# BaeHann/feature_level_style_transfer_for_TSC

Measured on AMD Instinct MI355X. Metric: train-step samples/sec (univariate TS, len=512, batch=256) at 1/2/4/8 MI355X, higher is better.
Workload: dtype bf16x3

## Files before the change

### feature_level_style_transfer_for_tsc_amd/_lib.py

```python
from __future__ import annotations

import ctypes
import os
from ctypes import POINTER, Structure, c_char_p, c_float, c_int, c_int32, c_int64, c_void_p
from typing import Optional

import torch

ABI_VERSION = 21
_LIB_NAME = "libfst_hip.so"
_HERE = os.path.dirname(os.path.abspath(__file__))
LIB_PATH = os.environ.get("FST_HIP_LIB", os.path.join(_HERE, _LIB_NAME))


class FstLibraryError(RuntimeError):
    pass


class WSrc(Structure):
    _fields_ = [("w", c_void_p), ("off0", c_int64), ("sm", c_int64), ("sc", c_int64), ("st", c_int64)]


_P = c_void_p
_I32P = c_void_p
_SIGNATURES = {
    "fst_version": (c_int, []),
    "fst_last_error": (c_char_p, []),
    "fst_pack_weights": (c_int, [_I32P, _I32P, c_int, POINTER(WSrc), POINTER(WSrc), c_int, c_int, c_int, c_int, _P, c_void_p]),
    "fst_pack_weights_bf16x3": (c_int, [_I32P, _I32P, c_int, POINTER(WSrc), POINTER(WSrc), c_int, c_int, c_int, c_int, _P, c_void_p]),
    "fst_unpack_weights": (c_int, [_I32P, _I32P, c_int, _P, c_int, _P, c_int64, c_int64, c_int64, c_int64,
                                   _P, c_int64, c_int64, c_int64, c_int64, c_int, c_void_p]),
    "fst_mask_taps": (c_int, [_P, _I32P, _I32P, c_int, c_int, c_int, c_void_p]),
    "fst_conv_gemm": (c_int, [_P, c_int64, _P, c_int64, _P, _I32P, _I32P, c_int, _P, _P, c_int64, _P, c_int64,
                              _P, c_int64, c_int, c_int, c_int, c_int, c_int, c_int, c_int, c_int, c_void_p]),
    "fst_conv_wgrad": (c_int, [_P, c_int64, _P, c_int64, _P, c_int64, _P, c_int64, c_int, _P, _I32P, _I32P, c_int,
                               c_int, c_int, c_int, c_int, c_int, c_int64, c_void_p]),
    "fst_conv_last_route": (c_int, [POINTER(c_int32)]),
    "fst_row_sum": (c_int, [_P, c_int64, c_int, c_int, c_int, _P, c_void_p]),
    "fst_bn_stats": (c_int, [_P, c_int, c_int, c_int, _P, c_int64, c_void_p]),
    "fst_bn_finalize": (c_int, [_P, c_int, _P, _P, _P, _P, c_int, c_int, c_float, c_float, _P, c_void_p]),
    "fst_bn_apply": (c_int, [_P, _P, _P, _P, _P, c_int, c_int, c_int, c_int, c_int64, c_void_p]),
    "fst_bn_bwd_reduce": (c_int, [_P, _P, _P, _P, c_int, c_int, c_int, c_int, _P, c_int64, c_void_p]),
    "fst_bn_bwd_apply": (c_int, [_P, _P, _P, _P, _P, c_int, _P, _P, _P, c_int, c_int, c_int, c_int, c_int, c_int, c_int64, c_void_p]),
    "fst_bn_bwd_reduce_join": (c_int, [_P, _P, _P, _P, _P, c_int, c_int, c_int, _P, _P, c_int64, c_void_p]),
    "fst_bn_bwd_apply_join": (c_int, [_P, _P, _P, _P, _P, _P, _P, c_int, _P, _P, _P, _P, _P, _P, c_int, c_int, c_int, c_int, c_int,
                                      c_int64, c_void_p]),
    "fst_gate_fwd": (c_int, [_P, _P, c_int, c_int, c_int, c_int64, c_void_p]),
    "fst_gate_bwd": (c_int, [_P, _P, _P, c_int, c_int, c_int, c_int64, c_void_p]),
    "fst_coupling_sum_slots": (c_int64, [c_int, c_int, c_int]),
    "fst_coupling_fwd": (c_int, [_P, _P, _P, c_int, c_int, c_int, c_int64, _P, c_void_p]),
    "fst_coupling_bwd": (c_int, [_P, _P, _P, _P, _P, _P, _P, _P, c_int, c_int, c_int, c_int64, c_void_p]),
    "fst_coupling_inv_fwd": (c_int, [_P, _P, _P, c_int, c_int, c_int, c_int64, c_void_p]),
    "fst_coupling_inv_bwd": (c_int, [_P, _P, _P, _P, _P, c_int, c_int, c_int, c_int64, c_void_p]),
    "fst_rmsprop_multi": (c_int, [_P, _P, _P, _P, _P, c_int, c_float, c_float, c_void_p]),
    "fst_adam_multi": (c_int, [_P, _P, _P, _P, _P, c_int, _P, c_float, c_float, c_float, c_float, c_void_p]),
    "fst_rmsprop_multi_dev": (c_int, [_P, _P, _P, _P, _P, c_int, c_float, c_float, c_void_p]),
    "fst_adam_multi_dev": (c_int, [_P, _P, _P, _P, _P, c_int, _P, _P, c_float, c_float, c_float, c_void_p]),
    "fst_nonfinite_slots": (c_int64, [c_int]),
    "fst_nonfinite_multi": (c_int, [_P, _P, _I32P, c_int, c_int32, _I32P, c_int64, _I32P, _I32P, _P, _I32P, c_void_p]),
    "fst_rmsprop_multi_guard": (c_int, [_P, _P, _P, _P, _P, _P, c_int, c_float, c_float, _I32P, c_void_p]),
    "fst_adam_multi_guard": (c_int, [_P, _P, _P, _P, _P, c_int, _P, c_float, _P, c_float, c_float, c_float, _I32P, c_void_p]),
    "fst_guard_copy_multi": (c_int, [_P, _P, _P, c_int, _I32P, c_int, c_void_p]),
    "fst_wn_stack_fwd_ok": (c_int, [c_int, c_int, c_int, c_int]),
    "fst_wn_stack_fwd": (c_int, [_P, _P, _P, c_int64, _P, _P, _P, c_int64, _P, c_int, c_int, c_int, c_int, c_int, c_int64, c_void_p]),
    "fst_wn_stack_infer": (c_int, [_P, _P, _P, c_int64, _P, _P, c_int64, _P, c_int, c_int, c_int, c_int, c_int, c_int64, c_void_p]),
    "fst_wn_stack_bwd_ok": (c_int, [c_int, c_int, c_int, c_int]),
    "fst_wn_stack_bwd": (c_int, [_P, _P, _P, _P, _P, _P, _P, _P, _P, c_int64, c_int, c_int, c_int, c_int, c_int, c_int64, c_void_p]),
    "fst_wn_stack_bwd_proj": (c_int, [_P, _P, _P, _P, _P, _P, _P, _P, c_int, c_int64, _P, c_int64, c_int, c_int, c_int, c_int, c_int,
                                      c_int64, c_void_p]),
    "fst_wn_wgrad_ok": (c_int, [c_int, c_int, c_int, c_int, c_int, c_int]),
    "fst_wn_wgrad_workspace_floats": (c_int64, [c_int, c_int, c_int, c_int, c_int, c_int]),
    "fst_wn_wgrad_in": (c_int, [_P, _P, _P, c_int, c_int64, _P, _P, _P, c_int64, c_int, c_int, c_int, c_int, c_int, c_int, c_int64,
                                c_void_p]),
    "fst_wn_wgrad_rs": (c_int, [_P, _P, _P, c_int, _P, _P, c_int64, c_int, c_int, c_int, c_int, c_int64, c_void_p]),
    "fst_wn_wgrad_in_slabs": (c_int, [_P, _P, _P, c_int, c_int64, _P, c_int64, c_int, c_int, c_int, c_int, c_int, c_int, c_int64,
                                      c_void_p]),
    "fst_wn_wgrad_rs_slabs": (c_int, [_P, _P, _P, c_int, _P, c_int64, c_int, c_int, c_int, c_int, c_int64, c_void_p]),
    "fst_wn_wgrad_reduce_many": (c_int, [_I32P, _I32P, _I32P, _P, _P, _P, _P, c_int, c_int, c_int, c_int, c_int, c_void_p]),
    "fst_nt_gemm_workspace_floats": (c_int64, [c_int, c_int, c_int]),
    "fst_nt_gemm": (c_int, [_P, _P, _P, _P, c_int64, c_int, c_int, c_int, _P, _P, c_int, c_float, _P, c_void_p]),
    "fst_tap_wgrad_ok": (c_int, [c_int, c_int, c_int, c_int, c_int, c_int, c_int]),
    "fst_tap_wgrad_workspace_floats": (c_int64, [c_int, c_int, c_int, c_int, c_int]),
    "fst_tap_wgrad": (c_int, [_P, _P, _P, _P, c_int64, c_int, c_int, c_int, c_int, c_int, c_int, c_int, c_int, c_int64, c_int64, c_void_p]),
    "fst_dense_tap_wgrad_ok": (c_int, [c_int, c_int, c_int, c_int, c_int, c_int]),
    "fst_dense_tap_wgrad_workspace_floats": (c_int64, [c_int, c_int, c_int, c_int, c_int]),
    "fst_dense_tap_wgrad": (c_int, [_P, _P, _P, _P, c_int64, c_int, c_int, c_int, c_int, c_int, c_int, c_int64, c_int64, c_void_p]),
    "fst_wn_last_route": (c_int, [POINTER(c_int32)]),
    "fst_relu_bwd": (c_int, [_P, _P, _P, c_int64, c_void_p]),
    "fst_gemm_workspace_floats": (c_int64, [c_int, c_int, c_int]),
    "fst_gemm": (c_int, [_P, c_int64, c_int, _P, c_int64, c_int, _P, c_int64, c_int, c_int, c_int, _P, c_int, c_float, _P, c_int64,
                         c_void_p]),
    "fst_gemm_f32_workspace_floats": (c_int64, [c_int, c_int, c_int]),
    "fst_gemm_f32": (c_int, [_P, c_int64, c_int, _P, c_int64, c_int, _P, c_int64, c_int, c_int, c_int, _P, c_int, c_float, _P, c_int64,
                             c_void_p]),
    "fst_act_bwd": (c_int, [_P, _P, _P, c_int64, c_float, c_void_p]),
    "fst_batch_sum": (c_int, [_P, _P, _P, c_int, c_int64, c_int, c_void_p]),
    "fst_noise_transfer_fwd": (c_int, [_P, c_int, c_int, _P, _P, c_float, c_float, _P, _P, _P, _P, _P, _P, _P, c_int, c_int, c_void_p]),
    "fst_bcast_add": (c_int, [_P, _P, _P, c_int, c_int64, c_void_p]),
    "fst_noise_transfer_bwd": (c_int, [_P, c_int, _P, _P, _P, _P, c_int, c_int, c_void_p]),
    "fst_noise_transfer_dw": (c_int, [_P, _P, _P, _P, c_int, c_int, c_void_p]),
    "fst_noise_transfer_bwd_apply": (c_int, [_P, _P, _P, _P, c_float, c_float, c_int, _P, _P, c_int64, c_void_p]),
    "fst_wn_fold_fwd": (c_int, [_P, c_int, _P, _P, c_void_p]),
    "fst_wn_fold_bwd": (c_int, [_P, c_int, _P, _P, _P, c_void_p]),
    "fst_logdet_inv": (c_int, [_P, c_int, _P, _P, c_void_p]),
    "fst_wn_image_bytes": (c_int64, [c_int, c_int]),
    "fst_wn_pack": (c_int, [_P, _P, _P, _P, _P, _P, c_int, c_int, c_int, c_int, _P, c_int64, c_void_p]),
    "fst_wn_pack_stack": (c_int, [_P, _P, _P, _P, _P, _P, c_int, c_int, c_int, c_int, _P, c_int64, c_void_p]),
    "fst_wn_layer_fwd": (c_int, [_P, c_int64, _P, c_int64, _P, c_int64, _P, _P, _P, _P, c_int, c_int, c_int, c_int, c_int, c_int,
                                 c_int, c_int64, c_void_p]),
    "fst_wn_layer_infer": (c_int, [_P, c_int64, _P, c_int64, _P, c_int64, _P, _P, c_int, c_int, c_int, c_int, c_int, c_int, c_int,
                                   c_int64, c_void_p]),
    "fst_wn_bwd_image_bytes": (c_int64, [c_int, c_int]),
    "fst_wn_pack_bwd": (c_int, [_P, c_int, c_int, c_int, _P, c_int64, c_void_p]),
    "fst_wn_pack_bwd_stack": (c_int, [_P, c_int, c_int, c_int, _P, c_int64, c_void_p]),
    "fst_wn_bwd_proj_image_bytes": (c_int64, [c_int, c_int, c_int]),
    "fst_wn_pack_bwd_proj_stack": (c_int, [_P, _P, c_int, c_int, c_int, _P, c_int64, c_void_p]),
    "fst_wn_layer_bwd": (c_int, [_P, _P, _P, _P, c_int64, _P, _P, c_int64, c_int, c_int, c_int, c_int, c_int64, c_void_p]),
    "fst_wn_dgrad_image_bytes": (c_int64, [c_int]),
    "fst_wn_pack_dgrad": (c_int, [_P, _P, c_int, c_int, c_int, _P, c_int64, c_void_p]),
    "fst_wn_pack_dgrad_stack": (c_int, [_P, _P, c_int, c_int, c_int, c_int, _P, c_int64, c_void_p]),
    "fst_wn_dgrad_fits": (c_int, [c_int, c_int, c_int]),
    "fst_wn_layer_dgrad": (c_int, [_P, _P, c_int64, _P, _P, _P, _P, c_int64, c_int, c_int, c_int, c_int, c_int, c_int64, c_int64,
                                   c_void_p]),
    "fst_gru_fwd": (c_int, [_P, _P, _P, _P, _P, _I32P, c_int, c_int, c_int, c_int, c_int64, c_void_p]),
    "fst_gru_bwd": (c_int, [_P, _P, _P, _P, _I32P, c_int, _P, _P, c_int, c_int, c_int, c_int64, c_void_p]),
    "fst_lstm2_fwd": (c_int, [_P, _P, _P, _P, c_int, c_int, c_int64, c_void_p]),
    "fst_lstm2_bwd": (c_int, [_P, _P, _P, _P, _P, c_int, c_int, c_int64, c_void_p]),
    "fst_axpy": (c_int, [_P, _P, c_float, c_int64, c_void_p]),
    "fst_add_slices": (c_int, [_P, c_int64, _P, c_int64, _P, c_int64, c_int, c_int, c_int, c_void_p]),
    "fst_cpc_workspace_floats": (c_int64, [c_int, c_int, c_int, c_int]),
    "fst_cpc_nce_slots": (c_int64, [c_int, c_int, c_int, c_int]),
    "fst_cpc_nce_fwd": (c_int, [_P, c_int64, c_int64, c_int64, _I32P, _P, c_int, c_int, c_int, c_int, c_int, _P, _P, _P, c_void_p]),
    "fst_cpc_nce_bwd": (c_int, [_P, c_int64, c_int64, c_int64, _I32P, _P, _P, c_int, c_int, c_int, c_int, c_int, _P, _P, _P,
                                c_void_p]),
}
EXPORTED_SYMBOLS = tuple(_SIGNATURES)

_lib: Optional[ctypes.CDLL] = None


def load(path: Optional[str] = None) -> ctypes.CDLL:
    global _lib
    if _lib is not None and path is None:
        return _lib
    p = path or LIB_PATH
    if not os.path.exists(p):
        raise FstLibraryError(
            f"{p} not found — build it with `python -c 'import __graft_entry__ as g; g.build()'` "
            "(hipcc --offload-arch=gfx950).  There is no CPU fallback.")
    try:
        lib = ctypes.CDLL(p)
    except OSError as e:
        raise FstLibraryError(f"cannot load {p}: {e}") from e
    for name, (res, args) in _SIGNATURES.items():
        try:
            fn = getattr(lib, name)
        except AttributeError as e:
            raise FstLibraryError(f"{p} does not export {name}; rebuild the library") from e
        fn.restype, fn.argtypes = res, args
    if lib.fst_version() != ABI_VERSION:
        raise FstLibraryError(f"{p}: ABI version {lib.fst_version()} != expected {ABI_VERSION}; rebuild")
    if path is None:
        _lib = lib
    return lib


def check(rc: int, what: str) -> None:
    if rc != 0:
        msg = load().fst_last_error()
        raise RuntimeError(f"{what} failed (rc={rc}): {msg.decode() if msg else '?'}")


def stream_ptr() -> int:
    return torch.cuda.current_stream().cuda_stream


def ptr(t: Optional[torch.Tensor]) -> Optional[int]:
    return None if t is None else t.data_ptr()


def require_gpu_tensor(t: torch.Tensor, name: str) -> None:
    if not t.is_cuda:
        raise FstLibraryError(f"{name} lives on {t.device}; the fst ops run on an MI355X only (no CPU fallback)")
    if t.dtype != torch.float32:
        raise TypeError(f"{name} must be float32, got {t.dtype}")
```

### feature_level_style_transfer_for_tsc_amd/csrc/wn_fused.hip

```cpp
#include "fst_device.h"
#include <type_traits>

#define WS_MAXL 10
#define WN_TN 128
#define WN_A_BYTES (8 * 2048)
#define WN_TILE_BYTES (32 * 36 * 4)
#define WN_FWD_LDS(NW) (3 * (WN_A_BYTES + 2 * (((NW) + 1) * 1024 + 128)))

__device__ __forceinline__ float wn_sigmoid(float x) {
  return __builtin_amdgcn_rcpf(1.0f + __builtin_amdgcn_exp2f(-1.44269504f * x));
}
__device__ __forceinline__ float wn_tanh(float x) {
  return 1.0f - 2.0f * __builtin_amdgcn_rcpf(1.0f + __builtin_amdgcn_exp2f(2.88539008f * x));
}

constexpr int WN_GRP = 2;
__host__ __device__ __forceinline__ void wn_stage_chunk_tap(int k, int CH, int& c, int& tap) {
  const int g = k / (3 * WN_GRP), rem = k - g * 3 * WN_GRP;
  const int gs = CH - g * WN_GRP < WN_GRP ? CH - g * WN_GRP : WN_GRP;
  tap = rem / gs;
  c = g * WN_GRP + rem - gs * tap;
}

struct WnPackParams {
// ... 508 lines not shown
#pragma unroll
    for (int mb = 0; mb < 8; ++mb) {
      if (mb + 1 < 8 && !(p.last && mb + 1 < 4)) a_frag(mb + 1);
      if (!(p.last && mb < 4)) mfma_bf3(acc[mb], fah[mb % 2], fal[mb % 2], bh2[ks], bl2[ks]);
      if (more && mb >= 4) {
        __builtin_amdgcn_sched_barrier(0);
        issue_piece(nxt, mb - 4);
        __builtin_amdgcn_sched_barrier(0);
      }
    }
    slot = slot == 2 ? 0 : slot + 1;
  }

  FST_T(tg2);
  FST_ACC(7, tg1, tg2);
#pragma unroll
  for (int blk = 0; blk < 4; ++blk) {
    const int rows_e = n - blk * 32;
    if (!p.last) ws_acc_store(acc[blk], an_rs, wl, blk * 32, tcol, rows_e, L);
    ws_acc_store(acc[blk + 4], out_rs, wl, blk * 32, tcol, rows_e, L);
  }
  FST_T(tg3);
  FST_ACC(8, tg2, tg3);
  FST_ACC(9, ts0, tg3);
  FST_FLUSH(wn_stamps);
}

template <int NW>
__global__ __launch_bounds__(64 * NW, NW == 4 ? 2 : 1) void wn_layer_fwd_kernel(WnFwdParams p) {
  extern __shared__ __attribute__((aligned(16))) float lds[];
  int wg = blockIdx.x;
  if ((p.n_wg & 7) == 0) wg = (wg & 7) * (p.n_wg >> 3) + (wg >> 3);
  const int b = wg / p.tiles_per_seq;
  const int t0 = (wg - b * p.tiles_per_seq) * (32 * NW);
  wn_fwd_tile<NW>(*(WnFwdArgs*)__builtin_amdgcn_kernarg_segment_ptr(), b, t0, reinterpret_cast<char*>(lds));
}

struct WnFwdStackParams {
  WnFwdParams layer[WS_MAXL];
  int nl;
};

__global__ __launch_bounds__(512, 1) void wn_stack_fwd_kernel(WnFwdStackParams ps_by_value) {
  extern __shared__ __attribute__((aligned(16))) float lds[];
  typedef const __attribute__((address_space(4))) WnFwdStackParams StackArgs;
  StackArgs& ps = *(StackArgs*)__builtin_amdgcn_kernarg_segment_ptr();
  (void)ps_by_value;
  char* const ldsb = reinterpret_cast<char*>(lds);
  const int B = ps.layer[0].B, passes = ps.layer[0].tiles_per_seq;
  for (int b = blockIdx.x; b < B; b += gridDim.x) {
    for (int layer = 0; layer < ps.nl; ++layer) {
      for (int pass = 0; pass < passes; ++pass) {
        WnFwdArgs* qp = &ps.layer[layer];
        asm volatile("" : "+s"(qp));
        wn_fwd_tile<8>(*qp, b, pass * 256, ldsb);
        wait_vmcnt<0>();
        __syncthreads();
      }
    }
  }
}

template <int NW>
__global__ __launch_bounds__(64 * NW, NW == 4 ? 2 : 1) void wn_layer_infer_kernel(WnFwdParams p) {
  extern __shared__ __attribute__((aligned(16))) float lds[];
  int wg = blockIdx.x;
  if ((p.n_wg & 7) == 0) wg = (wg & 7) * (p.n_wg >> 3) + (wg >> 3);
  const int b = wg / p.tiles_per_seq;
  const int t0 = (wg - b * p.tiles_per_seq) * (32 * NW);
  wn_fwd_tile<NW, false>(*(WnFwdArgs*)__builtin_amdgcn_kernarg_segment_ptr(), b, t0, reinterpret_cast<char*>(lds));
}

__global__ __launch_bounds__(512, 1) void wn_stack_infer_kernel(WnFwdStackParams ps_by_value) {
  extern __shared__ __attribute__((aligned(16))) float lds[];
  typedef const __attribute__((address_space(4))) WnFwdStackParams StackArgs;
  StackArgs& ps = *(StackArgs*)__builtin_amdgcn_kernarg_segment_ptr();
  (void)ps_by_value;
  char* const ldsb = reinterpret_cast<char*>(lds);
  const int B = ps.layer[0].B, passes = ps.layer[0].tiles_per_seq;
  for (int b = blockIdx.x; b < B; b += gridDim.x) {
    for (int layer = 0; layer < ps.nl; ++layer) {
      for (int pass = 0; pass < passes; ++pass) {
        WnFwdArgs* qp = &ps.layer[layer];
        asm volatile("" : "+s"(qp));
        wn_fwd_tile<8, false>(*qp, b, pass * 256, ldsb);
        wait_vmcnt<0>();
        __syncthreads();
      }
    }
  }
}

extern "C" int fst_wn_stack_fwd_ok(int n, int h, int L, int nl) {
  return n > 0 && n < 128 && h > 0 && L > 0 && L % 256 == 0 && nl >= 1 && nl <= WS_MAXL;
}

static int wn_stack_fwd_launch(const char* who, bool save, const float* const* a_in, const int64_t* a_bs, const void* const* images,
                               int64_t image_bytes, float* const* ts, float* const* a_next, const float* u0, int64_t u0_bs,
                               float* out, int nl, int B, int L, int n, int h, int64_t numel_a, void* stream) {
  FST_REQUIRE(a_in && a_bs && images && (ts || !save) && a_next && u0 && out, "%s: null operand", who);
  FST_REQUIRE(fst_wn_stack_fwd_ok(n, h, L, nl) && B > 0, "%s: B=%d L=%d n=%d h=%d nl=%d (needs n < 128, L %% 256 == 0, "
              "1 <= nl <= %d)", who, B, L, n, h, nl, WS_MAXL);
  FST_REQUIRE((long long)B * n * L == (long long)numel_a, "%s: B*n*L = %d*%d*%d does not match the element count %lld "
              "of the [B, n, L] tensors", who, B, n, L, (long long)numel_a);
  FST_REQUIRE(image_bytes == fst_wn_image_bytes(n, h), "%s: images are %lld bytes, expected %lld", who,
              (long long)image_bytes, (long long)fst_wn_image_bytes(n, h));
  FST_REQUIRE(B == 1 || u0_bs >= (int64_t)h * L, "%s: batch stride of u0 smaller than a sample", who);
  FST_REQUIRE(u0_bs % 4 == 0 && fst_aligned16(u0) && fst_aligned16(out), "%s: needs 16-byte aligned tensors", who);
  WnFwdStackParams p = {};
  for (int i = 0; i < nl; ++i) {
    const bool last = i == nl - 1;
    float* const ts_i = save ? ts[i] : nullptr;
    FST_REQUIRE(a_in[i] && images[i] && (ts_i || !save) && (a_next[i] || last), "%s: null operand of layer %d", who, i);
    FST_REQUIRE(a_bs[i] >= (int64_t)n * L && a_bs[i] % 4 == 0 && fst_aligned16(a_in[i]) && fst_aligned16(images[i]) && fst_aligned16(ts_i) && fst_aligned16(a_next[i]),
                "%s: layer %d: batch stride %lld smaller than a sample, or an operand that is not 16-byte aligned", who, i,
                (long long)a_bs[i]);
    FST_REQUIRE(last || a_in[i + 1] == a_next[i], "%s: the input of layer %d is not the a_next of layer %d", who, i + 1, i);
    FST_REQUIRE(save || last || a_next[i] != a_in[i], "%s: layer %d would store a_next over the input its neighbouring "
                "tiles still read", who, i);
    WnFwdParams& q = p.layer[i];
    q.a = a_in[i]; q.a_bs = a_bs[i]; q.u0 = u0; q.u0_bs = u0_bs; q.img = static_cast<const char*>(images[i]);
    q.ts = ts_i; q.acts = nullptr; q.a_next = last ? nullptr : a_next[i]; q.out = out;
    q.B = B; q.L = L; q.n = n; q.h = h; q.dil = 1 << i; q.first = i == 0; q.last = last;
    q.CH = wn_ch(n); q.CH2 = wn_ch2(h); q.tiles_per_seq = L / 256; q.n_wg = 0;
  }
  p.nl = nl;
  const int cus = fst_cu_count_or(256);
  const dim3 grid((unsigned)(B < cus ? B : cus));
  if (int rc = fst_allow_full_lds(save ? (const void*)wn_stack_fwd_kernel : (const void*)wn_stack_infer_kernel, who)) return rc;
  fst_wn_set_route(save ? FST_WN_ROUTE_STACK_FWD : FST_WN_ROUTE_STACK_INFER, 8, 0, 0, 0, (int)grid.x, 1, 1, L / 256, 3, nl, WN_FWD_LDS(8));
  if (save) {
    hipLaunchKernelGGL(wn_stack_fwd_kernel, grid, dim3(512), WN_FWD_LDS(8), (hipStream_t)stream, p);
  } else {
    hipLaunchKernelGGL(wn_stack_infer_kernel, grid, dim3(512), WN_FWD_LDS(8), (hipStream_t)stream, p);
  }
  FST_LAUNCH_CHECK();
  return 0;
}

extern "C" int fst_wn_stack_fwd(const float* const* a_in, const int64_t* a_bs, const void* const* images, int64_t image_bytes,
                                float* const* ts, float* const* a_next, const float* u0, int64_t u0_bs, float* out, int nl, int B,
                                int L, int n, int h, int64_t numel_a, void* stream) {
  fst_wn_clear_route();
  return wn_stack_fwd_launch("fst_wn_stack_fwd", true, a_in, a_bs, images, image_bytes, ts, a_next, u0, u0_bs, out, nl, B, L, n, h,
                             numel_a, stream);
}

extern "C" int fst_wn_stack_infer(const float* const* a_in, const int64_t* a_bs, const void* const* images, int64_t image_bytes,
                                  float* const* a_next, const float* u0, int64_t u0_bs, float* out, int nl, int B, int L, int n, int h,
                                  int64_t numel_a, void* stream) {
  fst_wn_clear_route();
  return wn_stack_fwd_launch("fst_wn_stack_infer", false, a_in, a_bs, images, image_bytes, nullptr, a_next, u0, u0_bs, out, nl, B, L,
                             n, h, numel_a, stream);
}

static int wn_layer_fwd_launch(const char* who, bool save, const float* a, int64_t a_bs, const float* u0, int64_t u0_bs,
                               const void* image, int64_t image_bytes, float* ts, float* acts, float* a_next, float* out, int first,
                               int last, int B, int L, int n, int h, int dil, int64_t numel_a, void* stream) {
  FST_REQUIRE(a && u0 && image && (ts || !save) && out && (last || a_next), "%s: null operand", who);
  FST_REQUIRE(B > 0 && L > 0 && n > 0 && n < 128 && h > 0 && dil > 0, "%s: B=%d L=%d n=%d h=%d dil=%d (needs n < 128)", who,
              B, L, n, h, dil);
  FST_REQUIRE((long long)B * n * L == (long long)numel_a, "%s: B*n*L = %d*%d*%d does not match the element count %lld "
              "of the [B, n, L] tensors", who, B, n, L, (long long)numel_a);
  FST_REQUIRE(image_bytes == fst_wn_image_bytes(n, h), "%s: image is %lld bytes, expected %lld", who,
              (long long)image_bytes, (long long)fst_wn_image_bytes(n, h));
  FST_REQUIRE(B == 1 || (a_bs >= (int64_t)n * L && u0_bs >= (int64_t)h * L), "%s: batch stride smaller than a sample", who);
  FST_REQUIRE(L % 4 == 0 && a_bs % 4 == 0 && u0_bs % 4 == 0 && fst_aligned16(a) && fst_aligned16(u0) && fst_aligned16(image) && fst_aligned16(ts) && fst_aligned16(acts) &&
              fst_aligned16(a_next) && fst_aligned16(out), "%s: needs L %% 4 == 0 and 16-byte aligned tensors (L=%d)", who, L);
  FST_REQUIRE(save || last || a_next != a, "%s: a_next is a — a tile's neighbours read a's halo while the tile stores a_next", who);
  WnFwdParams p;
  p.a = a; p.a_bs = a_bs; p.u0 = u0; p.u0_bs = u0_bs; p.img = static_cast<const char*>(image);
  p.ts = ts; p.acts = acts; p.a_next = last ? nullptr : a_next; p.out = out;
  p.B = B; p.L = L; p.n = n; p.h = h; p.dil = dil; p.first = first ? 1 : 0; p.last = last ? 1 : 0;
  p.CH = wn_ch(n); p.CH2 = wn_ch2(h);
  const int cus = fst_cu_count_or(256);
  const int nw = (L % 256 == 0 && (long long)B * (L / 256) >= cus) ? 8 : 4;
  const int tn = 32 * nw;
  p.tiles_per_seq = (L + tn - 1) / tn;
  p.n_wg = B * p.tiles_per_seq;
  const dim3 grid((unsigned)p.n_wg), block(64 * nw);
  const int lds = nw == 8 ? WN_FWD_LDS(8) : WN_FWD_LDS(4);
  const void* const kernel = save ? (nw == 8 ? (const void*)wn_layer_fwd_kernel<8> : (const void*)wn_layer_fwd_kernel<4>)
                                  : (nw == 8 ? (const void*)wn_layer_infer_kernel<8> : (const void*)wn_layer_infer_kernel<4>);
  if (int rc = fst_allow_full_lds(kernel, who)) return rc;
  fst_wn_set_route(save ? FST_WN_ROUTE_LAYER_FWD : FST_WN_ROUTE_LAYER_INFER, nw, 0, 0, 0, p.n_wg, 1, 1, p.tiles_per_seq, 3, 1, lds);
  if (save) {
    if (nw == 8) hipLaunchKernelGGL(wn_layer_fwd_kernel<8>, grid, block, lds, (hipStream_t)stream, p);
    else hipLaunchKernelGGL(wn_layer_fwd_kernel<4>, grid, block, lds, (hipStream_t)stream, p);
  } else {
    if (nw == 8) hipLaunchKernelGGL(wn_layer_infer_kernel<8>, grid, block, lds, (hipStream_t)stream, p);
    else hipLaunchKernelGGL(wn_layer_infer_kernel<4>, grid, block, lds, (hipStream_t)stream, p);
  }
  FST_LAUNCH_CHECK();
  return 0;
}

extern "C" int fst_wn_layer_fwd(const float* a, int64_t a_bs, const float* u0, int64_t u0_bs, const void* image,
                                int64_t image_bytes, float* ts, float* acts, float* a_next, float* out, int first, int last,
                                int B, int L, int n, int h, int dil, int64_t numel_a, void* stream) {
  fst_wn_clear_route();
  return wn_layer_fwd_launch("fst_wn_layer_fwd", true, a, a_bs, u0, u0_bs, image, image_bytes, ts, acts, a_next, out, first, last, B, L,
                             n, h, dil, numel_a, stream);
}

extern "C" int fst_wn_layer_infer(const float* a, int64_t a_bs, const float* u0, int64_t u0_bs, const void* image,
                                  int64_t image_bytes, float* a_next, float* out, int first, int last, int B, int L, int n, int h,
                                  int dil, int64_t numel_a, void* stream) {
  fst_wn_clear_route();
  return wn_layer_fwd_launch("fst_wn_layer_infer", false, a, a_bs, u0, u0_bs, image, image_bytes, nullptr, nullptr, a_next, out, first,
                             last, B, L, n, h, dil, numel_a, stream);
}

constexpr int WN_BWD_OCC = 2;
#define WN_BW_NB 4
#define WN_BW_GS (WN_BW_NB * 1024 + 128)
#define WN_BW_A (4 * 2048)
#define WN_BW_SLOT (WN_BW_A + 2 * WN_BW_GS)
#define WN_BW_LDS (3 * WN_BW_SLOT)

struct WnPackBwdParams {
  const float* rs_w;
  int n, last, CH;
  uint4* img;
  int acc_order;
};

__device__ __forceinline__ void wn_pack_bwd_body(const WnPackBwdParams& p, int bx, int n_blocks) {
  const int lane = threadIdx.x, blk = bx & 3, st = bx >> 2;
  const int n = p.n, hh = lane >> 5, m = blk * 32 + (lane & 31);
  const int src = p.last ? 0 : st / p.CH, c = st - src * p.CH;
  float v[8];
#pragma unroll
  for (int j = 0; j < 8; ++j) {
    const bool perm = p.acc_order && !p.last && src == 0;
    const int ch = 16 * c + (perm ? 8 * (j >> 2) + 4 * hh + (j & 3) : 8 * hh + j);
    v[j] = (m < n && ch < n) ? p.rs_w[(long long)(src * n + ch) * n + m] : 0.f;
  }
  unsigned hi[4], lo[4];
#pragma unroll
  for (int j = 0; j < 4; ++j) split_bf16_pair(v[2 * j], v[2 * j + 1], hi[j], lo[j]);
  uint4* dst = p.img + ((long long)st * 4 + blk) * 128 + lane;
  dst[0] = make_uint4(hi[0], hi[1], hi[2], hi[3]);
  dst[64] = make_uint4(lo[0], lo[1], lo[2], lo[3]);
  if (bx == 0 && lane == 0) p.img[(long long)n_blocks * 128] = make_uint4(0u, 0u, 0u, 0u);
}

__global__ __launch_bounds__(64) void wn_pack_bwd_kernel(WnPackBwdParams p) { wn_pack_bwd_body(p, blockIdx.x, gridDim.x); }

struct WnPackBwdStackParams {
  const float* rs_w[WS_MAXL];
  uint4* img[WS_MAXL];
  int n, nl, CH, acc_order;
};

__global__ __launch_bounds__(64) void wn_pack_bwd_stack_kernel(WnPackBwdStackParams s) {
  const int i = blockIdx.y, last = i == s.nl - 1 ? 1 : 0, n_blocks = (last ? 1 : 2) * s.CH * 4;
  if ((int)blockIdx.x >= n_blocks) return;
  const WnPackBwdParams p = {s.rs_w[i], s.n, last, s.CH, s.img[i], s.acc_order};
  wn_pack_bwd_body(p, blockIdx.x, n_blocks);
}

extern "C" int64_t fst_wn_bwd_image_bytes(int n, int last) {
  if (n <= 0) return -1;
  return (int64_t)(last ? 1 : 2) * wn_ch(n) * WN_BW_A + 16;
}

extern "C" int fst_wn_pack_bwd(const float* rs_w, int n, int last, int acc_order, void* image, int64_t image_bytes, void* stream) {
  FST_REQUIRE(rs_w && image && n > 0 && n <= 128, "fst_wn_pack_bwd: bad arguments (n=%d, needs n <= 128)", n);
  FST_REQUIRE(image_bytes == fst_wn_bwd_image_bytes(n, last), "fst_wn_pack_bwd: image is %lld bytes, expected %lld",
              (long long)image_bytes, (long long)fst_wn_bwd_image_bytes(n, last));
  FST_REQUIRE(fst_aligned16(image), "fst_wn_pack_bwd: image must be 16-byte aligned");
  WnPackBwdParams p = {rs_w, n, last ? 1 : 0, wn_ch(n), static_cast<uint4*>(image), acc_order ? 1 : 0};
  const int stages = (last ? 1 : 2) * p.CH;
  hipLaunchKernelGGL(wn_pack_bwd_kernel, dim3((unsigned)(stages * 4)), dim3(64), 0, (hipStream_t)stream, p);
  FST_LAUNCH_CHECK();
  return 0;
}

extern "C" int fst_wn_pack_bwd_stack(const float* const* rs_w, int nl, int n, int acc_order, void* const* images, int64_t image_bytes,
                                     void* stream) {
  FST_REQUIRE(rs_w && images && n > 0 && n <= 128, "fst_wn_pack_bwd_stack: bad arguments (n=%d, needs n <= 128)", n);
  FST_REQUIRE(nl >= 1 && nl <= WS_MAXL, "fst_wn_pack_bwd_stack: %d layers (1..%d)", nl, WS_MAXL);
  FST_REQUIRE(image_bytes == fst_wn_bwd_image_bytes(n, 0), "fst_wn_pack_bwd_stack: images are %lld bytes, expected %lld",
              (long long)image_bytes, (long long)fst_wn_bwd_image_bytes(n, 0));
  WnPackBwdStackParams s = {};
  for (int i = 0; i < nl; ++i) {
    FST_REQUIRE(rs_w[i] && images[i], "fst_wn_pack_bwd_stack: null operand in layer %d", i);
    FST_REQUIRE(fst_aligned16(images[i]), "fst_wn_pack_bwd_stack: images must be 16-byte aligned");
    s.rs_w[i] = rs_w[i];
    s.img[i] = static_cast<uint4*>(images[i]);
  }
  s.n = n; s.nl = nl; s.CH = wn_ch(n); s.acc_order = acc_order ? 1 : 0;
  const int stages = (nl > 1 ? 2 : 1) * s.CH;
  hipLaunchKernelGGL(wn_pack_bwd_stack_kernel, dim3((unsigned)(stages * 4), (unsigned)nl), dim3(64), 0, (hipStream_t)stream, s);
  FST_LAUNCH_CHECK();
  return 0;
}

struct WnPackBwdProjParams {
  const float* rs_w[WS_MAXL];
  uint4* img[WS_MAXL];
  const float* end_w;
  int n, h2, nl, CH, CHO;
};

__global__ __launch_bounds__(64) void wn_pack_bwd_proj_stack_kernel(WnPackBwdProjParams s) {
  const int i = blockIdx.y, last = i == s.nl - 1 ? 1 : 0, n_da = last ? 0 : s.CH, n_blocks = (n_da + s.CHO) * 4;
  const int bx = blockIdx.x;
  if (bx >= n_blocks) return;
  if ((bx >> 2) < n_da) {
    const WnPackBwdParams p = {s.rs_w[i], s.n, 0, s.CH, s.img[i], 1};
    wn_pack_bwd_body(p, bx, n_blocks);
    return;
  }
  const int lane = threadIdx.x, blk = bx & 3, c = (bx >> 2) - n_da;
  const int n = s.n, m = blk * 32 + (lane & 31), hh = lane >> 5;
  const float* const w_skip = s.rs_w[i] + (long long)(last ? 0 : n) * n;
  __shared__ float e_rows[16 * 128];
  for (int x = lane; x < 16 * n; x += 64) {
    const int r = x / n, k = x - r * n;
    e_rows[r * 128 + k] = 16 * c + r < s.h2 ? s.end_w[(long long)(16 * c + r) * n + k] : 0.f;
  }
  __syncthreads();
  float v[8];
#pragma unroll
  for (int j = 0; j < 8; ++j) v[j] = 0.f;
  if (m < n) {
#pragma unroll 8
    for (int k = 0; k < n; ++k) {
      const float w = w_skip[(long long)k * n + m];
#pragma unroll
      for (int j = 0; j < 8; ++j) v[j] = fmaf(e_rows[(8 * hh + j) * 128 + k], w, v[j]);
    }
  }
#pragma unroll
  for (int j = 0; j < 8; ++j)
    if (16 * c + 8 * hh + j >= s.h2) v[j] = 0.f;
  unsigned hi[4], lo[4];
#pragma unroll
  for (int j = 0; j < 4; ++j) split_bf16_pair(v[2 * j], v[2 * j + 1], hi[j], lo[j]);
  uint4* dst = s.img[i] + ((long long)(bx >> 2) * 4 + blk) * 128 + lane;
  dst[0] = make_uint4(hi[0], hi[1], hi[2], hi[3]);
  dst[64] = make_uint4(lo[0], lo[1], lo[2], lo[3]);
  if (bx == 0 && lane == 0) s.img[i][(long long)n_blocks * 128] = make_uint4(0u, 0u, 0u, 0u);
}

extern "C" int64_t fst_wn_bwd_proj_image_bytes(int n, int h2, int last) {
  if (n <= 0 || h2 <= 0) return -1;
  return (int64_t)((last ? 0 : wn_ch(n)) + wn_ch(h2)) * WN_BW_A + 16;
}

extern "C" int fst_wn_pack_bwd_proj_stack(const float* const* rs_w, const float* end_w, int nl, int n, int h2, void* const* images,
                                          int64_t image_bytes, void* stream) {
  FST_REQUIRE(rs_w && end_w && images && n > 0 && n <= 128 && h2 > 0 && h2 <= 64,
              "fst_wn_pack_bwd_proj_stack: bad arguments (n=%d, h2=%d; needs n <= 128, h2 <= 64)", n, h2);
  FST_REQUIRE(nl >= 1 && nl <= WS_MAXL, "fst_wn_pack_bwd_proj_stack: %d layers (1..%d)", nl, WS_MAXL);
  FST_REQUIRE(image_bytes == fst_wn_bwd_proj_image_bytes(n, h2, 0), "fst_wn_pack_bwd_proj_stack: images are %lld bytes, expected %lld",
              (long long)image_bytes, (long long)fst_wn_bwd_proj_image_bytes(n, h2, 0));
  WnPackBwdProjParams s = {};
  for (int i = 0; i < nl; ++i) {
    FST_REQUIRE(rs_w[i] && images[i], "fst_wn_pack_bwd_proj_stack: null operand in layer %d", i);
    FST_REQUIRE(fst_aligned16(images[i]), "fst_wn_pack_bwd_proj_stack: images must be 16-byte aligned");
    s.rs_w[i] = rs_w[i];
    s.img[i] = static_cast<uint4*>(images[i]);
  }
  s.end_w = end_w; s.n = n; s.h2 = h2; s.nl = nl; s.CH = wn_ch(n); s.CHO = wn_ch(h2);
  const int stages = (nl > 1 ? s.CH : 0) + s.CHO;
  hipLaunchKernelGGL(wn_pack_bwd_proj_stack_kernel, dim3((unsigned)(stages * 4), (unsigned)nl), dim3(64), 0, (hipStream_t)stream, s);
  FST_LAUNCH_CHECK();
  return 0;
}

struct WnBwdParams {
  const float* d_a;
  const float* d_out;
  const float* ts;
  const char* img;
  float* dg;
  float* row_sums;
  int B, L, n, last, CH, tiles_per_seq, n_wg;
};

__device__ __forceinline__ void wn_bwd_multiply(f32x16 (&acc)[4], const char* base, int lane, bf16x8 bh, bf16x8 bl) {
#pragma unroll
  for (int mb = 0; mb < 4; ++mb) {
    bf16x8 ah, al;
    lds_read_a_frag(base, mb, lane, ah, al);
    mfma_bf3(acc[mb], ah, al, bh, bl);
  }
}

__device__ __forceinline__ void wn_reduce_row_sums(const float* rsum, int R, float* out, int stride, int col, int tid) {
  __syncthreads();
  if (tid < R) {
    float s8 = 0.f;
#pragma unroll
    for (int w = 0; w < 8; ++w) s8 += rsum[w * R + tid];
    out[(long long)tid * stride + col] = s8;
  }
}

__global__ __launch_bounds__(256, WN_BWD_OCC) void wn_layer_bwd_kernel(WnBwdParams p) {
  extern __shared__ __attribute__((aligned(16))) float lds[];
  char* const ldsb = reinterpret_cast<char*>(lds);
  const int tid = threadIdx.x, lane = tid & 63;
  const int half = lane >> 5, l31 = lane & 31;
  const int wave_s = __builtin_amdgcn_readfirstlane(tid >> 6);
  int wg = blockIdx.x;
  if ((p.n_wg & 7) == 0) wg = (wg & 7) * (p.n_wg >> 3) + (wg >> 3);
  const int b = wg / p.tiles_per_seq;
  const int t0 = (wg - b * p.tiles_per_seq) * WN_TN;
  const int wave_n0 = wave_s * 32;
  const int L = p.L, n = p.n, CH = p.CH;
  const int S3 = (p.last ? 1 : 2) * CH;
  const char* const zero16 = p.img + (long long)S3 * WN_BW_A;
  const float* const ts_b = p.ts + (long long)b * (2 * n) * L;
  const int tcol = t0 + wave_n0;

  auto issue = [&](int k, int slot) {
    char* const sl = ldsb + slot * WN_BW_SLOT;
    const char* asrc = p.img + (long long)k * WN_BW_A;
    const bool from_da = !p.last && k < CH;
    const int c = from_da ? k : k - (p.last ? 0 : CH);
    const float* xb = (from_da ? p.d_a : p.d_out) + ((long long)b * n + 16 * c) * L;
    const int c_count = min(16, n - 16 * c);
#pragma unroll
    for (int i = 0; i < 4; ++i) {
      const int idx = wave_s + 4 * i;
      if (idx < 8) {
        lds_dma16(asrc + idx * 1024 + lane * 16, sl + idx * 1024);
      } else {
        const int bi = idx - 8;
        const int gq = bi >> 2, m = bi & 3;
        const int row = 8 * gq + (lane >> 3);
        const int t = t0 + 32 * m + 4 * (lane & 7);
        const bool ok = row < c_count && t < L;
        const char* src = ok ? reinterpret_cast<const char*>(xb + ((long long)row * L + t)) : zero16;
        lds_dma16(src, sl + WN_BW_A + gq * WN_BW_GS + m * 1024);
      }
    }
  };

  f32x16 acc[4];
#pragma unroll
  for (int mb = 0; mb < 4; ++mb)
#pragma unroll
    for (int r = 0; r < 16; ++r) acc[mb][r] = 0.f;

  float4 qt[4], qs[4];
  wn_fetch_tile(qt, ts_b, n, L, tcol, lane);
  wn_fetch_tile(qs, ts_b + (long long)n * L, n, L, tcol, lane);
  asm volatile("" ::: "memory");
  issue(0, 0);
  if (S3 > 1) issue(1, 1);
  int slot = 0;
  for (int k = 0; k < S3; ++k) {
    if (k + 1 < S3) wait_vmcnt<4>(); else wait_vmcnt<0>();
    __builtin_amdgcn_s_barrier();
    if (k + 2 < S3) issue(k + 2, slot >= 1 ? slot - 1 : 2);
    const char* base = ldsb + slot * WN_BW_SLOT;
    const int colx = wave_n0 + l31;
    const char* bp = base + WN_BW_A + half * WN_BW_GS + (colx >> 5) * 1024 + (colx & 31) * 4;
    float v[8];
#pragma unroll
    for (int j = 0; j < 8; ++j) v[j] = *reinterpret_cast<const float*>(bp + j * 128);
    bf16x8 bh, bl;
    split_bf16x8(v, bh, bl);
    wn_bwd_multiply(acc, base, lane, bh, bl);
    slot = slot == 2 ? 0 : slot + 1;
  }
  __syncthreads();
  float* const tile = reinterpret_cast<float*>(ldsb + wave_s * WN_TILE_BYTES);
  float* const rsum = reinterpret_cast<float*>(ldsb + 4 * WN_TILE_BYTES);
  float* const rsum_w = rsum + wave_s * 256;
  if (p.row_sums) {
#pragma unroll
    for (int w = 0; w < 4; ++w) rsum[w * 256 + tid] = 0.f;
    __syncthreads();
  }
  float* const dg_b = p.dg + (long long)b * (2 * n) * L;
#pragma unroll
  for (int blk = 0; blk < 4; ++blk) {
    const int rows_valid = n - blk * 32;
    float tv[16], sv[16], gt[16], gs[16];
    wn_tile_to_acc(tv, qt, tile, lane);
    wn_tile_to_acc(sv, qs, tile, lane);
    if (blk < 3) {
      wn_fetch_tile(qt, ts_b + (long long)((blk + 1) * 32) * L, n - (blk + 1) * 32, L, tcol, lane);
      wn_fetch_tile(qs, ts_b + (long long)(n + (blk + 1) * 32) * L, n - (blk + 1) * 32, L, tcol, lane);
    }
#pragma unroll
    for (int r = 0; r < 16; ++r) {
      const float d = acc[blk][r], t = tv[r], s = sv[r];
      gt[r] = d * s * (1.f - t * t);
      gs[r] = d * t * s * (1.f - s);
    }
    wn_store_tile<0>(gt, tile, dg_b + (long long)(blk * 32) * L, nullptr, rows_valid, L, tcol, lane);
    if (p.row_sums) wn_tile_row_sums(tile, rsum_w, blk * 32, rows_valid, L, tcol, lane);
    wn_store_tile<0>(gs, tile, dg_b + (long long)(n + blk * 32) * L, nullptr, rows_valid, L, tcol, lane);
    if (p.row_sums) wn_tile_row_sums(tile, rsum_w, n + blk * 32, rows_valid, L, tcol, lane);
  }
  if (p.row_sums) {
    __syncthreads();
    p.row_sums[(long long)tid * p.n_wg + wg] = (rsum[tid] + rsum[256 + tid]) + (rsum[512 + tid] + rsum[768 + tid]);
  }
}

extern "C" int fst_wn_layer_bwd(const float* d_a, const float* d_out, const float* ts, const void* image, int64_t image_bytes,
                                float* dg, float* row_sums, int64_t row_sums_rows, int last, int B, int L, int n,
                                int64_t numel_a, void* stream) {
  fst_wn_clear_route();
  FST_REQUIRE(d_out && ts && image && dg && (last || d_a), "fst_wn_layer_bwd: null operand");
  FST_REQUIRE(B > 0 && L > 0 && n > 0 && n <= 128, "fst_wn_layer_bwd: B=%d L=%d n=%d (needs n <= 128)", B, L, n);
  FST_REQUIRE((long long)B * n * L == (long long)numel_a, "fst_wn_layer_bwd: B*n*L = %d*%d*%d does not match the element count %lld "
              "of the [B, n, L] tensors", B, n, L, (long long)numel_a);
  FST_REQUIRE(image_bytes == fst_wn_bwd_image_bytes(n, last), "fst_wn_layer_bwd: image is %lld bytes, expected %lld",
              (long long)image_bytes, (long long)fst_wn_bwd_image_bytes(n, last));
  FST_REQUIRE(L % 4 == 0 && fst_aligned16(d_a) && fst_aligned16(d_out) && fst_aligned16(ts) && fst_aligned16(image) && fst_aligned16(dg),
              "fst_wn_layer_bwd: needs L %% 4 == 0 and 16-byte aligned tensors (L=%d)", L);
  WnBwdParams p;
  p.d_a = last ? nullptr : d_a; p.d_out = d_out; p.ts = ts; p.img = static_cast<const char*>(image); p.dg = dg;
  p.row_sums = row_sums;
  p.B = B; p.L = L; p.n = n; p.last = last ? 1 : 0; p.CH = wn_ch(n);
  p.tiles_per_seq = (L + WN_TN - 1) / WN_TN;
  p.n_wg = B * p.tiles_per_seq;
  FST_REQUIRE(row_sums == nullptr || row_sums_rows == p.n_wg, "fst_wn_layer_bwd: row_sums has %lld rows, the launch has %d "
              "workgroups (B x ceil(L/128))", (long long)row_sums_rows, p.n_wg);
  if (int rc = fst_allow_full_lds((const void*)wn_layer_bwd_kernel, "fst_wn_layer_bwd")) return rc;
  fst_wn_set_route(FST_WN_ROUTE_LAYER_BWD, 0, 0, 0, 0, p.n_wg, 1, 1, p.tiles_per_seq, 3, 1, WN_BW_LDS);
  hipLaunchKernelGGL(wn_layer_bwd_kernel, dim3((unsigned)p.n_wg), dim3(256), WN_BW_LDS, (hipStream_t)stream, p);
  FST_LAUNCH_CHECK();
  return 0;
}

#define DG_NCB 2
#define DG_TN (8 * 32 * DG_NCB)
#define DG_A_BLOCKS 13
#define DG_A_BYTES (DG_A_BLOCKS * 2048)

struct WnPackDgradParams {
  const float* in_w;
  const float* cond_w;
  int n, h, CHK;
  uint4* img;
};

__device__ __forceinline__ void wn_pack_dgrad_body(const WnPackDgradParams& p, int bx, int n_blocks) {
  const int lane = threadIdx.x, ab = bx % DG_A_BLOCKS, c = bx / DG_A_BLOCKS;
  const int n = p.n, h = p.h, hh = lane >> 5, l31 = lane & 31;
  int tap, blk;
  if (ab < 4) { tap = 0; blk = ab; } else if (ab < 9) { tap = 1; blk = ab - 4; } else { tap = 2; blk = ab - 9; }
  float v[8];
#pragma unroll
  for (int j = 0; j < 8; ++j) {
    const int k = 16 * c + 8 * hh + j;
    float w = 0.f;
    if (k < 2 * n) {
      if (blk < 4) {
        const int m = blk * 32 + l31;
        if (m < n) w = p.in_w[((long long)k * n + m) * 3 + tap];
      } else {
        if (l31 < h) w = p.cond_w[(long long)k * h + l31];
      }
    }
    v[j] = w;
  }
  unsigned hi[4], lo[4];
#pragma unroll
  for (int j = 0; j < 4; ++j) split_bf16_pair(v[2 * j], v[2 * j + 1], hi[j], lo[j]);
  uint4* dst = p.img + (long long)bx * 128 + lane;
  dst[0] = make_uint4(hi[0], hi[1], hi[2], hi[3]);
  dst[64] = make_uint4(lo[0], lo[1], lo[2], lo[3]);
  if (bx == 0 && lane == 0) p.img[(long long)n_blocks * 128] = make_uint4(0u, 0u, 0u, 0u);
}

__global__ __launch_bounds__(64) void wn_pack_dgrad_kernel(WnPackDgradParams p) { wn_pack_dgrad_body(p, blockIdx.x, gridDim.x); }

struct WnPackDgradStackParams {
  const float* in_w[WS_MAXL];
  const float* cond_w[WS_MAXL];
  uint4* img[WS_MAXL];
  int n, h, CHK;
};

__global__ __launch_bounds__(64) void wn_pack_dgrad_stack_kernel(WnPackDgradStackParams s) {
  const int i = blockIdx.y;
  const WnPackDgradParams p = {s.in_w[i], s.cond_w[i], s.n, s.h, s.CHK, s.img[i]};
  wn_pack_dgrad_body(p, blockIdx.x, gridDim.x);
}

extern "C" int64_t fst_wn_dgrad_image_bytes(int n) {
  if (n <= 0) return -1;
  return (int64_t)((2 * n + 15) / 16) * DG_A_BYTES + 16;
}

extern "C" int fst_wn_pack_dgrad(const float* in_w, const float* cond_w, int n, int h, int ntaps, void* image, int64_t image_bytes,
                                 void* stream) {
  FST_REQUIRE(in_w && cond_w && image && n > 0 && n <= 128 && h > 0 && h <= 32, "fst_wn_pack_dgrad: needs n <= 128, h <= 32 (n=%d h=%d)", n, h);
  FST_REQUIRE(ntaps == 3, "fst_wn_pack_dgrad: the fused WN kernels are 3-tap (in_w [2n][n][3]); got %d taps", ntaps);
  FST_REQUIRE(image_bytes == fst_wn_dgrad_image_bytes(n), "fst_wn_pack_dgrad: image is %lld bytes, expected %lld",
              (long long)image_bytes, (long long)fst_wn_dgrad_image_bytes(n));
  FST_REQUIRE(fst_aligned16(image), "fst_wn_pack_dgrad: image must be 16-byte aligned");
  WnPackDgradParams p = {in_w, cond_w, n, h, (2 * n + 15) / 16, static_cast<uint4*>(image)};
  hipLaunchKernelGGL(wn_pack_dgrad_kernel, dim3((unsigned)(p.CHK * DG_A_BLOCKS)), dim3(64), 0, (hipStream_t)stream, p);
  FST_LAUNCH_CHECK();
  return 0;
}

extern "C" int fst_wn_pack_dgrad_stack(const float* const* in_w, const float* const* cond_w, int nl, int n, int h, int ntaps,
                                       void* const* images, int64_t image_bytes, void* stream) {
  FST_REQUIRE(in_w && cond_w && images && n > 0 && n <= 128 && h > 0 && h <= 32, "fst_wn_pack_dgrad_stack: needs n <= 128, h <= 32 (n=%d h=%d)", n, h);
  FST_REQUIRE(nl >= 1 && nl <= WS_MAXL, "fst_wn_pack_dgrad_stack: %d layers (1..%d)", nl, WS_MAXL);
  FST_REQUIRE(ntaps == 3, "fst_wn_pack_dgrad_stack: the fused WN kernels are 3-tap (in_w [2n][n][3]); got %d taps", ntaps);
  FST_REQUIRE(image_bytes == fst_wn_dgrad_image_bytes(n), "fst_wn_pack_dgrad_stack: images are %lld bytes, expected %lld",
              (long long)image_bytes, (long long)fst_wn_dgrad_image_bytes(n));
  WnPackDgradStackParams s = {};
  for (int i = 0; i < nl; ++i) {
    FST_REQUIRE(in_w[i] && cond_w[i] && images[i], "fst_wn_pack_dgrad_stack: null operand in layer %d", i);
    FST_REQUIRE(fst_aligned16(images[i]), "fst_wn_pack_dgrad_stack: images must be 16-byte aligned");
    s.in_w[i] = in_w[i]; s.cond_w[i] = cond_w[i];
    s.img[i] = static_cast<uint4*>(images[i]);
  }
  s.n = n; s.h = h; s.CHK = (2 * n + 15) / 16;
  hipLaunchKernelGGL(wn_pack_dgrad_stack_kernel, dim3((unsigned)(s.CHK * DG_A_BLOCKS), (unsigned)nl), dim3(64), 0, (hipStream_t)stream, s);
  FST_LAUNCH_CHECK();
  return 0;
}

__device__ __forceinline__ void wn_dgrad_issue(char* sl, const char* img, const float* dg_b, int c, int t0, int n, int L, int dil,
                                               int nblkw, int gsw, int wave_s, int lane) {
  const char* asrc = img + (long long)c * DG_A_BYTES;
  const char* const zero16 = img + (long long)((2 * n + 15) / 16) * DG_A_BYTES;
  const float* xb = dg_b + (long long)(16 * c) * L;
  const int c_count = min(16, 2 * n - 16 * c);
  const int w4 = (t0 - dil) & ~3;
  const int NI = DG_A_BLOCKS * 2 + 2 * nblkw;
  for (int idx = wave_s; idx < NI; idx += 8) {
    if (idx < 2 * DG_A_BLOCKS) {
      lds_dma16(asrc + idx * 1024 + lane * 16, sl + idx * 1024);
    } else {
      const int bi = idx - 2 * DG_A_BLOCKS;
      const int gq = bi >= nblkw ? 1 : 0, m = bi - gq * nblkw;
      const int row = 8 * gq + (lane >> 3);
      const int t = w4 + 32 * m + 4 * (lane & 7);
      const bool ok = row < c_count && t >= 0 && t < L;
      const char* src = ok ? reinterpret_cast<const char*>(xb + ((long long)row * L + t)) : zero16;
      lds_dma16(src, sl + DG_A_BYTES + gq * gsw + m * 1024);
    }
  }
}

__device__ __forceinline__ void wn_dgrad_stage(f32x16 (&acc)[5][DG_NCB], const char* base, int gsw, int wave_n0, int dil, int sub,
                                               int lane) {
  const int half = lane >> 5, l31 = lane & 31;
#pragma unroll
  for (int tap = 0; tap < 3; ++tap) {
    bf16x8 bh[DG_NCB], bl[DG_NCB];
#pragma unroll
    for (int cb = 0; cb < DG_NCB; ++cb) {
      const int colx = wave_n0 + 32 * cb + l31 + (2 - tap) * dil + sub;
      const char* bp = base + DG_A_BYTES + half * gsw + (colx >> 5) * 1024 + (colx & 31) * 4;
      float v8[8];
#pragma unroll
      for (int j = 0; j < 8; ++j) v8[j] = *reinterpret_cast<const float*>(bp + j * 128);
      split_bf16x8(v8, bh[cb], bl[cb]);
    }
    const char* ab = base + (tap == 0 ? 0 : (tap == 1 ? 4 : 9)) * 2048;
#pragma unroll
    for (int mb = 0; mb < 5; ++mb) {
      if (mb == 4 && tap != 1) continue;
      bf16x8 ah, al;
      lds_read_a_frag(ab, mb, lane, ah, al);
#pragma unroll
      for (int cb = 0; cb < DG_NCB; ++cb) mfma_bf3(acc[mb][cb], ah, al, bh[cb], bl[cb]);
    }
  }
}

struct WnDgradParams {
  const float* dg;
  const char* img;
  const float* d_a;
  float* d_a_new;
  float* d_u0;
  long long d_u0_bs;
  float* row_sums;
  int B, L, n, h, dil, CHK, tiles_per_seq, n_wg;
  int nblkw;
  int gsw;
  int slot;
  int ns;
};

template <int N>
__device__ __forceinline__ void wn_wait_sw(int n) {
  if (n == N) { wait_vmcnt<N>(); return; }
  if constexpr (N > 0) wn_wait_sw<N - 1>(n);
}

__global__ __launch_bounds__(512, 2) void wn_layer_dgrad_kernel(WnDgradParams p) {
  extern __shared__ __attribute__((aligned(16))) float lds[];
  char* const ldsb = reinterpret_cast<char*>(lds);
  const int tid = threadIdx.x, lane = tid & 63;
  const int half = lane >> 5, l31 = lane & 31;
  const int wave_s = __builtin_amdgcn_readfirstlane(tid >> 6);
  const int wave_n0 = wave_s * (32 * DG_NCB);
  const int L = p.L, n = p.n, CHK = p.CHK, dil = p.dil;
  const int NI = DG_A_BLOCKS * 2 + 2 * p.nblkw;
  const int my_pieces = (NI - wave_s + 7) >> 3;
  const int depth = p.ns - 1;

  auto tile_of = [&](int v, int& b, int& t0) {
    int wg = v;
    if ((p.n_wg & 7) == 0) wg = (wg & 7) * (p.n_wg >> 3) + (wg >> 3);
    b = wg / p.tiles_per_seq;
    t0 = (wg - b * p.tiles_per_seq) * DG_TN;
    return wg;
  };
  auto issue = [&](int b, int t0, int c, int slot) {
    wn_dgrad_issue(ldsb + slot * p.slot, p.img, p.dg + (long long)b * (2 * n) * L, c, t0, n, L, dil, p.nblkw, p.gsw, wave_s, lane);
  };

  int first_slot = 0;
  for (int v = blockIdx.x; v < p.n_wg; v += gridDim.x) {
    int b, t0;
    const int wg = tile_of(v, b, t0);
    const int sub = (t0 - dil) & 3;
    f32x16 acc[5][DG_NCB];
#pragma unroll
    for (int mb = 0; mb < 5; ++mb)
#pragma unroll
      for (int cb = 0; cb < DG_NCB; ++cb) {
        const float* src = mb < 4 ? (p.d_a ? p.d_a + ((long long)b * n + mb * 32) * L : nullptr) : p.d_u0 + (long long)b * p.d_u0_bs;
        const int rows = mb < 4 ? (p.d_a ? n - mb * 32 : 0) : p.h;
        wn_acc_load(acc[mb][cb], src, rows, L, t0 + wave_n0 + 32 * cb, lane);
      }
    if (first_slot == 0)
      for (int d = 0; d < depth && d < CHK; ++d) issue(b, t0, d, d);

    int slot = first_slot;
    for (int c = 0; c < CHK; ++c) {
      const int newer = min(depth - 1, CHK - 1 - c);
      wn_wait_sw<16>(newer * my_pieces);
      __builtin_amdgcn_s_barrier();
      if (c + depth < CHK) issue(b, t0, c + depth, (slot + depth) % p.ns);
      wn_dgrad_stage(acc, ldsb + slot * p.slot, p.gsw, wave_n0, dil, sub, lane);
      slot = slot + 1 == p.ns ? 0 : slot + 1;
    }
    __syncthreads();
    if (v + (int)gridDim.x < p.n_wg) {
      int bn, tn;
      tile_of(v + gridDim.x, bn, tn);
      for (int d = 0; d < depth && d < CHK; ++d) issue(bn, tn, d, 1 + d);
      first_slot = 1;
    }
    float* const tile = reinterpret_cast<float*>(ldsb + wave_s * WN_TILE_BYTES);
    float* const rsum = reinterpret_cast<float*>(ldsb + 8 * WN_TILE_BYTES);
    float* const rsum_w = rsum + wave_s * 128;
    if (p.row_sums) {
      rsum[tid] = 0.f; rsum[512 + tid] = 0.f;
      __syncthreads();
    }
#pragma unroll
    for (int k = 0; k < 5 * DG_NCB; ++k) {
      const int i = k / DG_NCB, cb = k % DG_NCB, tcol = t0 + wave_n0 + 32 * cb;
      float* dst = i < 4 ? p.d_a_new + ((long long)b * n + i * 32) * L : p.d_u0 + (long long)b * p.d_u0_bs;
      const int rows = i < 4 ? n - i * 32 : p.h;
      wn_acc_store(acc[i][cb], dst, rows, L, tcol, lane);
      if (p.row_sums && i < 4) {
#pragma unroll
        for (int r = 0; r < 16; ++r) tile[((r & 3) + 8 * (r >> 2) + 4 * half) * 36 + l31] = acc[i][cb][r];
        wn_tile_row_sums(tile, rsum_w, i * 32, rows, L, tcol, lane);
      }
    }
    if (p.row_sums) wn_reduce_row_sums(rsum, 128, p.row_sums, p.n_wg, wg, tid);
  }
}

static inline void wn_dgrad_geometry(int dil, int* nblkw, int* gsw, int* slot) {
  *nblkw = (DG_TN + 2 * dil + 3 + 31) / 32;
  *gsw = *nblkw * 1024 + 128;
  *slot = DG_A_BYTES + 2 * *gsw;
}

extern "C" int fst_wn_dgrad_fits(int n, int h, int dil) {
  if (!(n > 0 && n <= 128 && h > 0 && h <= 32 && dil > 0)) return 0;
  int nblkw, gsw, slot;
  wn_dgrad_geometry(dil, &nblkw, &gsw, &slot);
  return 2 * slot <= 160 * 1024 ? 1 : 0;
}

extern "C" int fst_wn_layer_dgrad(const float* dg, const void* image, int64_t image_bytes, const float* d_a, float* d_a_new,
                                  float* d_u0, float* row_sums, int64_t row_sums_rows, int B, int L, int n, int h, int dil,
                                  int64_t numel_a, int64_t d_u0_bs, void* stream) {
  fst_wn_clear_route();
  FST_REQUIRE(dg && image && d_a_new && d_u0, "fst_wn_layer_dgrad: null operand");
  FST_REQUIRE(B > 0 && L > 0 && n > 0 && n <= 128 && h > 0 && h <= 32 && dil > 0, "fst_wn_layer_dgrad: B=%d L=%d n=%d h=%d dil=%d", B, L,
              n, h, dil);
  FST_REQUIRE((long long)B * n * L == (long long)numel_a,
              "fst_wn_layer_dgrad: B*n*L does not match the element count %lld of the [B][n][L] tensors", (long long)numel_a);
  FST_REQUIRE(d_u0_bs >= (int64_t)h * L && d_u0_bs % 4 == 0,
              "fst_wn_layer_dgrad: d_u0 batch stride %lld (needs >= h*L = %lld and a multiple of 4)", (long long)d_u0_bs, (long long)h * L);
  FST_REQUIRE(image_bytes == fst_wn_dgrad_image_bytes(n), "fst_wn_layer_dgrad: image is %lld bytes, expected %lld",
              (long long)image_bytes, (long long)fst_wn_dgrad_image_bytes(n));
  FST_REQUIRE(L % 4 == 0 && fst_aligned16(dg) && fst_aligned16(image) && fst_aligned16(d_a) && fst_aligned16(d_a_new) && fst_aligned16(d_u0),
              "fst_wn_layer_dgrad: needs L %% 4 == 0 and 16-byte aligned tensors (L=%d)", L);
  WnDgradParams p;
  p.dg = dg; p.img = static_cast<const char*>(image); p.d_a = d_a; p.d_a_new = d_a_new; p.d_u0 = d_u0; p.d_u0_bs = d_u0_bs;
  p.row_sums = row_sums;
  p.B = B; p.L = L; p.n = n; p.h = h; p.dil = dil; p.CHK = (2 * n + 15) / 16;
  p.tiles_per_seq = (L + DG_TN - 1) / DG_TN;
  p.n_wg = B * p.tiles_per_seq;
  FST_REQUIRE(row_sums == nullptr || row_sums_rows == p.n_wg, "fst_wn_layer_dgrad: row_sums has %lld rows, the launch has %d "
              "workgroups (B x ceil(L/512))", (long long)row_sums_rows, p.n_wg);
  wn_dgrad_geometry(dil, &p.nblkw, &p.gsw, &p.slot);
  p.ns = 2;
  FST_REQUIRE(2 * p.slot <= 160 * 1024, "fst_wn_layer_dgrad: dilation %d needs a %d-byte window slot: too large for LDS", dil, p.slot);
  size_t lds_bytes = (size_t)p.ns * p.slot;
  if (lds_bytes < 8 * WN_TILE_BYTES + 4096) lds_bytes = 8 * WN_TILE_BYTES + 4096;
  if (int rc = fst_allow_full_lds((const void*)wn_layer_dgrad_kernel, "fst_wn_layer_dgrad")) return rc;
  int grid = p.n_wg;
  const int cus = fst_cu_count();
  if (cus > 0 && grid > cus && (size_t)2 * lds_bytes > 160 * 1024) grid = cus;
  fst_wn_set_route(FST_WN_ROUTE_LAYER_DGRAD, 0, 0, 0, 0, grid, 1, 1, p.tiles_per_seq, p.ns, 1, (int)lds_bytes);
  hipLaunchKernelGGL(wn_layer_dgrad_kernel, dim3((unsigned)grid), dim3(512), lds_bytes, (hipStream_t)stream, p);
  FST_LAUNCH_CHECK();
  return 0;
}

__device__ __forceinline__ void ws_row_sums(const float (&v)[16], float* rows_w, int row0, int rows_valid, bool col_ok, int lane) {
  const int l31 = lane & 31, half = lane >> 5;
  float a8[8], a4[4], a2[2];
  const bool b4 = (l31 & 16) != 0, b3 = (l31 & 8) != 0, b2 = (l31 & 4) != 0, b1 = (l31 & 2) != 0;
#pragma unroll
  for (int j = 0; j < 8; ++j) {
    const float lo = col_ok ? v[j] : 0.f, hi = col_ok ? v[8 + j] : 0.f;
    a8[j] = (b4 ? hi : lo) + __shfl_xor(b4 ? lo : hi, 16, 64);
  }
#pragma unroll
  for (int j = 0; j < 4; ++j) a4[j] = (b3 ? a8[4 + j] : a8[j]) + __shfl_xor(b3 ? a8[j] : a8[4 + j], 8, 64);
#pragma unroll
  for (int j = 0; j < 2; ++j) a2[j] = (b2 ? a4[2 + j] : a4[j]) + __shfl_xor(b2 ? a4[j] : a4[2 + j], 4, 64);
  float a1 = (b1 ? a2[1] : a2[0]) + __shfl_xor(b1 ? a2[0] : a2[1], 2, 64);
  a1 += __shfl_xor(a1, 1, 64);
  const int j = (b4 ? 8 : 0) + (b3 ? 4 : 0) + (b2 ? 2 : 0) + (b1 ? 1 : 0);
  const int row = (j & 3) + 8 * (j >> 2) + 4 * half;
  if ((l31 & 1) == 0 && row < rows_valid) rows_w[row0 + row] += a1;
}

#define WS_TN 512
#define WS_NB 8
#define WS_GS (WS_NB * 1024 + 128)
#define WS_SLOT_A (WN_BW_A + 2 * WS_GS)
#define WS_LDS_A (16 * WN_BW_A)

struct WnStackParams {
  const float* ts[WS_MAXL];
  const char* img_b[WS_MAXL];
  const char* img_d[WS_MAXL];
  float* dg[WS_MAXL];
  float* da_out[WS_MAXL];
  float* rs_b[WS_MAXL];
  float* rs_d[WS_MAXL];
  const float* d_out;
  float* d_u0;
  long long d_u0_bs;
  int dil[WS_MAXL], nblkw[WS_MAXL], gsw[WS_MAXL], slot_d[WS_MAXL];
  int nl, B, L, n, h, CH, CHK;
  int SR, SCH;
};

__global__ __launch_bounds__(512, 2) void wn_stack_bwd_kernel(WnStackParams p_by_value) {
  const auto& p = *(const __attribute__((address_space(4))) WnStackParams*)__builtin_amdgcn_kernarg_segment_ptr();
  (void)p_by_value;
  extern __shared__ __attribute__((aligned(16))) float lds[];
  char* const ldsb = reinterpret_cast<char*>(lds);
  const int tid = threadIdx.x, lane = tid & 63;
  const int half = lane >> 5, l31 = lane & 31;
  const int wave_s = __builtin_amdgcn_readfirstlane(tid >> 6);
  const int wave_n0 = wave_s * 64;
  const int L = p.L, n = p.n, CH = p.CH, CHK = p.CHK;
  float* const rsum = reinterpret_cast<float*>(ldsb + WS_LDS_A);
  float* const rsum_w = rsum + wave_s * 256;
  const unsigned vlane = (unsigned)(4 * half * L + l31) * 4u;
  const WsLane wl0 = ws_lane(vlane, wave_n0, L, lane), wl1 = ws_lane(vlane, wave_n0 + 32, L, lane);

  auto issue_res = [&](int i) {
    const int S3 = (i == p.nl - 1 ? 0 : CH) + p.SCH;
    const char* const img = p.img_b[i];
    for (int c = 0; c < S3; ++c)
      lds_dma16(img + (long long)c * WN_BW_A + wave_s * 1024 + lane * 16, ldsb + c * WN_BW_A + wave_s * 1024);
  };
  const unsigned vfrag = (unsigned)(8 * half * L + l31) * 4u;

  FST_SUMS(12);
  FST_T(tw0);
  bool primed = false;
  for (int b = blockIdx.x; b < p.B; b += gridDim.x) {
    f32x16 acc[5][2];
#pragma unroll
    for (int mb = 0; mb < 4; ++mb)
#pragma unroll
      for (int cb = 0; cb < 2; ++cb)
#pragma unroll
        for (int r = 0; r < 16; ++r) acc[mb][cb][r] = 0.f;
    for (int i = p.nl - 1; i >= 0; --i) {
      const bool last = i == p.nl - 1;
      {
        const __amdgpu_buffer_rsrc_t ts_t = ws_rsrc(p.ts[i] + (long long)b * (2 * n) * L);
        const __amdgpu_buffer_rsrc_t ts_s = ws_rsrc(p.ts[i] + ((long long)b * 2 + 1) * n * L);
        const __amdgpu_buffer_rsrc_t dg_t = ws_rsrc(p.dg[i] + (long long)b * (2 * n) * L);
        const __amdgpu_buffer_rsrc_t dg_s = ws_rsrc(p.dg[i] + ((long long)b * 2 + 1) * n * L);
        const __amdgpu_buffer_rsrc_t dout_r = ws_rsrc(p.d_out + (long long)b * p.SR * L);
        float* const rs_out = p.rs_b[i];
        FST_T(ta0);
        if (!primed) issue_res(i);
        primed = false;
        if (rs_out) {
#pragma unroll
          for (int w = 0; w < 4; ++w) rsum[w * 512 + tid] = 0.f;
        }
        wait_vmcnt<0>();
        __syncthreads();
        FST_T(ta1);
        FST_ACC(0, ta0, ta1);
        const char* const w_dout = ldsb + (long long)(last ? 0 : CH) * WN_BW_A;
        auto run_pass = [&](auto pc) {
          constexpr int cb = decltype(pc)::value;
          const WsLane wl = cb ? wl1 : wl0;
          const int tcol = wave_n0 + 32 * cb;
          f32x16 da[4];
#pragma unroll
          for (int mb = 0; mb < 4; ++mb)
#pragma unroll
            for (int r = 0; r < 16; ++r) da[mb][r] = 0.f;
          FST_T(tp0);
          const unsigned vf = tcol + l31 < L ? vfrag : WS_OOB, vf_lo = half == 0 ? vf : WS_OOB;
          auto load_dout = [&](float (&v)[8], int c) {
            const int Lq = ws_opaque(L), nq = ws_opaque(p.SR);
            const int sbase = (16 * c * Lq + tcol) * 4;
#pragma unroll
            for (int j = 0; j < 8; ++j) {
              float x = 0.f;
              if (16 * c + j < nq)
                x = __builtin_bit_cast(float, __builtin_amdgcn_raw_buffer_load_b32(dout_r, 16 * c + 8 + j < nq ? vf : vf_lo, sbase + j * Lq * 4, 0));
              v[j] = x;
            }
          };
          float vn[8];
          load_dout(vn, 0);
          const int SCH = p.SCH;
          for (int k = 0; k < SCH; ++k) {
            float v[8];
#pragma unroll
            for (int j = 0; j < 8; ++j) v[j] = vn[j];
            if (k + 1 < SCH) load_dout(vn, k + 1);
            bf16x8 bh, bl;
            split_bf16x8(v, bh, bl);
            wn_bwd_multiply(da, w_dout + k * WN_BW_A, lane, bh, bl);
          }
          if (!last) {
            auto da_stage = [&](auto cc) {
              constexpr int c = decltype(cc)::value;
              if (c < CH) {
                float v[8];
#pragma unroll
                for (int j = 0; j < 8; ++j) v[j] = acc[c >> 1][cb][8 * (c & 1) + j];
                bf16x8 bh, bl;
                split_bf16x8(v, bh, bl);
                wn_bwd_multiply(da, ldsb + c * WN_BW_A, lane, bh, bl);
                __builtin_amdgcn_sched_barrier(0);
              }
            };
            da_stage(std::integral_constant<int, 0>{}); da_stage(std::integral_constant<int, 1>{});
            da_stage(std::integral_constant<int, 2>{}); da_stage(std::integral_constant<int, 3>{});
            da_stage(std::integral_constant<int, 4>{}); da_stage(std::integral_constant<int, 5>{});
            da_stage(std::integral_constant<int, 6>{}); da_stage(std::integral_constant<int, 7>{});
          }
          FST_T(tp1);
          FST_ACC(1, tp0, tp1);
#pragma unroll
          for (int blk = 0; blk < 4; ++blk) {
            const int rows_valid = n - blk * 32;
            f32x16 tv, sv;
            ws_acc_load(tv, ts_t, wl, blk * 32, tcol, rows_valid, L);
            ws_acc_load(sv, ts_s, wl, blk * 32, tcol, rows_valid, L);
            float gt[16], gs[16];
#pragma unroll
            for (int r = 0; r < 16; ++r) {
              const float d = da[blk][r], t = tv[r], s2 = sv[r];
              gt[r] = d * s2 * (1.f - t * t);
              gs[r] = d * t * s2 * (1.f - s2);
            }
            ws_acc_store(gt, dg_t, wl, blk * 32, tcol, rows_valid, L);
            ws_acc_store(gs, dg_s, wl, blk * 32, tcol, rows_valid, L);
            if (rs_out) {
              ws_row_sums(gt, rsum_w, blk * 32, rows_valid, tcol + l31 < L, lane);
              ws_row_sums(gs, rsum_w, n + blk * 32, rows_valid, tcol + l31 < L, lane);
            }
            __builtin_amdgcn_sched_barrier(0);
          }
          FST_T(tp2);
          FST_ACC(2, tp1, tp2);
        };
        run_pass(std::integral_constant<int, 0>{});
        run_pass(std::integral_constant<int, 1>{});
        if (rs_out) wn_reduce_row_sums(rsum, 256, rs_out, p.B, b, tid);
        FST_T(ta3);
        wait_vmcnt<0>();
        __syncthreads();
        FST_T(ta4);
        FST_ACC(3, ta3, ta4);
      }
      {
        const int dil = p.dil[i], nblkw = p.nblkw[i], gsw = p.gsw[i], slotb = p.slot_d[i];
        const char* const img = p.img_d[i];
        const float* const dgr = p.dg[i] + (long long)b * (2 * n) * L;
        float* const da_store = p.da_out[i];
        const __amdgpu_buffer_rsrc_t dan_r = ws_rsrc(da_store ? da_store + (long long)b * n * L : nullptr);
        const __amdgpu_buffer_rsrc_t du_r = ws_rsrc(p.d_u0 + (long long)b * p.d_u0_bs);
        float* const rs_out = p.rs_d[i];
        const int sub = (0 - dil) & 3;
        auto issue = [&](int c, int slot) { wn_dgrad_issue(ldsb + slot * slotb, img, dgr, c, 0, n, L, dil, nblkw, gsw, wave_s, lane); };
        FST_T(tb0);
        ws_acc_load(acc[4][0], du_r, wl0, 0, wave_n0, p.h, L);
        ws_acc_load(acc[4][1], du_r, wl1, 0, wave_n0 + 32, p.h, L);
        asm volatile("" ::: "memory");
        issue(0, 0);
        int slot = 0;
        FST_T(tb1);
        FST_ACC(4, tb0, tb1);
        for (int c = 0; c < CHK; ++c) {
          wait_vmcnt<0>();
          __builtin_amdgcn_s_barrier();
          if (c + 1 < CHK) issue(c + 1, slot ^ 1);
          wn_dgrad_stage(acc, ldsb + slot * slotb, gsw, wave_n0, dil, sub, lane);
          slot ^= 1;
        }
        FST_T(tb2);
        FST_ACC(5, tb1, tb2);
        __syncthreads();
        {
          const int ni = i > 0 ? i - 1 : p.nl - 1, nb = i > 0 ? b : b + (int)gridDim.x;
          if (nb < p.B) {
            issue_res(ni);
            primed = true;
          }
        }
        if (rs_out) {
          rsum[tid] = 0.f; rsum[512 + tid] = 0.f;
          __syncthreads();
        }
#pragma unroll
        for (int k = 0; k < 5 * DG_NCB; ++k) {
          const int ib = k / DG_NCB, cb = k % DG_NCB, tcol = wave_n0 + 32 * cb;
          const int rows = ib < 4 ? n - ib * 32 : p.h;
          if (ib < 4) {
            if (da_store) ws_acc_store(acc[ib][cb], dan_r, cb ? wl1 : wl0, ib * 32, tcol, rows, L);
          } else {
            ws_acc_store(acc[ib][cb], du_r, cb ? wl1 : wl0, 0, tcol, rows, L);
          }
          if (rs_out && ib < 4) {
            float av[16];
#pragma unroll
            for (int r = 0; r < 16; ++r) av[r] = acc[ib][cb][r];
            ws_row_sums(av, rsum + wave_s * 128, ib * 32, rows, tcol + l31 < L, lane);
          }
        }
        if (rs_out) wn_reduce_row_sums(rsum, 128, rs_out, p.B, b, tid);
        FST_T(tb3);
        FST_ACC(6, tb2, tb3);
        wait_vmcnt<0>();
        __syncthreads();
        FST_T(tb4);
        FST_ACC(7, tb3, tb4);
      }
    }
  }
  FST_T(tw1);
  FST_ACC(9, tw0, tw1);
  FST_FLUSH(wn_stamps);
}

extern "C" int fst_wn_stack_bwd_ok(int n, int h, int L, int nl) {
  if (!(n > 0 && n <= 128 && h > 0 && h <= 32 && L > 0 && L <= WS_TN && L % 4 == 0 && nl > 0 && nl <= WS_MAXL)) return 0;
  for (int i = 0; i < nl; ++i)
    if (i >= 20 || !fst_wn_dgrad_fits(n, h, 1 << i)) return 0;
  return 1;
}

static int wn_stack_bwd_launch(const char* who, const float* const* ts, const void* const* img_b, const void* const* img_d,
                               float* const* dg, float* const* da_out, float* const* rs_b, float* const* rs_d, const float* skip,
                               int skip_rows, float* d_u0, int64_t d_u0_bs, int nl, int B, int L, int n, int h, int64_t numel_a,
                               void* stream) {
  FST_REQUIRE(ts && img_b && img_d && dg && da_out && skip && d_u0, "%s: null table", who);
  FST_REQUIRE(fst_wn_stack_bwd_ok(n, h, L, nl), "%s: not served: n=%d h=%d L=%d nl=%d (needs n <= 128, h <= 32, "
              "L <= 512, L %% 4 == 0, nl <= %d)", who, n, h, L, nl, WS_MAXL);
  FST_REQUIRE(B > 0 && (long long)B * n * L == (long long)numel_a,
              "%s: B*n*L does not match the element count %lld of the [B][n][L] tensors", who, (long long)numel_a);
  FST_REQUIRE(d_u0_bs >= (int64_t)h * L && d_u0_bs % 4 == 0,
              "%s: d_u0 batch stride %lld (needs >= h*L = %lld and a multiple of 4)", who, (long long)d_u0_bs, (long long)h * L);
  FST_REQUIRE((rs_b == nullptr) == (rs_d == nullptr), "%s: row sums of both kinds or of neither", who);
  WnStackParams p = {};
  size_t lds_bytes = WS_LDS_A + 8192;
  for (int i = 0; i < nl; ++i) {
    FST_REQUIRE(ts[i] && img_b[i] && img_d[i] && dg[i] && (i > 0 || da_out[i]), "%s: null operand of layer %d", who, i);
    FST_REQUIRE(fst_aligned16(ts[i]) && fst_aligned16(img_b[i]) && fst_aligned16(img_d[i]) && fst_aligned16(dg[i]) && fst_aligned16(da_out[i]),
                "%s: operands of layer %d must be 16-byte aligned", who, i);
    p.ts[i] = ts[i]; p.img_b[i] = static_cast<const char*>(img_b[i]); p.img_d[i] = static_cast<const char*>(img_d[i]);
    p.dg[i] = dg[i]; p.da_out[i] = da_out[i];
    p.rs_b[i] = rs_b ? rs_b[i] : nullptr; p.rs_d[i] = rs_d ? rs_d[i] : nullptr;
    p.dil[i] = 1 << i;
    wn_dgrad_geometry(p.dil[i], &p.nblkw[i], &p.gsw[i], &p.slot_d[i]);
    if ((size_t)2 * p.slot_d[i] > lds_bytes) lds_bytes = (size_t)2 * p.slot_d[i];
  }
  FST_REQUIRE(fst_aligned16(skip) && fst_aligned16(d_u0), "%s: %s / d_u0 must be 16-byte aligned", who, skip_rows == n ? "d_out" : "d_o");
  FST_REQUIRE(lds_bytes <= 160 * 1024, "%s: %zu bytes of LDS", who, lds_bytes);
  p.d_out = skip; p.d_u0 = d_u0; p.d_u0_bs = d_u0_bs;
  p.nl = nl; p.B = B; p.L = L; p.n = n; p.h = h; p.CH = wn_ch(n); p.CHK = (2 * n + 15) / 16;
  p.SR = skip_rows; p.SCH = wn_ch(skip_rows);
  FST_REQUIRE((size_t)(p.CH + p.SCH) * WN_BW_A <= WS_LDS_A, "%s: a weight image of %d stages does not fit its LDS", who, p.CH + p.SCH);
  if (int rc = fst_allow_full_lds((const void*)wn_stack_bwd_kernel, who)) return rc;
  const int cus = fst_cu_count_or(256);
  const int grid = B < cus ? B : cus;
  fst_wn_set_route(FST_WN_ROUTE_STACK_BWD, 0, 0, 0, 0, grid, 1, 1, 1, 2, nl, (int)lds_bytes);
  hipLaunchKernelGGL(wn_stack_bwd_kernel, dim3((unsigned)grid), dim3(512), lds_bytes, (hipStream_t)stream, p);
  FST_LAUNCH_CHECK();
  return 0;
}

extern "C" int fst_wn_stack_bwd(const float* const* ts, const void* const* img_b, const void* const* img_d, float* const* dg,
                                float* const* da_out, float* const* rs_b, float* const* rs_d, const float* d_out, float* d_u0,
                                int64_t d_u0_bs, int nl, int B, int L, int n, int h, int64_t numel_a, void* stream) {
  fst_wn_clear_route();
  return wn_stack_bwd_launch("fst_wn_stack_bwd", ts, img_b, img_d, dg, da_out, rs_b, rs_d, d_out, n, d_u0, d_u0_bs, nl, B, L, n, h,
                             numel_a, stream);
}

extern "C" int fst_wn_stack_bwd_proj(const float* const* ts, const void* const* img_b, const void* const* img_d, float* const* dg,
                                     float* const* da_out, float* const* rs_b, float* const* rs_d, const float* d_o, int h2,
                                     int64_t numel_o, float* d_u0, int64_t d_u0_bs, int nl, int B, int L, int n, int h,
                                     int64_t numel_a, void* stream) {
  fst_wn_clear_route();
  FST_REQUIRE(h2 > 0 && h2 <= 64, "fst_wn_stack_bwd_proj: h2=%d (needs 0 < h2 <= 64)", h2);
  FST_REQUIRE(B > 0 && L > 0 && (long long)B * h2 * L == (long long)numel_o,
              "fst_wn_stack_bwd_proj: B*h2*L does not match the element count %lld of d_o [B][h2][L]", (long long)numel_o);
  return wn_stack_bwd_launch("fst_wn_stack_bwd_proj", ts, img_b, img_d, dg, da_out, rs_b, rs_d, d_o, h2, d_u0, d_u0_bs, nl, B, L, n, h,
                             numel_a, stream);
}
```

### feature_level_style_transfer_for_tsc_amd/ops.py

```python
from __future__ import annotations

import ctypes
import math
import os
from typing import Callable, Dict, List, NamedTuple, Optional, Sequence, Tuple

import torch

from . import _lib
from . import dist as _dist
from ._lib import WSrc, check, ptr, stream_ptr
from .plan import Plan, Segment, build_plan, pick_mb

EPI_RELU, EPI_ACC2, EPI_ATOMIC, EPI_ACC1 = 1, 2, 4, 8
GEMM_BF16X3 = 16
WGRAD_SLABS = 32
MATH = os.environ.get("FST_MATH", "bf16x3")
LDS_BUDGET = 96 * 1024
LDS_MULTI_CHUNK = 44 * 1024
PIPE_C = 16

_PARTIAL_BACKWARD = False


class KernelTimer:

    def __init__(self, detail: bool = False):
        self.detail = detail
        self.records = {}

    def begin(self):
        ev = torch.cuda.Event(enable_timing=True)
        ev.record()
        return ev

    def end(self, key: str, start, flops: float, nbytes: float = 0.0):
        ev = torch.cuda.Event(enable_timing=True)
        ev.record()
        self.records.setdefault(key, []).append((start, ev, flops, nbytes))

    def summary(self):
        torch.cuda.synchronize()
        out = {}
        for key, recs in self.records.items():
            ms = sum(r[0].elapsed_time(r[1]) for r in recs)
            out[key] = {"launches": len(recs), "total_ms": ms, "avg_us": 1e3 * ms / len(recs),
                        "flops": sum(r[2] for r in recs), "bytes": sum(r[3] for r in recs)}
        return out


KERNEL_TIMER: Optional[KernelTimer] = None


ROUTE_GEMM, ROUTE_PIPE, ROUTE_BF3, ROUTE_WIN_BF3, ROUTE_WIN_ROWS, ROUTE_WGRAD = 1, 2, 3, 4, 5, 6
ROUTE_EPI_PLAIN, ROUTE_EPI_ADD, ROUTE_EPI_ATOMIC, ROUTE_EPI_VEC, ROUTE_EPI_VEC_ADD = 0, 1, 2, 3, 4
_ROUTE_NAMES = {ROUTE_GEMM: "conv_gemm_kernel", ROUTE_PIPE: "conv_gemm_pipe_kernel", ROUTE_BF3: "conv_gemm_bf3_kernel",
                ROUTE_WIN_BF3: "conv_win_bf3_kernel", ROUTE_WIN_ROWS: "conv_win_rows_kernel", ROUTE_WGRAD: "conv_wgrad_kernel"}
_ROUTE_NARGS = {ROUTE_GEMM: 2, ROUTE_PIPE: 3, ROUTE_BF3: 2, ROUTE_WIN_BF3: 2, ROUTE_WIN_ROWS: 0, ROUTE_WGRAD: 5}
_ROUTE_BOOLS = {(ROUTE_PIPE, 2), (ROUTE_WGRAD, 2), (ROUTE_WGRAD, 4)}


def last_route() -> Tuple[int, ...]:
    out = (ctypes.c_int32 * 8)()
    _lib.load().fst_conv_last_route(out)
    return tuple(out)


WN_ROUTE_WGRAD, WN_ROUTE_TZ, WN_ROUTE_LAYER_FWD, WN_ROUTE_STACK_FWD, WN_ROUTE_LAYER_BWD, WN_ROUTE_LAYER_DGRAD, WN_ROUTE_STACK_BWD = \
    1, 2, 3, 4, 5, 6, 7
WN_ROUTE_LAYER_INFER, WN_ROUTE_STACK_INFER = 8, 9
WN_ROUTE_LEN = 12
_WN_ROUTE_NAMES = {WN_ROUTE_WGRAD: "wn_wgrad_kernel", WN_ROUTE_TZ: "tz_wgrad_kernel", WN_ROUTE_LAYER_FWD: "wn_layer_fwd_kernel",
                   WN_ROUTE_STACK_FWD: "wn_stack_fwd_kernel", WN_ROUTE_LAYER_BWD: "wn_layer_bwd_kernel",
                   WN_ROUTE_LAYER_DGRAD: "wn_layer_dgrad_kernel", WN_ROUTE_STACK_BWD: "wn_stack_bwd_kernel",
                   WN_ROUTE_LAYER_INFER: "wn_layer_infer_kernel", WN_ROUTE_STACK_INFER: "wn_stack_infer_kernel"}


def wn_last_route() -> Tuple[int, ...]:
    out = (ctypes.c_int32 * WN_ROUTE_LEN)()
    _lib.load().fst_wn_last_route(out)
    return tuple(out)


def wn_route_kernel_name(route: Sequence[int]) -> str:
    fam, tf = route[0], ("false", "true")
    if fam == WN_ROUTE_WGRAD:
        return f"wn_wgrad_kernel<2, {route[1]}, {tf[route[2]]}, {tf[route[3]]}, {route[4]}>"
    if fam == WN_ROUTE_TZ:
        return f"tz_wgrad_kernel<{route[1]}, {tf[route[2]]}>"
    if fam == WN_ROUTE_LAYER_FWD:
        return f"wn_layer_fwd_kernel<{route[1]}>"
    if fam == WN_ROUTE_LAYER_INFER:
        return f"wn_layer_infer_kernel<{route[1]}>"
    return _WN_ROUTE_NAMES[fam]


def route_kernel_name(route: Sequence[int]) -> str:
    fam = route[0]
    args = [("true" if route[1 + i] else "false") if (fam, i) in _ROUTE_BOOLS else str(route[1 + i])
            for i in range(_ROUTE_NARGS[fam])]
    return _ROUTE_NAMES[fam] + (f"<{', '.join(args)}>" if args else "")


def bf3_ok(plan: Plan, L: int) -> bool:
    if MATH != "bf16x3":
        return False
    return (plan.pipeable and L % 4 == 0) or plan.windowed16


def _plan_macs_per_step(plan: Plan, M: int) -> int:
    total = 0
    ch, en = plan.chunks(), plan.entries()
    rows_per_group = plan.MB * 32
    for g in range(plan.n_mgroups):
        rows = max(0, min(M, (g + 1) * rows_per_group) - g * rows_per_group)
        for q in range(plan.n_chunks):
            lo, hi = int(en[g, q, 0]), int(en[g, q, 1])
            if hi > lo:
                total += rows * (hi - lo) * int(ch[q, 2])
    return total


class partial_backward:

    def __enter__(self):
        global _PARTIAL_BACKWARD
        self._prev, _PARTIAL_BACKWARD = _PARTIAL_BACKWARD, True
        return self

    def __exit__(self, *exc):
        global _PARTIAL_BACKWARD
        _PARTIAL_BACKWARD = self._prev
        return False


def _want_weight_grad(spec=None) -> bool:
    return (not _PARTIAL_BACKWARD) or bool(getattr(spec, "always_weight_grad", False))

Tensor = torch.Tensor


def _ncl(t: Tensor, name: str) -> Tuple[int, int]:
    _lib.require_gpu_tensor(t, name)
    if t.dim() != 3 or t.stride(2) != 1 or (t.size(1) > 1 and t.stride(1) != t.size(2)):
        raise ValueError(f"{name}: expected NCL view with channel stride L, got shape {tuple(t.shape)} strides {t.stride()}")
    return t.stride(0), t.size(2)


def _same_numel(*tensors: Optional[Tensor]) -> int:
    ts = [t for t in tensors if t is not None]
    n = ts[0].numel()
    for t in ts:
        if t.numel() != n or not t.is_contiguous():
            raise ValueError(f"pointwise launch over tensors of different extents / non-contiguous: {[tuple(x.shape) for x in ts]}")
    return n


def _gate_numel(acts: Tensor, *pairs: Tensor) -> int:
    n = _same_numel(acts)
    for t in pairs:
        if t.numel() != 2 * n or not t.is_contiguous():
            raise ValueError(f"gate launch: {tuple(t.shape)} is not the contiguous [B, 2n, L] partner of {tuple(acts.shape)}")
    return n


def _wsrc(t: Optional[Tensor], off0: int, sm: int, sc: int, st: int) -> WSrc:
    if t is not None:
        _lib.require_gpu_tensor(t, "weight")
    return WSrc(ptr(t) if t is not None else None, off0, sm, sc, st)


_PACK_CACHE: Optional[dict] = None


class pack_cache:

    def __enter__(self):
        global _PACK_CACHE
        self._prev, _PACK_CACHE = _PACK_CACHE, {}
        return self

    def __exit__(self, *exc):
        global _PACK_CACHE
        _PACK_CACHE = self._prev
        return False


def pack_weights(plan: Plan, M: int, w0: Tensor, s0: Tuple[int, int, int, int], w1: Optional[Tensor] = None,
                 s1: Tuple[int, int, int, int] = (0, 0, 0, 0), parts=None, bf3: bool = False) -> Tensor:
    if _PACK_CACHE is not None:
        key = (id(plan), bf3, M, w0.data_ptr(), w0._version, s0, None if w1 is None else (w1.data_ptr(), w1._version), s1,
               None if parts is None else tuple((p[0], p[1], p[2], p[3], p[4].data_ptr(), p[4]._version, p[5]) for p in parts))
        hit = _PACK_CACHE.get(key)
        if hit is not None:
            return hit[0]
        a = _pack_weights(plan, M, w0, s0, w1, s1, parts, bf3)
        _PACK_CACHE[key] = (a, w0, w1, plan, parts)
        return a
    return _pack_weights(plan, M, w0, s0, w1, s1, parts, bf3)


def _pack_weights(plan: Plan, M: int, w0: Tensor, s0, w1: Optional[Tensor], s1, parts=None, bf3: bool = False) -> Tensor:
    lib = _lib.load()
    a = torch.empty(plan.packed_floats_bf3 if bf3 else plan.packed_floats, device=w0.device, dtype=torch.float32)
    fn, who = (lib.fst_pack_weights_bf16x3, "fst_pack_weights_bf16x3") if bf3 else (lib.fst_pack_weights, "fst_pack_weights")
    second = (w1, s1)
    if parts is None:
        parts = [(0, -1, 0, M, w0, s0)]
    else:
        second = (None, (0, 0, 0, 0))
    for (g0, g1, row_base, row_end, w, sw) in parts:
        src0 = _wsrc(w, *sw)
        src1 = _wsrc(second[0], *second[1]) if second[0] is not None else None
        check(fn(ptr(plan.dev(w0.device)), plan.host_ptr(), plan.length, ctypes.byref(src0),
                 ctypes.byref(src1) if src1 is not None else None, row_end, g0, g1, row_base, ptr(a), stream_ptr()), who)
    return a


def unpack_weights(plan: Plan, M: int, a: Tensor, dw0: Tensor, s0, dw1: Optional[Tensor] = None, s1=(0, 0, 0, 0)) -> None:
    lib = _lib.load()
    n_slabs = a.size(0) if a.dim() == 2 else 1
    check(lib.fst_unpack_weights(ptr(plan.dev(a.device)), plan.host_ptr(), plan.length, ptr(a), M, ptr(dw0), *s0,
                                 ptr(dw1), *s1, n_slabs, stream_ptr()), "fst_unpack_weights")


def conv_gemm(plan: Plan, a: Tensor, x0: Tensor, x1: Optional[Tensor], bias: Optional[Tensor], B: int, L: int, M: int,
              y: Optional[Tensor], res: Optional[Tensor] = None, y2: Optional[Tensor] = None, msplit: Optional[int] = None,
              nb: int = 1, ksplit: int = 1, flags: int = 0, m2_start: Optional[int] = None, bf3: bool = False) -> None:
    lib = _lib.load()
    if bf3:
        flags |= GEMM_BF16X3
    msplit = M if msplit is None else msplit
    m2_start = msplit if m2_start is None else m2_start
    x0_bs, _ = _ncl(x0, "x0")
    x1_bs = _ncl(x1, "x1")[0] if x1 is not None else 0
    y_bs = _ncl(y, "y")[0] if y is not None else 0
    res_bs = _ncl(res, "res")[0] if res is not None else 0
    y2_bs = _ncl(y2, "y2")[0] if y2 is not None else 0
    t0 = KERNEL_TIMER.begin() if KERNEL_TIMER is not None else None
    check(lib.fst_conv_gemm(ptr(x0), x0_bs, ptr(x1), x1_bs, ptr(a), ptr(plan.dev(x0.device)), plan.host_ptr(),
                            plan.length, ptr(bias), ptr(y), y_bs, ptr(res), res_bs, ptr(y2), y2_bs, msplit, m2_start, B, L,
                            M, nb, ksplit, flags, stream_ptr()), "fst_conv_gemm")
    if t0 is not None:
        key = route_kernel_name(last_route())
        if KERNEL_TIMER.detail:
            key += f" M={M} rec={plan.total_records} dil={plan.dil}"
        rows_in = x0.size(1) + (x1.size(1) if x1 is not None else 0) + (res.size(1) if res is not None else 0)
        rows_out = (msplit if y is not None else 0) + ((M - m2_start) if y2 is not None else 0)
        if y2 is not None and flags & EPI_ACC2:
            rows_in += M - m2_start
        if flags & EPI_ACC1 and y is not None:
            rows_in += msplit
        KERNEL_TIMER.end(key, t0, 2.0 * B * L * _plan_macs_per_step(plan, M), 4.0 * B * L * (rows_in + rows_out))


def conv_wgrad(plan: Plan, x0: Tensor, x1: Optional[Tensor], dy: Tensor, dy2: Optional[Tensor], msplit: int, B: int,
               L: int, M: int, ksplit: int, x0_mul_off: int = 0) -> Tensor:
    lib = _lib.load()
    n_slabs = max(1, min(ksplit, B * ((L + 31) // 32)))
    da = torch.empty(n_slabs, plan.packed_floats, device=x0.device, dtype=torch.float32)
    x0_bs, _ = _ncl(x0, "x0")
    x1_bs = _ncl(x1, "x1")[0] if x1 is not None else 0
    dy_bs, _ = _ncl(dy, "dy")
    dy2_bs = _ncl(dy2, "dy2")[0] if dy2 is not None else 0
    t0 = KERNEL_TIMER.begin() if KERNEL_TIMER is not None else None
    bf3 = MATH == "bf16x3"
    check(lib.fst_conv_wgrad(ptr(x0), x0_bs, ptr(x1), x1_bs, ptr(dy), dy_bs, ptr(dy2), dy2_bs, msplit, ptr(da),
                             ptr(plan.dev(x0.device)), plan.host_ptr(), plan.length, B, L, M, ksplit,
                             (GEMM_BF16X3 if bf3 else 0) | WGRAD_SLABS, x0_mul_off, stream_ptr()),
          "fst_conv_wgrad")
    if t0 is not None:
        key = route_kernel_name(last_route())
        if KERNEL_TIMER.detail:
            key += f" M={M} rec={plan.total_records} ksplit={ksplit}"
        rows_in = x0.size(1) + (x1.size(1) if x1 is not None else 0) + M
        KERNEL_TIMER.end(key, t0, 2.0 * B * L * _plan_macs_per_step(plan, M), 4.0 * B * L * rows_in + 8.0 * plan.packed_floats)
    return da


def row_sum(x: Tensor, out: Optional[Tensor] = None) -> Tensor:
    lib = _lib.load()
    bs, L = _ncl(x, "x")
    B, C = x.size(0), x.size(1)
    if out is None:
        out = torch.empty(C, device=x.device, dtype=torch.float32)
    check(lib.fst_row_sum(ptr(x), bs, B, C, L, ptr(out), stream_ptr()), "fst_row_sum")
    return out


def wgrad_ksplit(B: int, L: int, n_wg_per_slice: int) -> int:
    tiles = B * ((L + 31) // 32)
    target = 384 if n_wg_per_slice == 1 else 512
    k = max(1, target // max(1, n_wg_per_slice))
    if k >= 16:
        k -= k % 8
    return max(1, min(tiles, k))


class ConvSpec:

    def __init__(self, M: int, C0: int, ntaps: int = 1, dil: int = 1, pad_left: int = 0, C1: int = 0,
                 row_live: Optional[Sequence[Tuple[int, int]]] = None, dense_dw: bool = True):
        self.M, self.C0, self.ntaps, self.dil, self.pad_left, self.C1 = M, C0, ntaps, dil, pad_left, C1
        self.row_live = list(row_live) if row_live is not None else None
        self.dense_dw = dense_dw
        self.dense_if_fast = False
        if C1:
            if pad_left % dil or not (0 <= pad_left // dil < ntaps):
                raise ValueError("the 1x1 side input needs a tap with zero offset")
        self.x1_tap = pad_left // dil if C1 else 0
        self._plans: Dict[Tuple[str, int], Plan] = {}
        self.mb = 1 if self.row_live is not None and ntaps > 2 else pick_mb(M)

    def dense_tap_wgrad_ok(self, B: int, L: int, x0: Tensor, dy: Tensor) -> bool:
        if self.C1 or MATH != "bf16x3" or not (self.dense_dw or self.row_live is None or self.dense_if_fast) or self.dil != 1:
            return False
        if not (x0.is_contiguous() and dy.is_contiguous()):
            return False
        if x0.data_ptr() % 16 or dy.data_ptr() % 16 or dy.size(1) != self.M or x0.size(1) != self.C0:
            return False
        return bool(_lib.load().fst_dense_tap_wgrad_ok(B, L, self.M, self.C0, self.ntaps, self.pad_left))

    def tap_wgrad_ok(self, B: int, L: int, x0: Tensor, dy: Tensor) -> bool:
        if self.C1 or MATH != "bf16x3" or not (self.dense_dw or self.row_live is None) or self.ntaps < 2 or self.C0 < 64:
            return False
        if os.environ.get("FST_TAP_WGRAD", "0") != "1" or not (x0.is_contiguous() and dy.is_contiguous()):
            return False
        if x0.data_ptr() % 16 or dy.data_ptr() % 16:
            return False
        served = _lib.load().fst_tap_wgrad_ok(B, L, self.M, self.C0, self.ntaps, self.dil, self.pad_left)
        return served == 1 or (served == 2 and has_slack(x0))

    def _halo(self) -> int:
        return (self.ntaps - 1) * self.dil

    def nb_for(self, B: int, L: int, mb: int, windowed_c: int, halo: int) -> int:
        tiles128 = (L + 127) // 128
        win_bf3 = windowed_c >= 8 and MATH == "bf16x3"
        if win_bf3:
            windowed_c, mb = min(windowed_c, PIPE_C), min(mb, 2)
        best = 1
        for nb in ((4, 2, 1) if windowed_c else (2, 1)):
            if mb * nb > (4 if win_bf3 else 8) or nb > max(1, tiles128):
                continue
            if windowed_c and windowed_c <= 64 and ((windowed_c + 1) & ~1) * (128 * nb + halo) * 4 > LDS_BUDGET:
                continue
            if windowed_c > 64 and nb > 2:
                continue
            best = nb
            if B * ((L + 128 * nb - 1) // (128 * nb)) >= 512:
                break
        return best

    def _fwd_segments(self) -> List[Segment]:
        segs = [Segment(0, self.C0, 0, self.ntaps)]
        if self.C1:
            segs.append(Segment(1, self.C1, self.x1_tap, self.x1_tap + 1))
        return segs

    def _windowed(self, channels: int) -> bool:
        return self.dil == 1 and self.ntaps > 3

    def _chunking(self, channels: int, nb: int, ntaps: int) -> Tuple[int, bool]:
        if not self._windowed(channels):
            return PIPE_C, True
        if MATH == "bf16x3" and channels >= 8:
            return PIPE_C, False
        halo = (ntaps - 1) * self.dil
        cap = (LDS_BUDGET // (4 * (128 * nb + halo))) & ~1
        if channels <= cap:
            return (channels + 1) & ~1, False
        cap = (LDS_MULTI_CHUNK // (4 * (128 * nb + halo))) & ~1
        n = (channels + cap - 1) // cap
        return ((channels + n - 1) // n + 1) & ~1, False

    def fwd_plan(self, nb: int) -> Plan:
        key = ("fwd", nb)
        if key not in self._plans:
            chunk_c, split = self._chunking(max(self.C0, self.C1), nb, self.ntaps)
            mb = min(self.mb, 2) if (chunk_c == PIPE_C and not split) else self.mb
            self._plans[key] = build_plan(self.M, self._fwd_segments(), self.ntaps, self.dil, self.pad_left, MB=mb,
                                          chunk_c=chunk_c, split_taps=split, row_live=self.row_live)
        return self._plans[key]

    def dx0_plan(self, nb: int) -> Plan:
        key = ("dx0", nb)
        if key not in self._plans:
            col_live = None
            if self.row_live is not None:
                col_live = [(self.ntaps - hi, self.ntaps - lo) for lo, hi in self.row_live]
            chunk_c, split = self._chunking(self.M, nb, self.ntaps)
            mb = min(pick_mb(self.C0), 2) if (chunk_c == PIPE_C and not split) else None
            self._plans[key] = build_plan(self.C0, [Segment(0, self.M, 0, self.ntaps, col_live)], self.ntaps, self.dil,
                                          self._halo() - self.pad_left, MB=mb, chunk_c=chunk_c, split_taps=split)
        return self._plans[key]

# ... 578 lines not shown

def wn_wgrad_reduce_many(slabs: list, B: int, L: int, n: int, h: int) -> None:
    lib = _lib.load()
    for c0 in range(0, len(slabs), WN_WGRAD_MAX_REDUCE):
        chunk = slabs[c0: c0 + WN_WGRAD_MAX_REDUCE]
        ne = len(chunk)
        ints = lambda vals: (ctypes.c_int32 * ne)(*[int(v) for v in vals])
        check(lib.fst_wn_wgrad_reduce_many(ints(e[0] for e in chunk), ints(e[1] for e in chunk), ints(e[2] for e in chunk),
                                           _ptr_table([e[3] for e in chunk]), (ctypes.c_int64 * ne)(*[e[3].numel() for e in chunk]),
                                           _ptr_table([e[4] for e in chunk]), _ptr_table([e[5] for e in chunk]), ne, B, L, n, h,
                                           stream_ptr()), "fst_wn_wgrad_reduce_many")
    del slabs[:]


def _tap_wgrad(who: str, taps_name: str, timer_key: str, dy: Tensor, x: Tensor, dw: Tensor, M: int, C: int, taps: int, *geometry) -> None:
    lib = _lib.load()
    B, _, L = dy.shape
    if tuple(dy.shape) != (B, M, L) or tuple(x.shape) != (B, C, L) or not (dy.is_contiguous() and x.is_contiguous()):
        raise ValueError(f"{who}: dy {tuple(dy.shape)} / x {tuple(x.shape)} must be contiguous [B, {M}, L] / [B, {C}, L]")
    if tuple(dw.shape) != (M, C, taps) or not dw.is_contiguous() or dw.dtype != torch.float32:
        raise ValueError(f"{who}: gradient target of shape {tuple(dw.shape)}, expected contiguous {(M, C, taps)}")
    ws_n = getattr(lib, f"fst_{who}_workspace_floats")(B, L, M, C, taps)
    if ws_n <= 0:
        raise ValueError(f"{who}: unsupported shape B={B} L={L} M={M} C={C} {taps_name}={taps}")
    ws = torch.empty(ws_n, device=dy.device, dtype=torch.float32)
    t0 = KERNEL_TIMER.begin() if KERNEL_TIMER is not None else None
    check(getattr(lib, f"fst_{who}")(ptr(dy), ptr(x), ptr(dw), ptr(ws), ws_n, B, L, M, C, taps, *geometry, dy.numel(), x.numel(),
                                     stream_ptr()), f"fst_{who}")
    if t0 is not None:
        KERNEL_TIMER.end(timer_key, t0, 2.0 * B * L * M * C * taps, 4.0 * B * L * (M + C))


def dense_tap_wgrad(dy: Tensor, x: Tensor, dw: Tensor, M: int, C: int, K: int, pad_left: int) -> None:
    _tap_wgrad("dense_tap_wgrad", "K", f"tz_wgrad_kernel M={M} C={C} bf3", dy, x, dw, M, C, K, pad_left)


def tap_wgrad(dy: Tensor, x: Tensor, dw: Tensor, M: int, C: int, ntaps: int, dil: int, pad_left: int) -> None:
    _tap_wgrad("tap_wgrad", "ntaps", "tap_wgrad (wn_wgrad_kernel<2, 3>) bf3", dy, x, dw, M, C, ntaps, dil, pad_left, int(has_slack(x)))


def _ptr_sets(ts: Sequence[Tensor]):
    arr = (ctypes.c_void_p * len(ts))()
    for i, t in enumerate(ts):
        if t.dtype != torch.float32 or not t.is_cuda:
            raise ValueError("operand sets must be fp32 device tensors")
        arr[i] = t.data_ptr()
    return arr


class WNGradPool:

    def __init__(self):
        self.pending: dict = {}
        self.task = None

    def add(self, key, operands) -> None:
        task = torch._C._current_graph_task_id()
        if task != self.task:
            self.pending, self.task = {}, task
        self.pending.setdefault(key, []).append(operands)

    def take(self) -> dict:
        pending, self.pending = self.pending, {}
        return pending if self.task == torch._C._current_graph_task_id() else {}


class WGradJoinFn(torch.autograd.Function):

    @staticmethod
    def forward(ctx, pool: WNGradPool, specs: "WNSpecs", flat: Tensor):
        ctx.pool, ctx.specs = pool, specs
        return flat.view_as(flat)

    @staticmethod
    def backward(ctx, g):
        S, pool = ctx.specs, ctx.pool
        pending = pool.take()
        if not pending:
            return None, None, g
        g = g.contiguous()
        nl, n, h = S.n_layers, S.n, S.h
        dw = S.unflatten(g)
        g_cond_w, g_in_w, g_rs_w = dw[2], dw[6: 6 + nl], dw[6 + 2 * nl: 6 + 3 * nl]
        slabs, later = {}, []
        for (kind, i), sets in pending.items():
            groups = {}
            for s in sets:
                lead = s[0] if kind == 0 else s[1]
                shape = (lead.size(0), lead.size(2)) + ((s[2].stride(0),) if kind == 0 else ())
                groups.setdefault(shape, []).append(s)
            own = True
            for shape, members in groups.items():
                for c0 in range(0, len(members), WN_WGRAD_MAX_SETS):
                    chunk = members[c0: c0 + WN_WGRAD_MAX_SETS]
                    cols = [list(col) for col in zip(*chunk)]
                    to = None if c0 else slabs.setdefault(shape[:2], [])
                    if kind == 0:
                        t_in, t_cond = g_in_w[i], g_cond_w[2 * n * i: 2 * n * (i + 1)]
                        if not own:
                            t_in, t_cond = torch.empty_like(t_in), torch.empty_like(t_cond)
                            later += [(g_in_w[i], t_in), (g_cond_w[2 * n * i: 2 * n * (i + 1)], t_cond)]
                        wn_wgrad_in(cols[0], cols[1], cols[2], t_in, t_cond, n, h, 2 ** i, slabs=to)
                    else:
                        last = i == nl - 1
                        t_rs = g_rs_w[i]
                        if not own:
                            t_rs = torch.empty_like(t_rs)
                            later.append((g_rs_w[i], t_rs))
                        wn_wgrad_rs(None if last else cols[0], cols[1], cols[2], t_rs, last, n, slabs=to)
                    own = False
        for (B, L), entries in slabs.items():
            wn_wgrad_reduce_many(entries, B, L, n, h)
        for seg, t in later:
            seg.add_(t)
        return None, None, g


class WNFoldPlan:

    def __init__(self, specs: "WNSpecs", normed: Sequence[bool]):
        assert len(normed) == len(specs.shapes)
        self.specs, self.normed = specs, list(normed)
        self._key, self._table = None, None
        self.n_rows = sum(sh[0] if nm else 1 for sh, nm in zip(specs.shapes, normed))
        self.grad_offsets, off = [], 0
        for sh, nm in zip(specs.shapes, normed):
            numel = int(math.prod(sh))
            self.grad_offsets.append(off)
            off += numel
            if nm:
                self.grad_offsets.append(off)
                off += sh[0]
        self.grad_numel = off

    def n_inputs(self) -> int:
        return len(self.grad_offsets)

    def table(self, tensors: Sequence[Tensor]) -> Tensor:
        import numpy as np
        key = tuple(t.data_ptr() for t in tensors) + (str(tensors[0].device),)
        if key == self._key:
            return self._table
        rows, it, gi = [], iter(tensors), 0
        for i, (sh, nm) in enumerate(zip(self.specs.shapes, self.normed)):
            dst, numel = self.specs.offsets[i], int(math.prod(sh))
            if nm:
                v, g = next(it), next(it)
                M, rowlen = sh[0], numel // sh[0]
                assert v.is_contiguous() and g.is_contiguous() and tuple(v.shape) == tuple(sh) and g.numel() == M
                m = np.arange(M, dtype=np.int64)
                blk = np.stack([v.data_ptr() + 4 * rowlen * m, g.data_ptr() + 4 * m, dst + rowlen * m, np.full(M, rowlen, np.int64),
                                self.grad_offsets[gi] + rowlen * m, self.grad_offsets[gi + 1] + m], axis=1)
                gi += 2
            else:
                t = next(it)
                assert t.is_contiguous() and t.numel() == numel
                blk = np.array([[t.data_ptr(), 0, dst, numel, self.grad_offsets[gi], 0]], dtype=np.int64)
                gi += 1
            rows.append(blk)
        tab = np.concatenate(rows, axis=0)
        assert tab.shape == (self.n_rows, 6)
        self._table = torch.from_numpy(tab).to(tensors[0].device)
        self._key = key
        return self._table


class WNFoldFn(torch.autograd.Function):

    @staticmethod
    def forward(ctx, plan: WNFoldPlan, *tensors: Tensor):
        lib = _lib.load()
        assert len(tensors) == plan.n_inputs()
        for t in tensors:
            _lib.require_gpu_tensor(t, "WN parameter")
        tab = plan.table(tensors)
        dev = tensors[0].device
        flat = torch.empty(plan.specs.flat_numel, device=dev, dtype=torch.float32)
        norms = torch.empty(plan.n_rows, device=dev, dtype=torch.float32)
        check(lib.fst_wn_fold_fwd(ptr(tab), plan.n_rows, ptr(flat), ptr(norms), stream_ptr()), "fst_wn_fold_fwd")
        ctx.plan, ctx.tab = plan, tab
        ctx.shapes = [tuple(t.shape) for t in tensors]
        ctx.save_for_backward(norms)
        return flat

    @staticmethod
    def backward(ctx, d_flat):
        lib = _lib.load()
        (norms,) = ctx.saved_tensors
        plan: WNFoldPlan = ctx.plan
        d_flat = d_flat.contiguous()
        dpar = torch.empty(plan.grad_numel, device=d_flat.device, dtype=torch.float32)
        check(lib.fst_wn_fold_bwd(ptr(ctx.tab), plan.n_rows, ptr(d_flat), ptr(norms), ptr(dpar), stream_ptr()), "fst_wn_fold_bwd")
        grads = []
        for off, sh in zip(plan.grad_offsets, ctx.shapes):
            grads.append(dpar[off: off + int(math.prod(sh))].view(sh))
        return (None, *grads)


def wn_fused_ok(n: int, h: int, L: int, *tensors: Tensor, kernel: int = 3) -> bool:
    if MATH != "bf16x3" or kernel != 3 or not (0 < n < 128) or L % 4 != 0 or os.environ.get("FST_WN_FUSED", "1") == "0":
        return False
    return all(t.data_ptr() % 16 == 0 and t.stride(0) % 4 == 0 for t in tensors)


WN_PACK_MAX_LAYERS = 10


class _WnImages(NamedTuple):
    nl: int
    key: Callable
    nbytes: Callable
    sources: Callable
    one: Optional[Callable]
    stack: Callable


def _pack_one(f: _WnImages, i: int) -> Tensor:
    if _PACK_CACHE is not None:
        hit = _PACK_CACHE.get(f.key(i))
        if hit is not None:
            return hit[0]
    src = [t.contiguous() for t in f.sources(i)]
    img = torch.empty(f.nbytes(i) // 4, device=src[0].device, dtype=torch.float32)
    f.one(i, src, img)
    if _PACK_CACHE is not None:
        _PACK_CACHE[f.key(i)] = (img, *f.sources(i), src)
    return img


def _pack_stack(f: _WnImages) -> List[Tensor]:
    hits = [None if _PACK_CACHE is None else _PACK_CACHE.get(f.key(i)) for i in range(f.nl)]
    if _PACK_CACHE is not None and all(hit is not None for hit in hits):
        return [hit[0] for hit in hits]
    if f.one is not None and (f.nl > WN_PACK_MAX_LAYERS or any(hit is not None for hit in hits)):
        return [_pack_one(f, i) for i in range(f.nl)]
    srcs = [[t.contiguous() for t in f.sources(i)] for i in range(f.nl)]
    imgs = [torch.empty(f.nbytes(i) // 4, device=srcs[i][0].device, dtype=torch.float32) for i in range(f.nl)]
    f.stack(srcs, imgs)
    if _PACK_CACHE is not None:
        for i, img in enumerate(imgs):
            _PACK_CACHE[f.key(i)] = (img, *f.sources(i), srcs[i])
    return imgs


def _wn_fwd_images(who: str, layers: Sequence[Sequence[Tensor]], lasts: Sequence[bool], n: int, h: int) -> _WnImages:
    lib, nl = _lib.load(), len(layers)
    for in_w in (l[0] for l in layers):
        if in_w.dim() != 3 or in_w.size(0) != 2 * n or in_w.size(1) != n:
            raise ValueError(f"{who}: in_w must be [2n, n, taps], got {tuple(in_w.shape)} for n={n}")
    nbytes = lib.fst_wn_image_bytes(n, h)
    return _WnImages(
        nl, lambda i: ("wn", n, h, lasts[i]) + tuple((t.data_ptr(), t._version) for t in layers[i]), lambda i: nbytes,
        lambda i: layers[i],
        lambda i, src, img: check(lib.fst_wn_pack(*[ptr(t) for t in src], n, h, layers[i][0].size(2), int(lasts[i]), ptr(img), nbytes,
                                                  stream_ptr()), "fst_wn_pack"),
        lambda srcs, imgs: check(lib.fst_wn_pack_stack(*[_ptr_table([l[j] for l in srcs]) for j in range(6)], nl, n, h,
                                                       layers[0][0].size(2), _ptr_table(imgs), nbytes, stream_ptr()),
                                 "fst_wn_pack_stack"))


def wn_pack_layer(in_w: Tensor, cond_w: Tensor, in_b: Tensor, cond_b: Tensor, rs_w: Tensor, rs_b: Tensor, n: int, h: int,
                  last: bool) -> Tensor:
    return _pack_one(_wn_fwd_images("wn_pack_layer", [(in_w, cond_w, in_b, cond_b, rs_w, rs_b)], [last], n, h), 0)


def wn_pack_layers(layers: Sequence[Sequence[Tensor]], n: int, h: int) -> List[Tensor]:
    nl = len(layers)
    return _pack_stack(_wn_fwd_images("wn_pack_layers", layers, [i == nl - 1 for i in range(nl)], n, h))


def _wn_bwd_images(rs_ws: Sequence[Tensor], lasts: Sequence[bool], n: int, acc_order: bool) -> _WnImages:
    lib, nl = _lib.load(), len(rs_ws)
    nbytes = lambda i: lib.fst_wn_bwd_image_bytes(n, int(lasts[i]))
    return _WnImages(
        nl, lambda i: ("wn_bwd", n, lasts[i], acc_order, rs_ws[i].data_ptr(), rs_ws[i]._version), nbytes, lambda i: (rs_ws[i],),
        lambda i, src, img: check(lib.fst_wn_pack_bwd(ptr(src[0]), n, int(lasts[i]), int(acc_order), ptr(img), nbytes(i), stream_ptr()),
                                  "fst_wn_pack_bwd"),
        lambda srcs, imgs: check(lib.fst_wn_pack_bwd_stack(_ptr_table([s_[0] for s_ in srcs]), nl, n, int(acc_order), _ptr_table(imgs),
                                                           lib.fst_wn_bwd_image_bytes(n, 0), stream_ptr()), "fst_wn_pack_bwd_stack"))


def wn_pack_bwd(rs_w: Tensor, n: int, last: bool, acc_order: bool = False) -> Tensor:
    return _pack_one(_wn_bwd_images([rs_w], [last], n, acc_order), 0)


def wn_pack_bwd_layers(rs_ws: Sequence[Tensor], n: int, acc_order: bool = False) -> List[Tensor]:
    nl = len(rs_ws)
    return _pack_stack(_wn_bwd_images(rs_ws, [i == nl - 1 for i in range(nl)], n, acc_order))


def wn_pack_bwd_proj_layers(rs_ws: Sequence[Tensor], end_w: Tensor, n: int) -> List[Tensor]:
    lib, nl, h2 = _lib.load(), len(rs_ws), end_w.size(0)
    if nl > WN_PACK_MAX_LAYERS or tuple(end_w.shape) != (h2, n, 1) or h2 > 64:
        raise ValueError(f"wn_pack_bwd_proj_layers: {nl} layers, end_w {tuple(end_w.shape)} (at most {WN_PACK_MAX_LAYERS} layers, "
                         f"end_w [2h <= 64, n = {n}, 1])")
    return _pack_stack(_WnImages(
        nl, lambda i: ("wn_bwd_proj", n, h2, i == nl - 1, rs_ws[i].data_ptr(), rs_ws[i]._version, end_w.data_ptr(), end_w._version),
        lambda i: lib.fst_wn_bwd_proj_image_bytes(n, h2, int(i == nl - 1)), lambda i: (rs_ws[i], end_w), None,
        lambda srcs, imgs: check(lib.fst_wn_pack_bwd_proj_stack(_ptr_table([s_[0] for s_ in srcs]), ptr(srcs[0][1]), nl, n, h2,
                                                                _ptr_table(imgs), lib.fst_wn_bwd_proj_image_bytes(n, h2, 0),
                                                                stream_ptr()), "fst_wn_pack_bwd_proj_stack")))


def _wn_dgrad_images(in_ws: Sequence[Tensor], cond_ws: Sequence[Tensor], n: int, h: int) -> _WnImages:
    lib, nl = _lib.load(), len(in_ws)
    nbytes = lib.fst_wn_dgrad_image_bytes(n)
    return _WnImages(
        nl, lambda i: ("wn_dgrad", n, h, in_ws[i].data_ptr(), in_ws[i]._version, cond_ws[i].data_ptr(), cond_ws[i]._version),
        lambda i: nbytes, lambda i: (in_ws[i], cond_ws[i]),
        lambda i, src, img: check(lib.fst_wn_pack_dgrad(ptr(src[0]), ptr(src[1]), n, h, in_ws[i].size(2), ptr(img), nbytes, stream_ptr()),
                                  "fst_wn_pack_dgrad"),
        lambda srcs, imgs: check(lib.fst_wn_pack_dgrad_stack(_ptr_table([s_[0] for s_ in srcs]), _ptr_table([s_[1] for s_ in srcs]), nl, n,
                                                             h, in_ws[0].size(2), _ptr_table(imgs), nbytes, stream_ptr()),
                                 "fst_wn_pack_dgrad_stack"))


def wn_pack_dgrad(in_w: Tensor, cond_w: Tensor, n: int, h: int) -> Tensor:
    return _pack_one(_wn_dgrad_images([in_w], [cond_w], n, h), 0)


def wn_pack_dgrad_layers(in_ws: Sequence[Tensor], cond_ws: Sequence[Tensor], n: int, h: int) -> List[Tensor]:
    return _pack_stack(_wn_dgrad_images(in_ws, cond_ws, n, h))


def _wn_layer_forward(save: bool, a: Tensor, u0: Tensor, img: Tensor, ts: Optional[Tensor], acts: Optional[Tensor],
                      a_next: Optional[Tensor], out: Tensor, first: bool, last: bool, n: int, h: int, dil: int) -> None:
    lib = _lib.load()
    a_bs, L = _ncl(a, "a")
    u0_bs, _ = _ncl(u0, "u0")
    B = a.size(0)
    numel = _same_numel(a, out, acts, a_next)
    if save and (ts.numel() != 2 * numel or not ts.is_contiguous()):
        raise ValueError("wn_layer_fwd: ts must be the contiguous [B, 2n, L] partner of a")
    if save:
        fn, who, key, saved = lib.fst_wn_layer_fwd, "fst_wn_layer_fwd", "wn_layer_fwd_kernel", (ptr(ts), ptr(acts))
    else:
        fn, who, key, saved = lib.fst_wn_layer_infer, "fst_wn_layer_infer", "wn_layer_infer_kernel", ()
    t0 = KERNEL_TIMER.begin() if KERNEL_TIMER is not None else None
    check(fn(ptr(a), a_bs, ptr(u0), u0_bs, ptr(img), img.numel() * 4, *saved, ptr(a_next), ptr(out), int(first), int(last), B, L, n, h,
             dil, numel, stream_ptr()), who)
    if t0 is not None:
        rs_rows = n if last else 2 * n
        flops = 2.0 * B * L * (2 * n * (3 * n + h) + rs_rows * n)
        rows = n + h + (0 if first else n) + (0 if last else n) + n
        rows += (2 * n if save else 0) + (n if acts is not None else 0)
        KERNEL_TIMER.end(key, t0, flops, 4.0 * B * L * rows)


def wn_layer_fwd(a: Tensor, u0: Tensor, img: Tensor, ts: Tensor, acts: Optional[Tensor], a_next: Optional[Tensor], out: Tensor,
                 first: bool, last: bool, n: int, h: int, dil: int) -> None:
    _wn_layer_forward(True, a, u0, img, ts, acts, a_next, out, first, last, n, h, dil)


def wn_layer_infer(a: Tensor, u0: Tensor, img: Tensor, a_next: Optional[Tensor], out: Tensor, first: bool, last: bool, n: int, h: int,
                   dil: int) -> None:
    _wn_layer_forward(False, a, u0, img, None, None, a_next, out, first, last, n, h, dil)


def wn_bwd_partials(n_layers: int, B: int, L: int, device) -> Tensor:
    return torch.empty(n_layers, 256, B * ((L + 127) // 128), device=device, dtype=torch.float32)


def wn_layer_bwd(d_a: Optional[Tensor], d_out: Tensor, ts: Tensor, img: Tensor, dg: Tensor, last: bool, n: int,
                 want_row_sums: bool = False, sums_out: Optional[Tensor] = None, part: Optional[Tensor] = None) -> Optional[Tensor]:
    lib = _lib.load()
    B, _, L = d_out.shape
    deferred = part is not None
    if part is None and want_row_sums:
        part = torch.empty(256, B * ((L + 127) // 128), device=dg.device, dtype=torch.float32)
    numel = _same_numel(d_out, d_a)
    for t in (ts, dg):
        if t.numel() != 2 * numel or not t.is_contiguous():
            raise ValueError("wn_layer_bwd: ts / dg must be contiguous [B, 2n, L]")
    if part is not None and (part.shape != (256, B * ((L + 127) // 128)) or not part.is_contiguous()):
        raise ValueError(f"wn_layer_bwd: partial-sum slab of shape {tuple(part.shape)}")
    t0 = KERNEL_TIMER.begin() if KERNEL_TIMER is not None else None
    check(lib.fst_wn_layer_bwd(ptr(d_a), ptr(d_out), ptr(ts), ptr(img), img.numel() * 4, ptr(dg), ptr(part),
                               0 if part is None else part.size(1), int(last), B, L, n, numel, stream_ptr()), "fst_wn_layer_bwd")
    if t0 is not None:
        k = n if last else 2 * n
        KERNEL_TIMER.end("wn_layer_bwd_kernel", t0, 2.0 * B * L * n * k, 4.0 * B * L * (k + 4 * n))
    if part is None or deferred:
        return None
    if sums_out is not None:
        return torch.sum(part[: 2 * n], dim=1, out=sums_out)
    return part.sum(dim=1)[: 2 * n]


WN_DGRAD_TILE = 512


def wn_dgrad_ok(n: int, h: int, dil: int) -> bool:
    return bool(_lib.load().fst_wn_dgrad_fits(n, h, dil))


def wn_dgrad_partials(n_layers: int, B: int, L: int, device) -> Tensor:
    return torch.empty(n_layers, 128, B * ((L + WN_DGRAD_TILE - 1) // WN_DGRAD_TILE), device=device, dtype=torch.float32)


def wn_layer_dgrad(dg: Tensor, img: Tensor, d_a: Optional[Tensor], d_u0: Tensor, n: int, h: int, dil: int,
                   want_row_sums: bool = False, sums_out: Optional[Tensor] = None, part: Optional[Tensor] = None):
    lib = _lib.load()
    B, _, L = dg.shape
    deferred = part is not None
    if part is None and want_row_sums:
        part = torch.empty(128, B * ((L + WN_DGRAD_TILE - 1) // WN_DGRAD_TILE), device=dg.device, dtype=torch.float32)
    d_a_new = torch.empty(B, n, L, device=dg.device, dtype=torch.float32)
    numel = _same_numel(d_a_new, d_a)
    if dg.numel() != 2 * numel or not dg.is_contiguous():
        raise ValueError("wn_layer_dgrad: dg must be contiguous [B, 2n, L]")
    d_u0_bs, _ = _ncl(d_u0, "d_u0")
    if tuple(d_u0.shape) != (B, h, L):
        raise ValueError(f"wn_layer_dgrad: d_u0 must be [B, h, L] = {(B, h, L)}, got {tuple(d_u0.shape)}")
    if part is not None and (part.shape != (128, B * ((L + WN_DGRAD_TILE - 1) // WN_DGRAD_TILE)) or not part.is_contiguous()):
        raise ValueError(f"wn_layer_dgrad: partial-sum slab of shape {tuple(part.shape)}")
    t0 = KERNEL_TIMER.begin() if KERNEL_TIMER is not None else None
    check(lib.fst_wn_layer_dgrad(ptr(dg), ptr(img), img.numel() * 4, ptr(d_a), ptr(d_a_new), ptr(d_u0), ptr(part),
                                 0 if part is None else part.size(1), B, L, n, h, dil, numel, d_u0_bs, stream_ptr()),
          "fst_wn_layer_dgrad")
    if t0 is not None:
        KERNEL_TIMER.end("wn_layer_dgrad_kernel", t0, 2.0 * B * L * 2 * n * (3 * n + h),
                         4.0 * B * L * (2 * n + (n if d_a is not None else 0) + n + 2 * h))
    if part is None:
        return d_a_new
    if deferred:
        return d_a_new, None
    if sums_out is not None:
        return d_a_new, torch.sum(part[:n], dim=1, out=sums_out)
    return d_a_new, part.sum(dim=1)[:n]


def wn_skip_proj_ok(h: int, need_w: bool) -> bool:
    mode = os.environ.get("FST_WN_SKIP_PROJ", "1")
    return 2 * h <= 64 and (mode == "2" or (mode != "0" and _PARTIAL_BACKWARD and not need_w))


def wn_stack_bwd_ok(n: int, h: int, L: int, nl: int) -> bool:
    if os.environ.get("FST_WN_STACK", "1") == "0":
        return False
    return bool(_lib.load().fst_wn_stack_bwd_ok(n, h, L, nl))


def wn_stack_fwd_ok(n: int, h: int, L: int, nl: int, B: int) -> bool:
    if os.environ.get("FST_WN_STACK_FWD", "1") == "0":
        return False
    lib = _lib.load()
    return bool(lib.fst_wn_stack_fwd_ok(n, h, L, nl)) and B * (L // 256) >= 2 * 256 and B >= 256


def _wn_stack_forward(save: bool, a_list: Sequence[Tensor], u0: Tensor, imgs: Sequence[Tensor], ts_list: Sequence[Tensor], out: Tensor,
                      n: int, h: int) -> None:
    lib = _lib.load()
    nl = len(imgs)
    B, L = u0.size(0), u0.size(2)
    u0_bs, _ = _ncl(u0, "u0")
    numel = _same_numel(out, *a_list)
    bs = (ctypes.c_int64 * nl)(*[_ncl(a, "a")[0] for a in a_list])
    for ts in ts_list:
        if ts.numel() != 2 * numel or not ts.is_contiguous():
            raise ValueError("wn_stack_fwd: every ts must be the contiguous [B, 2n, L] partner of a")
    if save:
        fn, who, key, saved = lib.fst_wn_stack_fwd, "fst_wn_stack_fwd", "wn_stack_fwd_kernel", (_ptr_table(ts_list),)
    else:
        fn, who, key, saved = lib.fst_wn_stack_infer, "fst_wn_stack_infer", "wn_stack_infer_kernel", ()
    t0 = KERNEL_TIMER.begin() if KERNEL_TIMER is not None else None
    check(fn(_ptr_table(a_list), bs, _ptr_table(imgs), imgs[0].numel() * 4, *saved, _ptr_table(list(a_list[1:]) + [None]), ptr(u0), u0_bs,
             ptr(out), nl, B, L, n, h, numel, stream_ptr()), who)
    if t0 is not None:
        flops = 2.0 * B * L * (nl * 2 * n * (3 * n + h) + (2 * nl - 1) * n * n)
        rows = nl * (n + h) + (nl - 1) * (n + 2 * n) + n
        rows += nl * 2 * n if save else 0
        KERNEL_TIMER.end(key, t0, flops, 4.0 * B * L * rows)


def wn_stack_fwd(a_list: Sequence[Tensor], u0: Tensor, imgs: Sequence[Tensor], ts_list: Sequence[Tensor], out: Tensor, n: int,
                 h: int) -> None:
    _wn_stack_forward(True, a_list, u0, imgs, ts_list, out, n, h)


def wn_stack_infer(a_list: Sequence[Tensor], u0: Tensor, imgs: Sequence[Tensor], out: Tensor, n: int, h: int) -> None:
    _wn_stack_forward(False, a_list, u0, imgs, (), out, n, h)


def _ptr_table(ts: Sequence[Optional[Tensor]]):
    arr = (ctypes.c_void_p * len(ts))()
    for i, t in enumerate(ts):
        arr[i] = None if t is None else t.data_ptr()
    return arr


def wn_stack_bwd(ts_list: Sequence[Tensor], imgs_b: Sequence[Tensor], imgs_d: Sequence[Tensor], dgs: Sequence[Tensor],
                 da_out: Sequence[Optional[Tensor]], d_out: Optional[Tensor], d_u0: Tensor, n: int, h: int,
                 part_b: Optional[Tensor] = None, part_d: Optional[Tensor] = None, do: Optional[Tensor] = None) -> None:
    lib = _lib.load()
    nl = len(ts_list)
    if (do is None) == (d_out is None):
        raise ValueError("wn_stack_bwd: d_out or do, one of them")
    if do is not None:
        if do.dim() != 3 or not do.is_contiguous() or do.dtype != torch.float32:
            raise ValueError("wn_stack_bwd: do must be a contiguous fp32 [B, 2h, L]")
        B, h2, L = do.shape
        numel = _same_numel(*[t for t in da_out if t is not None])
        if numel != B * n * L:
            raise ValueError(f"wn_stack_bwd: da_out must be [B, n, L] = {(B, n, L)}")
    else:
        B, _, L = d_out.shape
        numel = _same_numel(d_out, *[t for t in da_out if t is not None])
    for t in list(ts_list) + list(dgs):
        if t.numel() != 2 * numel or not t.is_contiguous():
            raise ValueError("wn_stack_bwd: ts / dg must be contiguous [B, 2n, L]")
    d_u0_bs, _ = _ncl(d_u0, "d_u0")
    if tuple(d_u0.shape) != (B, h, L):
        raise ValueError(f"wn_stack_bwd: d_u0 must be [B, h, L] = {(B, h, L)}, got {tuple(d_u0.shape)}")
    if (part_b is None) != (part_d is None):
        raise ValueError("wn_stack_bwd: row sums of both kinds or of neither")
    if part_b is not None and (tuple(part_b.shape) != (nl, 256, B) or tuple(part_d.shape) != (nl, 128, B)
                               or not (part_b.is_contiguous() and part_d.is_contiguous())):
        raise ValueError("wn_stack_bwd: row-sum slabs must be contiguous [nl, 256, B] and [nl, 128, B]")
    t0 = KERNEL_TIMER.begin() if KERNEL_TIMER is not None else None
    rs_b = None if part_b is None else _ptr_table([part_b[i] for i in range(nl)])
    rs_d = None if part_d is None else _ptr_table([part_d[i] for i in range(nl)])
    if do is not None:
        check(lib.fst_wn_stack_bwd_proj(_ptr_table(ts_list), _ptr_table(imgs_b), _ptr_table(imgs_d), _ptr_table(dgs),
                                        _ptr_table(da_out), rs_b, rs_d, ptr(do), h2, do.numel(), ptr(d_u0), d_u0_bs, nl, B, L, n, h,
                                        numel, stream_ptr()), "fst_wn_stack_bwd_proj")
    else:
        check(lib.fst_wn_stack_bwd(_ptr_table(ts_list), _ptr_table(imgs_b), _ptr_table(imgs_d), _ptr_table(dgs), _ptr_table(da_out),
                                   rs_b, rs_d, ptr(d_out), ptr(d_u0), d_u0_bs, nl, B, L, n, h, numel, stream_ptr()),
              "fst_wn_stack_bwd")
    if t0 is not None:
        sr = n if do is None else h2
        flops = 2.0 * B * L * (n * ((n + sr) * nl - n) + nl * 2 * n * (3 * n + h))
        rows = nl * (2 * n + sr + 2 * 2 * n + 2 * h) + n * sum(t is not None for t in da_out)
        KERNEL_TIMER.end("wn_stack_bwd_kernel", t0, flops, 4.0 * B * L * rows)


def _wn_layer(S: WNSpecs, ts: Sequence[Tensor], i: int):
    n, nl = S.n, S.n_layers
    rows = slice(2 * n * i, 2 * n * (i + 1))
    return ts[6 + i], ts[2][rows], ts[6 + nl + i], ts[3][rows], ts[6 + 2 * nl + i], ts[6 + 3 * nl + i]


def wn_infer_enabled() -> bool:
    return os.environ.get("FST_WN_INFER", "1") != "0"


def _wn_forward(specs: WNSpecs, u0: Tensor, flat: Tensor, save: bool = True):
    S, nl, n, h = specs, specs.n_layers, specs.n, specs.h
    flat = flat.contiguous()
    W = S.unflatten(flat)
    B, _, L = u0.shape
    dev = u0.device
    infer = not save and wn_infer_enabled()
    y0 = torch.empty(B, n, L, device=dev, dtype=torch.float32) if infer else empty_with_slack(B, n, L, dev)
    a = S.start.forward(u0, None, W[0], None, W[1], y=y0)
    fused = wn_fused_ok(n, h, L, a, u0, kernel=S.kernel)
    if fused:
        out = torch.empty(B, n, L, device=dev, dtype=torch.float32)
        imgs = wn_pack_layers([_wn_layer(S, W, i) for i in range(nl)], n, h)
        if infer:
            other = torch.empty_like(a) if nl > 1 else None
            a_list, ts_list = [a if i % 2 == 0 else other for i in range(nl)], None
        else:
            a_list = [a] + [empty_with_slack(B, n, L, dev) for _ in range(nl - 1)]
            ts_list = [torch.empty(B, 2 * n, L, device=dev, dtype=torch.float32) for _ in range(nl)]
        if wn_stack_fwd_ok(n, h, L, nl, B):
            _wn_stack_forward(not infer, a_list, u0, imgs, ts_list or (), out, n, h)
        else:
            for i in range(nl):
                last = i == nl - 1
                _wn_layer_forward(not infer, a_list[i], u0, imgs[i], ts_list[i] if ts_list else None, None,
                                  None if last else a_list[i + 1], out, i == 0, last, n, h, 2 ** i)
        if infer:
            return S.end.forward(out, None, W[4], None, W[5]), True, ()
        acts_list = ts_list
    else:
        lib = _lib.load()
        out = torch.zeros(B, n, L, device=dev, dtype=torch.float32)
        bias_g = torch.stack(W[6 + nl: 6 + 2 * nl]) + W[3].view(nl, 2 * n)
        a_list, ts_list, acts_list = [a], [], []
        for i in range(nl):
            in_w, cond_w, _, _, rs_w, rs_b = _wn_layer(S, W, i)
            g = S.ins[i].forward(a, u0, in_w, cond_w, bias_g[i])
            acts = torch.empty(B, n, L, device=dev, dtype=torch.float32)
            check(lib.fst_gate_fwd(ptr(g), ptr(acts), B, n, L, _gate_numel(acts, g), stream_ptr()), "fst_gate_fwd")
            ts_list.append(g)
            acts_list.append(acts)
            if i < nl - 1:
                a_next = torch.empty_like(a)
                S.rs[i].forward(acts, None, rs_w, None, rs_b, y=a_next, res=a, y2=out, msplit=n, flags=EPI_ACC2)
                a = a_next
                a_list.append(a)
            else:
                S.rs[i].forward(acts, None, rs_w, None, rs_b, y=None, y2=out, msplit=0, flags=EPI_ACC2)
    o = S.end.forward(out, None, W[4], None, W[5])
    return o, fused, (u0, out, *a_list, *ts_list, *acts_list, flat)


def _wn_backward(S: WNSpecs, fused: bool, sv, do: Tensor, d_u0: Tensor, need_w: bool, pool: Optional["WNGradPool"] = None):
    nl, h, n = S.n_layers, S.h, S.n
    u0, out, flat = sv[0], sv[1], sv[2 + 3 * nl]
    a_list, ts_list, acts_list = sv[2: 2 + nl], sv[2 + nl: 2 + 2 * nl], sv[2 + 2 * nl: 2 + 3 * nl]
    W = S.unflatten(flat)
    B, _, L = u0.shape
    deferring = need_w and pool is not None and fused and any(
        wn_wgrad_ok(0, B, L, n, h, 2 ** i, a_list[i]) or wn_wgrad_ok(1, B, L, n, h, 2 ** i) for i in range(nl))
    d_flat = (torch.zeros_like(flat) if deferring else torch.empty_like(flat)) if need_w else None
    G = S.unflatten(d_flat) if need_w else None
    do = do.contiguous()

    stack = fused and all(wn_dgrad_ok(n, h, 2 ** i) for i in range(nl)) and wn_stack_bwd_ok(n, h, L, nl)
    proj = stack and wn_skip_proj_ok(h, need_w)
    d_out = None if proj and not need_w else S.end.grad_x0(do, W[4])
    da_sums = None
    if need_w:
        S.end.grad_w(out, None, do, out0=G[4])
        row_sum(do, out=G[5])
        d_out_sum = row_sum(d_out, out=G[6 + 4 * nl - 1])
        o0 = S.offsets[6 + 3 * nl]
        d_rs_b = d_flat[o0: o0 + (nl - 1) * 2 * n].view(nl - 1, 2 * n)
        d_rs_b[:, n:] = d_out_sum
        da_sums = [G[1]] + [d_rs_b[i, :n] for i in range(nl - 1)]
    part_b = part_d = None
    if not fused:
        d_a = _wn_backward_unfused(S, W, G, a_list, ts_list, acts_list, u0, d_out, d_u0, da_sums)
    elif stack:
        d_a, part_b, part_d = _wn_backward_stack(S, W, G, a_list, ts_list, u0, d_out, d_u0, pool, do if proj else None)
    else:
        d_a, part_b, part_d = _wn_backward_layers(S, W, G, a_list, ts_list, u0, d_out, d_u0, da_sums, pool)
    S.start.grad_x0(d_a, W[0], out=d_u0, flags=EPI_ACC1)
    if need_w:
        S.start.grad_w(u0, None, d_a, out0=G[0])
        o0 = S.offsets[6 + nl]
        if part_b is not None:
            torch.sum(part_b[:, : 2 * n, :], dim=2, out=d_flat[o0: o0 + nl * 2 * n].view(nl, 2 * n))
        if part_d is not None:
            if nl > 1:
                torch.sum(part_d[1:, :n, :], dim=2, out=d_rs_b[:, :n])
            torch.sum(part_d[0, :n, :], dim=1, out=G[1])
        G[3].copy_(d_flat[o0: o0 + nl * 2 * n])
    return d_flat


def _wn_wgrad_rs(S: WNSpecs, i: int, d_a: Optional[Tensor], d_out: Tensor, ts: Tensor, G, pool) -> None:
    n, B, L, last, g_rs_w = S.n, d_out.size(0), d_out.size(2), i == S.n_layers - 1, _wn_layer(S, G, i)[4]
    if wn_wgrad_ok(1, B, L, n, S.h, 2 ** i):
        if pool is not None:
            pool.add((1, i), (d_a, d_out, ts))
        else:
            wn_wgrad_rs(d_a, d_out, ts, g_rs_w, last, n)
    elif last:
        S.rs[i].grad_w(ts[:, :n], None, d_out, x0_mul_off=n * L, out0=g_rs_w)
    else:
        S.rs[i].grad_w(ts[:, :n], None, d_a, d_out, msplit=n, x0_mul_off=n * L, out0=g_rs_w)


def _wn_wgrad_in(S: WNSpecs, i: int, dg: Tensor, a: Tensor, u0: Tensor, G, pool) -> None:
    n, h, B, L = S.n, S.h, dg.size(0), dg.size(2)
    g_in_w, g_cond_w = _wn_layer(S, G, i)[:2]
    if wn_wgrad_ok(0, B, L, n, h, 2 ** i, a):
        if pool is not None:
            pool.add((0, i), (dg, a, u0))
        else:
            wn_wgrad_in(dg, a, u0, g_in_w, g_cond_w, n, h, 2 ** i)
    else:
        S.ins[i].grad_w(a, u0, dg, out0=g_in_w, out1=g_cond_w)


def _wn_backward_stack(S: WNSpecs, W, G, a_list, ts_list, u0: Tensor, d_out: Optional[Tensor], d_u0: Tensor, pool,
                       do: Optional[Tensor] = None):
    nl, n, h = S.n_layers, S.n, S.h
    B, _, L = u0.shape
    rs_ws = [_wn_layer(S, W, i)[4] for i in range(nl)]
    imgs_b = wn_pack_bwd_layers(rs_ws, n, acc_order=True) if do is None else wn_pack_bwd_proj_layers(rs_ws, W[4], n)
    imgs_d = wn_pack_dgrad_layers([_wn_layer(S, W, i)[0] for i in range(nl)], [_wn_layer(S, W, i)[1] for i in range(nl)], n, h)
    new = lambda *shape: torch.empty(*shape, device=u0.device, dtype=torch.float32)
    if G is None:
        dgs, da_out = [new(B, 2 * n, L)] * nl, [new(B, n, L)] + [None] * (nl - 1)
        part_b = part_d = None
    else:
        dgs, da_out = [new(B, 2 * n, L) for _ in range(nl)], [new(B, n, L) for _ in range(nl)]
        part_b, part_d = new(nl, 256, B), new(nl, 128, B)
    wn_stack_bwd(ts_list, imgs_b, imgs_d, dgs, da_out, d_out if do is None else None, d_u0, n, h, part_b, part_d, do)
    if G is not None:
        for i in range(nl):
            _wn_wgrad_rs(S, i, da_out[i + 1] if i + 1 < nl else None, d_out, ts_list[i], G, pool)
            _wn_wgrad_in(S, i, dgs[i], a_list[i], u0, G, pool)
    return da_out[0], part_b, part_d


def _wn_backward_layers(S: WNSpecs, W, G, a_list, ts_list, u0: Tensor, d_out: Tensor, d_u0: Tensor, da_sums, pool):
    nl, n, h = S.n_layers, S.n, S.h
    B, _, L = d_out.shape
    dev = d_out.device
    fused_dg = [wn_dgrad_ok(n, h, 2 ** i) for i in range(nl)]
    part_b = wn_bwd_partials(nl, B, L, dev) if G is not None else None
    part_d = wn_dgrad_partials(nl, B, L, dev) if G is not None and all(fused_dg) else None
    d_a = None
    for i in reversed(range(nl)):
        last = i == nl - 1
        in_w, cond_w, _, _, rs_w, _ = _wn_layer(S, W, i)
        if G is not None:
            _wn_wgrad_rs(S, i, d_a, d_out, ts_list[i], G, pool)
        dg = torch.empty(B, 2 * n, L, device=dev, dtype=torch.float32)
        wn_layer_bwd(d_a, d_out, ts_list[i], wn_pack_bwd(rs_w, n, last), dg, last, n, part=None if part_b is None else part_b[i])
        if G is not None:
            _wn_wgrad_in(S, i, dg, a_list[i], u0, G, pool)
        if not fused_dg[i]:
            d_a = S.ins[i].grad_x01(dg, in_w, cond_w, d_a, d_u0)
            if G is not None:
                row_sum(d_a, out=da_sums[i])
        elif G is None:
            d_a = wn_layer_dgrad(dg, wn_pack_dgrad(in_w, cond_w, n, h), d_a, d_u0, n, h, 2 ** i)
        else:
            d_a = wn_layer_dgrad(dg, wn_pack_dgrad(in_w, cond_w, n, h), d_a, d_u0, n, h, 2 ** i, want_row_sums=True,
                                 sums_out=da_sums[i], part=None if part_d is None else part_d[i])[0]
    return d_a, part_b, part_d


def _wn_backward_unfused(S: WNSpecs, W, G, a_list, g_list, acts_list, u0: Tensor, d_out: Tensor, d_u0: Tensor, da_sums) -> Tensor:
    lib = _lib.load()
    nl, n = S.n_layers, S.n
    B, _, L = d_out.shape
    d_a = None
    for i in reversed(range(nl)):
        last = i == nl - 1
        in_w, cond_w, _, _, rs_w, _ = _wn_layer(S, W, i)
        dacts = torch.empty(B, n, L, device=d_out.device, dtype=torch.float32)
        plan = S.rs_T_last if last else S.rs_T
        bf3 = bf3_ok(plan, L)
        a_pk = pack_weights(plan, n, rs_w, (0, 1, n, 0), *(() if last else (rs_w, (n * n, 1, n, 0))), bf3=bf3)
        conv_gemm(plan, a_pk, d_out if last else d_a, None if last else d_out, None, B, L, n, dacts,
                  nb=S.start.nb_for(B, L, pick_mb(n), 0, 0), bf3=bf3)
        if G is not None:
            g_in_w, g_cond_w, g_in_b, _, g_rs_w, _ = _wn_layer(S, G, i)
            if last:
                S.rs[i].grad_w(acts_list[i], None, d_out, out0=g_rs_w)
            else:
                S.rs[i].grad_w(acts_list[i], None, d_a, d_out, msplit=n, out0=g_rs_w)
        dg = torch.empty(B, 2 * n, L, device=d_out.device, dtype=torch.float32)
        check(lib.fst_gate_bwd(ptr(g_list[i]), ptr(dacts), ptr(dg), B, n, L, _gate_numel(dacts, dg, g_list[i]), stream_ptr()),
              "fst_gate_bwd")
        if G is not None:
            S.ins[i].grad_w(a_list[i], u0, dg, out0=g_in_w, out1=g_cond_w)
            row_sum(dg, out=g_in_b)
        d_a = S.ins[i].grad_x01(dg, in_w, cond_w, d_a, d_u0)
        if G is not None:
            row_sum(d_a, out=da_sums[i])
    return d_a


class WNFn(torch.autograd.Function):

    @staticmethod
    def forward(ctx, specs: WNSpecs, u0: Tensor, flat: Tensor):
        o, fused, saved = _wn_forward(specs, u0, flat, save=any(ctx.needs_input_grad))
        ctx.specs, ctx.fused = specs, fused
        if saved:
            ctx.save_for_backward(*saved)
        return o

    @staticmethod
    def backward(ctx, do):
        u0 = ctx.saved_tensors[0]
        d_u0 = torch.zeros(u0.size(0), ctx.specs.h, u0.size(2), device=u0.device, dtype=torch.float32)
        d_flat = _wn_backward(ctx.specs, ctx.fused, ctx.saved_tensors, do, d_u0, ctx.needs_input_grad[2] and _want_weight_grad())
        return None, (d_u0 if ctx.needs_input_grad[1] else None), d_flat


def _coupling_forward(u: Tensor, o: Tensor):
    lib = _lib.load()
    B, C, L = u.shape
    xn = torch.empty_like(u)
    part = torch.empty(lib.fst_coupling_sum_slots(B, C // 2, L), 2, device=u.device, dtype=torch.float32)
    check(lib.fst_coupling_fwd(ptr(u), ptr(o), ptr(xn), B, C // 2, L, _same_numel(u, o, xn), ptr(part), stream_ptr()),
          "fst_coupling_fwd")
    sums = part.sum(dim=0)
    return xn, sums[0], sums[1]


def _scalar_f32(g: Optional[Tensor]) -> Optional[Tensor]:
    return None if g is None else g.contiguous().float()


def _coupling_backward(u: Tensor, o: Tensor, dxn: Optional[Tensor], g_ls: Optional[Tensor], g_sq: Optional[Tensor]):
    lib = _lib.load()
    B, C, L = u.shape
    if dxn is None and g_ls is None and g_sq is None:
        return torch.zeros_like(u), torch.zeros_like(o)
    du, d_o = torch.empty_like(u), torch.empty_like(o)
    dxn = None if dxn is None else dxn.contiguous()
    g_ls, g_sq = _scalar_f32(g_ls), _scalar_f32(g_sq)
    check(lib.fst_coupling_bwd(ptr(u), ptr(o), ptr(dxn), None, ptr(g_ls), ptr(g_sq), ptr(du), ptr(d_o), B, C // 2, L,
                               _same_numel(u, o, dxn, du, d_o), stream_ptr()), "fst_coupling_bwd")
    return du, d_o


class CouplingFn(torch.autograd.Function):

    @staticmethod
    def forward(ctx, u, o):
        u, o = u.contiguous(), o.contiguous()
        ctx.save_for_backward(u, o)
        ctx.set_materialize_grads(False)
        return _coupling_forward(u, o)

    @staticmethod
    def backward(ctx, dxn, g_ls, g_sq):
        u, o = ctx.saved_tensors
        return _coupling_backward(u, o, dxn, g_ls, g_sq)


class FlowFn(torch.autograd.Function):

    @staticmethod
    def forward(ctx, specs: WNSpecs, x: Tensor, flat: Tensor, inverse: bool, pool: Optional[WNGradPool] = None):
        lib = _lib.load()
        ctx.pool = pool
        x = x.contiguous()
        h = specs.h
        assert x.size(1) == 2 * h
        o, fused, saved = _wn_forward(specs, x[:, :h], flat, save=any(ctx.needs_input_grad))
        B, C, L = x.shape
        if inverse:
            xn = torch.empty_like(x)
            check(lib.fst_coupling_inv_fwd(ptr(x), ptr(o), ptr(xn), B, h, L, _same_numel(x, o, xn), stream_ptr()), "fst_coupling_inv_fwd")
            s_ls = s_sq = None
            keep = xn
        else:
            xn, s_ls, s_sq = _coupling_forward(x, o)
            keep = x
        ctx.specs, ctx.fused, ctx.inverse = specs, fused, inverse
        if saved:
            ctx.save_for_backward(keep, o, *saved)
        ctx.set_materialize_grads(False)
        return xn, o, s_ls, s_sq

    @staticmethod
    def backward(ctx, dxn, d_o_ext, g_ls, g_sq):
        lib = _lib.load()
        keep, o = ctx.saved_tensors[0], ctx.saved_tensors[1]
        sv = ctx.saved_tensors[2:]
        S: WNSpecs = ctx.specs
        B, C, L = keep.shape
        if ctx.inverse:
            if dxn is None:
                dx, d_o = torch.zeros_like(keep), torch.zeros_like(o)
            else:
                dx, d_o = torch.empty_like(keep), torch.empty_like(o)
                dxn = dxn.contiguous()
                check(lib.fst_coupling_inv_bwd(ptr(keep), ptr(o), ptr(dxn), ptr(dx), ptr(d_o), B, S.h, L,
                                               _same_numel(keep, o, dxn, dx, d_o), stream_ptr()), "fst_coupling_inv_bwd")
        else:
            dx, d_o = _coupling_backward(keep, o, dxn, g_ls, g_sq)
        if d_o_ext is not None:
            d_o = d_o + d_o_ext
        need_w = ctx.needs_input_grad[2] and _want_weight_grad()
        d_flat = _wn_backward(S, ctx.fused, sv, d_o, dx[:, : S.h], need_w, ctx.pool)
        return None, (dx if ctx.needs_input_grad[1] else None), d_flat, None, None


class CouplingInvFn(torch.autograd.Function):

    @staticmethod
    def forward(ctx, x, o):
        lib = _lib.load()
        x, o = x.contiguous(), o.contiguous()
        B, C, L = x.shape
        xn = torch.empty_like(x)
        check(lib.fst_coupling_inv_fwd(ptr(x), ptr(o), ptr(xn), B, C // 2, L, _same_numel(x, o, xn), stream_ptr()),
              "fst_coupling_inv_fwd")
        ctx.save_for_backward(xn, o)
        return xn

    @staticmethod
    def backward(ctx, dxn):
        lib = _lib.load()
        xn, o = ctx.saved_tensors
        B, C, L = xn.shape
        dx, d_o = torch.empty_like(xn), torch.empty_like(o)
        dxn = dxn.contiguous()
        check(lib.fst_coupling_inv_bwd(ptr(xn), ptr(o), ptr(dxn), ptr(dx), ptr(d_o), B, C // 2, L,
                                       _same_numel(xn, o, dxn, dx, d_o), stream_ptr()), "fst_coupling_inv_bwd")
        return dx, d_o


NT_SLICES = 32


def _scalar_arg(r):
    if isinstance(r, Tensor):
        if r.dtype != torch.float32 or not r.is_cuda or r.numel() != 1:
            raise ValueError("a device ratio must be one fp32 element")
        return ptr(r), 0.0
    return None, float(r)


class NoiseTransferFn(torch.autograd.Function):

    @staticmethod
    def forward(ctx, z_t, z_s, W, bias, avg_t, avg_s, r_t, r_s):
        lib = _lib.load()
        z_t, z_s = z_t.contiguous(), z_s.contiguous()
        B, C, L = z_s.shape
        N = C * L
        if z_t.shape[1:] != z_s.shape[1:] or tuple(avg_t.shape) != (C, L) or tuple(avg_s.shape) != (C, L) or N % 4:
            raise ValueError(f"NoiseTransferFn: z_t {tuple(z_t.shape)}, z_s {tuple(z_s.shape)}, state {tuple(avg_t.shape)} (C·L % 4 == 0)")
        if not (avg_t.is_contiguous() and avg_s.is_contiguous()):
            raise ValueError("NoiseTransferFn: the running sums must be contiguous (they are updated in place)")
        W2 = W.reshape(C, C).contiguous()
        bias = bias.contiguous()
        if z_t.size(0) != B:
            raise ValueError("NoiseTransferFn: the two batches must be equally large (the caller uses the ATen composition otherwise)")
        dev = z_s.device
        S = min(NT_SLICES, B)
        part = torch.empty(2, S, N, device=dev, dtype=torch.float32)
        check(lib.fst_batch_sum(ptr(z_t), ptr(z_s), ptr(part), B, N, S, stream_ptr()), "fst_batch_sum")
        maps = torch.empty(3, C, L, device=dev, dtype=torch.float32)
        (pt, ft), (ps, fs) = _scalar_arg(r_t), _scalar_arg(r_s)
        check(lib.fst_noise_transfer_fwd(ptr(part), S, B, pt, ps, ft, fs, ptr(avg_t), ptr(avg_s), ptr(W2), ptr(bias), ptr(maps[0]),
                                         ptr(maps[1]), ptr(maps[2]), C, L, stream_ptr()), "fst_noise_transfer_fwd")
        out = torch.empty_like(z_s)
        check(lib.fst_bcast_add(ptr(out), ptr(z_s), ptr(maps[2]), B, N, stream_ptr()), "fst_bcast_add")
        ctx.save_for_backward(maps, W2, *[r for r in (r_t, r_s) if isinstance(r, Tensor)])
        ctx.ratios = (r_t if not isinstance(r_t, Tensor) else None, r_s if not isinstance(r_s, Tensor) else None)
        ctx.w_shape, ctx.B = W.shape, B
        return out

    @staticmethod
    def backward(ctx, g):
        lib = _lib.load()
        maps, W2 = ctx.saved_tensors[0], ctx.saved_tensors[1]
        extra = list(ctx.saved_tensors[2:])
        r_t = ctx.ratios[0] if ctx.ratios[0] is not None else extra.pop(0)
        r_s = ctx.ratios[1] if ctx.ratios[1] is not None else extra.pop(0)
        g = g.contiguous()
        B, C, L = g.shape
        N = C * L
        dev = g.device
        S = min(NT_SLICES, B)
        part = torch.empty(S, N, device=dev, dtype=torch.float32)
        check(lib.fst_batch_sum(ptr(g), None, ptr(part), B, N, S, stream_ptr()), "fst_batch_sum")
        small = torch.empty(2, C, L, device=dev, dtype=torch.float32)
        check(lib.fst_noise_transfer_bwd(ptr(part), S, ptr(maps[1]), ptr(W2), ptr(small[0]), ptr(small[1]), C, L, stream_ptr()),
              "fst_noise_transfer_bwd")
        dW = db = None
        if ctx.needs_input_grad[2] or ctx.needs_input_grad[3]:
            dW = torch.empty(C, C, device=dev, dtype=torch.float32)
            db = torch.empty(C, device=dev, dtype=torch.float32)
            check(lib.fst_noise_transfer_dw(ptr(small[0]), ptr(maps[0]), ptr(dW), ptr(db), C, L, stream_ptr()), "fst_noise_transfer_dw")
            dW = dW.view(ctx.w_shape)
        dz_t = torch.empty_like(g) if ctx.needs_input_grad[0] else None
        dz_s = torch.empty_like(g) if ctx.needs_input_grad[1] else None
        if dz_t is not None or dz_s is not None:
            (pt, ft), (ps, fs) = _scalar_arg(r_t), _scalar_arg(r_s)
            check(lib.fst_noise_transfer_bwd_apply(ptr(g), ptr(small[1]), pt, ps, ft, fs, B, ptr(dz_t), ptr(dz_s), N, stream_ptr()),
                  "fst_noise_transfer_bwd_apply")
        return dz_t, dz_s, dW, db, None, None, None, None


class LogDetFn(torch.autograd.Function):

    @staticmethod
    def forward(ctx, W: Tensor):
        lib = _lib.load()
        _lib.require_gpu_tensor(W, "W")
        W = W.contiguous()
        n = W.size(0)
        assert W.dim() == 2 and W.size(1) == n and W.dtype == torch.float32
        out = torch.empty(2, device=W.device, dtype=torch.float32)
        inv_t = torch.empty_like(W)
        check(lib.fst_logdet_inv(ptr(W), n, ptr(out), ptr(inv_t), stream_ptr()), "fst_logdet_inv")
        ctx.save_for_backward(inv_t)
        return out[0]

    @staticmethod
    def backward(ctx, g):
        (inv_t,) = ctx.saved_tensors
        return g * inv_t


def logdet(W: Tensor) -> Tensor:
    if W.is_cuda and W.dim() == 2 and W.size(0) <= 96 and W.dtype == torch.float32:
        return LogDetFn.apply(W)
    return torch.logdet(W)

# ... 218 lines not shown
```

### include/fst_hip.h

```cpp
#ifndef FST_HIP_H
#define FST_HIP_H

#include <stdint.h>

#ifdef __cplusplus
extern "C" {
#endif

#define FST_ABI_VERSION 21

int fst_version(void);
const char* fst_last_error(void);

#define FST_PLAN_HEADER 16

typedef struct {
  const float* w;
  int64_t off0, sm, sc, st;
} fst_wsrc;

int fst_pack_weights(const int32_t* plan_dev, const int32_t* plan_host, int plan_len,
                     const fst_wsrc* src0_host, const fst_wsrc* src1_host,
                     int M, int g_begin, int g_end , int row_base ,
                     float* a_packed, void* stream);

int fst_pack_weights_bf16x3(const int32_t* plan_dev, const int32_t* plan_host, int plan_len,
                            const fst_wsrc* src0_host, const fst_wsrc* src1_host,
                            int M, int g_begin, int g_end, int row_base, void* a_image, void* stream);

int fst_unpack_weights(const int32_t* plan_dev, const int32_t* plan_host, int plan_len,
                       const float* a_packed, int M,
                       float* dw0, int64_t off0_0, int64_t sm0, int64_t sc0, int64_t st0,
                       float* dw1, int64_t off0_1, int64_t sm1, int64_t sc1, int64_t st1,
                       int n_slabs ,
                       void* stream);

int fst_mask_taps(float* w, const int32_t* live_lo, const int32_t* live_hi, int M, int C, int K, void* stream);

#define FST_EPI_RELU    1
#define FST_EPI_ACC2    2
#define FST_EPI_ATOMIC  4
#define FST_EPI_ACC1    8
#define FST_GEMM_BF16X3 16
#define FST_WGRAD_SLABS 32
int fst_conv_gemm(const float* x0, int64_t x0_bs, const float* x1, int64_t x1_bs,
                  const float* a_packed, const int32_t* plan_dev, const int32_t* plan_host, int plan_len,
                  const float* bias,
                  float* y, int64_t y_bs, const float* res, int64_t res_bs,
                  float* y2, int64_t y2_bs, int msplit, int m2_start ,
                  int B, int L, int M, int nb_cfg, int ksplit, int flags, void* stream);

int fst_conv_wgrad(const float* x0, int64_t x0_bs, const float* x1, int64_t x1_bs,
                   const float* dy, int64_t dy_bs, const float* dy2, int64_t dy2_bs, int msplit,
                   float* da_packed, const int32_t* plan_dev, const int32_t* plan_host, int plan_len,
                   int B, int L, int M, int ksplit, int flags , int64_t x0_mul_off, void* stream);

#define FST_ROUTE_GEMM      1
#define FST_ROUTE_PIPE      2
#define FST_ROUTE_BF3       3
#define FST_ROUTE_WIN_BF3   4
#define FST_ROUTE_WIN_ROWS  5
#define FST_ROUTE_WGRAD     6
#define FST_ROUTE_EPI_PLAIN   0
#define FST_ROUTE_EPI_ADD     1
#define FST_ROUTE_EPI_ATOMIC  2
#define FST_ROUTE_EPI_VEC     3
#define FST_ROUTE_EPI_VEC_ADD 4
int fst_conv_last_route(int32_t out[8]);

int fst_row_sum(const float* x, int64_t x_bs, int B, int C, int L, float* out, void* stream);

#define FST_BN_SLOTS 16
int fst_bn_stats(const float* y, int B, int C, int L, float* part , int64_t numel, void* stream);
int fst_bn_finalize(const float* part, int n_slots, const float* gamma, const float* beta,
                    float* running_mean, float* running_var, int train, int C, float eps, float momentum,
                    float* stats, void* stream);
int fst_bn_apply(const float* y, const float* stats, const float* res, const float* res_stats,
                 float* out, int B, int C, int L, int relu, int64_t numel, void* stream);
int fst_bn_bwd_reduce(const float* dy, const float* y, const float* out, const float* stats,
                      int B, int C, int L, int relu, float* red , int64_t numel, void* stream);
int fst_bn_bwd_apply(const float* dy, const float* y, const float* out, const float* stats, const float* red, int n_slots,
                     float* red_out, float* dx, float* row_sums, int B, int C, int L, int relu, int train, int B_total,
                     int64_t numel, void* stream);
int fst_bn_bwd_reduce_join(const float* dy, const float* ya, const float* yb, const float* stats_a, const float* stats_b,
                           int B, int C, int L, float* red_a, float* red_b, int64_t numel, void* stream);
int fst_bn_bwd_apply_join(const float* dy, const float* ya, const float* yb, const float* stats_a, const float* stats_b,
                          const float* red_a, const float* red_b, int n_slots, float* red_out_a, float* red_out_b,
                          float* dxa, float* dxb, float* row_sums_a, float* row_sums_b, int B, int C, int L, int train,
                          int B_total, int64_t numel, void* stream);

int fst_gate_fwd(float* g_ts, float* acts, int B, int n, int L, int64_t numel_acts, void* stream);
int fst_gate_bwd(const float* ts, const float* dacts, float* dg, int B, int n, int L, int64_t numel_acts, void* stream);
int64_t fst_coupling_sum_slots(int B, int h, int L);
int fst_coupling_fwd(const float* u, const float* o, float* xn, int B, int h, int L, int64_t numel, float* sums, void* stream);
int fst_coupling_bwd(const float* u, const float* o, const float* dxn, const float* dlogs, const float* g_ls, const float* g_sq,
                     float* du, float* d_o, int B, int h, int L, int64_t numel, void* stream);
int fst_coupling_inv_fwd(const float* x, const float* o, float* xn, int B, int h, int L, int64_t numel, void* stream);
int fst_coupling_inv_bwd(const float* xn, const float* o, const float* dxn,
                         float* dx, float* d_o, int B, int h, int L, int64_t numel, void* stream);

int fst_wn_fold_fwd(const int64_t* table_dev, int n_rows, float* flat, float* norms , void* stream);
int fst_wn_fold_bwd(const int64_t* table_dev, int n_rows, const float* d_flat, const float* norms, float* dpar, void* stream);

int fst_logdet_inv(const float* W, int n, float* out , float* inv_t , void* stream);

int64_t fst_wn_image_bytes(int n, int h);
int fst_wn_pack(const float* in_w, const float* cond_w, const float* in_b, const float* cond_b,
                const float* rs_w, const float* rs_b, int n, int h, int ntaps , int last, void* image, int64_t image_bytes, void* stream);
int fst_wn_pack_stack(const float* const* in_w, const float* const* cond_w, const float* const* in_b, const float* const* cond_b,
                      const float* const* rs_w, const float* const* rs_b, int nl, int n, int h, int ntaps, void* const* images,
                      int64_t image_bytes, void* stream);
int fst_wn_pack_bwd_stack(const float* const* rs_w, int nl, int n, int acc_order, void* const* images, int64_t image_bytes,
                          void* stream);
int fst_wn_pack_dgrad_stack(const float* const* in_w, const float* const* cond_w, int nl, int n, int h, int ntaps,
                            void* const* images, int64_t image_bytes, void* stream);
int64_t fst_wn_bwd_proj_image_bytes(int n, int h2, int last);
int fst_wn_pack_bwd_proj_stack(const float* const* rs_w, const float* end_w, int nl, int n, int h2, void* const* images,
                               int64_t image_bytes, void* stream);
int fst_wn_layer_fwd(const float* a, int64_t a_bs, const float* u0, int64_t u0_bs, const void* image, int64_t image_bytes,
                     float* ts, float* acts, float* a_next, float* out, int first, int last,
                     int B, int L, int n, int h, int dil, int64_t numel_a, void* stream);

int64_t fst_wn_bwd_image_bytes(int n, int last);
int fst_wn_pack_bwd(const float* rs_w, int n, int last,
                    int acc_order ,
                    void* image, int64_t image_bytes, void* stream);
int fst_wn_layer_bwd(const float* d_a_next , const float* d_out, const float* ts, const void* image,
                     int64_t image_bytes, float* dg,
                     float* row_sums ,
                     int64_t row_sums_rows, int last, int B, int L, int n, int64_t numel_a, void* stream);

int64_t fst_wn_dgrad_image_bytes(int n);
int fst_wn_pack_dgrad(const float* in_w, const float* cond_w, int n, int h, int ntaps , void* image,
                      int64_t image_bytes, void* stream);
int fst_wn_dgrad_fits(int n, int h, int dil);
int fst_wn_layer_dgrad(const float* dg, const void* image, int64_t image_bytes, const float* d_a, float* d_a_new, float* d_u0,
                       float* row_sums , int64_t row_sums_rows,
                       int B, int L, int n, int h, int dil, int64_t numel_a, int64_t d_u0_bs, void* stream);

int fst_wn_stack_fwd_ok(int n, int h, int L, int nl);
int fst_wn_stack_fwd(const float* const* a_in, const int64_t* a_bs, const void* const* images, int64_t image_bytes, float* const* ts,
                     float* const* a_next, const float* u0, int64_t u0_bs, float* out, int nl, int B, int L, int n, int h,
                     int64_t numel_a, void* stream);

int fst_wn_layer_infer(const float* a, int64_t a_bs, const float* u0, int64_t u0_bs, const void* image, int64_t image_bytes,
                       float* a_next, float* out, int first, int last, int B, int L, int n, int h, int dil, int64_t numel_a,
                       void* stream);
int fst_wn_stack_infer(const float* const* a_in, const int64_t* a_bs, const void* const* images, int64_t image_bytes,
                       float* const* a_next, const float* u0, int64_t u0_bs, float* out, int nl, int B, int L, int n, int h,
                       int64_t numel_a, void* stream);

int fst_wn_stack_bwd_ok(int n, int h, int L, int nl);
int fst_wn_stack_bwd(const float* const* ts, const void* const* img_b, const void* const* img_d, float* const* dg,
                     float* const* da_out, float* const* rs_b , float* const* rs_d ,
                     const float* d_out, float* d_u0, int64_t d_u0_bs, int nl, int B, int L, int n, int h, int64_t numel_a,
                     void* stream);
int fst_wn_stack_bwd_proj(const float* const* ts, const void* const* img_b, const void* const* img_d, float* const* dg,
                          float* const* da_out, float* const* rs_b , float* const* rs_d ,
                          const float* d_o, int h2, int64_t numel_o, float* d_u0, int64_t d_u0_bs, int nl, int B, int L, int n,
                          int h, int64_t numel_a, void* stream);

int fst_wn_wgrad_ok(int kind, int B, int L, int n, int h, int dil);
int64_t fst_wn_wgrad_workspace_floats(int kind, int B, int L, int n, int h, int last);
int fst_wn_wgrad_in(const float* const* dg, const float* const* a, const float* const* u0, int n_sets, int64_t u0_bs, float* dw_in,
                    float* dw_cond, float* workspace, int64_t workspace_floats, int B, int L, int n, int h, int dil, int a_slack,
                    int64_t numel_a, void* stream);
int fst_wn_wgrad_rs(const float* const* d_a , const float* const* d_out, const float* const* ts, int n_sets,
                    float* dw_rs, float* workspace, int64_t workspace_floats, int last, int B, int L, int n, int64_t numel_a,
                    void* stream);
int fst_wn_wgrad_in_slabs(const float* const* dg, const float* const* a, const float* const* u0, int n_sets, int64_t u0_bs,
                          float* workspace, int64_t workspace_floats, int B, int L, int n, int h, int dil, int a_slack,
                          int64_t numel_a, void* stream);
int fst_wn_wgrad_rs_slabs(const float* const* d_a , const float* const* d_out, const float* const* ts, int n_sets,
                          float* workspace, int64_t workspace_floats, int last, int B, int L, int n, int64_t numel_a, void* stream);
int fst_wn_wgrad_reduce_many(const int32_t* kind, const int32_t* last, const int32_t* n_sets, float* const* workspace,
                             const int64_t* workspace_floats, float* const* dw0, float* const* dw1, int n_entries, int B, int L,
                             int n, int h, void* stream);

int64_t fst_nt_gemm_workspace_floats(int M, int N, int K);
int fst_nt_gemm(const float* A, const float* Bm, float* C, float* workspace, int64_t workspace_floats, int M, int N, int K,
                const float* epi_p , const float* epi_r1 , int epi_ncls, float epi_scale,
                float* epi_raw , void* stream);

int fst_tap_wgrad_ok(int B, int L, int M, int C, int ntaps, int dil, int pad_left);
int64_t fst_tap_wgrad_workspace_floats(int B, int L, int M, int C, int ntaps);
int fst_tap_wgrad(const float* dy, const float* x, float* dw , float* workspace, int64_t workspace_floats,
                  int B, int L, int M, int C, int ntaps, int dil, int pad_left, int x_slack, int64_t numel_dy, int64_t numel_x,
                  void* stream);

int fst_dense_tap_wgrad_ok(int B, int L, int M, int C, int K, int pad_left);
int64_t fst_dense_tap_wgrad_workspace_floats(int B, int L, int M, int C, int K);
int fst_dense_tap_wgrad(const float* dy, const float* x, float* dw , float* workspace, int64_t workspace_floats,
                        int B, int L, int M, int C, int K, int pad_left, int64_t numel_dy, int64_t numel_x, void* stream);

#define FST_WN_ROUTE_LEN         12
#define FST_WN_ROUTE_WGRAD       1
#define FST_WN_ROUTE_TZ          2
#define FST_WN_ROUTE_LAYER_FWD   3
#define FST_WN_ROUTE_STACK_FWD   4
#define FST_WN_ROUTE_LAYER_BWD   5
#define FST_WN_ROUTE_LAYER_DGRAD 6
#define FST_WN_ROUTE_STACK_BWD   7
#define FST_WN_ROUTE_LAYER_INFER 8
#define FST_WN_ROUTE_STACK_INFER 9
int fst_wn_last_route(int32_t out[FST_WN_ROUTE_LEN]);

int fst_batch_sum(const float* x0, const float* x1, float* part, int B, int64_t N, int S, void* stream);
int fst_noise_transfer_fwd(const float* part, int S, int B, const float* r_t_dev, const float* r_s_dev, float r_t, float r_s,
                           float* avg_t, float* avg_s, const float* W, const float* bias, float* dist, float* pre, float* learned,
                           int C, int L, void* stream);
int fst_bcast_add(float* out, const float* x, const float* v, int B, int64_t N, void* stream);
int fst_noise_transfer_bwd(const float* part, int S, const float* pre, const float* W, float* dpre, float* dd, int C, int L,
                           void* stream);
int fst_noise_transfer_dw(const float* dpre, const float* dist, float* dW, float* dbias, int C, int L, void* stream);
int fst_noise_transfer_bwd_apply(const float* g, const float* dd, const float* r_t_dev, const float* r_s_dev, float r_t, float r_s,
                                 int B, float* dz_t, float* dz_s, int64_t N, void* stream);

int fst_relu_bwd(const float* dy, const float* y, float* out, int64_t n, void* stream);

#define FST_ACT_NONE  0
#define FST_ACT_RELU  1
#define FST_ACT_LEAKY 2
int64_t fst_gemm_workspace_floats(int M, int N, int K);
int fst_gemm(const float* A, int64_t lda, int ta, const float* B, int64_t ldb, int tb, float* C, int64_t ldc, int M, int N, int K,
             const float* bias, int act, float slope, float* workspace, int64_t workspace_floats, void* stream);
int64_t fst_gemm_f32_workspace_floats(int M, int N, int K);
int fst_gemm_f32(const float* A, int64_t lda, int ta, const float* B, int64_t ldb, int tb, float* C, int64_t ldc, int M, int N, int K,
                 const float* bias, int act, float slope, float* workspace, int64_t workspace_floats, void* stream);
int fst_act_bwd(const float* dy, const float* y, float* out, int64_t n, float slope, void* stream);
int fst_axpy(float* y, const float* x, float alpha, int64_t n, void* stream);
int fst_add_slices(float* dst, int64_t dst_bs, const float* a, int64_t a_bs, const float* b, int64_t b_bs,
                   int B, int C, int L, void* stream);

int64_t fst_cpc_workspace_floats(int T, int B, int C, int Bc);
int64_t fst_cpc_nce_slots(int T, int B, int C, int Bc);
int fst_cpc_nce_fwd(const float* enc, int64_t s_i, int64_t s_b, int64_t s_c, const int32_t* t0_dev ,
                    const float* pred , int T, int B, int C,
                    int Bc , int col_off ,
                    float* lse , float* nce_sum , float* workspace ,
                    void* stream);
int fst_cpc_nce_bwd(const float* enc, int64_t s_i, int64_t s_b, int64_t s_c, const int32_t* t0_dev ,
                    const float* pred, const float* lse, int T, int B, int C, int Bc, int col_off, const float* gout,
                    float* denc , float* dpred , void* stream);

int fst_gru_fwd(const float* xproj, const float* w_hh, const float* b_hh, float* h_all, float* gates,
                const int32_t* t_last_dev, int t_last, int B, int S, int H, int64_t numel_h, void* stream);
int fst_gru_bwd(const float* w_hh, const float* h_all, const float* gates, const float* dout,
                const int32_t* t_last_dev, int t_last, float* dxproj, float* dgh, int B, int S, int H,
                int64_t numel_h, void* stream);

int fst_lstm2_fwd(const float* xproj, const float* w_hh_t, float* h2, float* save, int B, int H, int64_t numel_xproj, void* stream);
int fst_lstm2_bwd(const float* w_hh, const float* save, const float* dh2, float* dxproj, float* dpre2, int B, int H,
                  int64_t numel_xproj, void* stream);

int fst_rmsprop_multi(float* const* p_host, const float* const* g_host, float* const* v_host, const int64_t* numel_host,
                      const float* lr_host, int n_tensors, float alpha, float eps, void* stream);
int fst_adam_multi(float* const* p_host, const float* const* g_host, float* const* m_host, float* const* v_host,
                   const int64_t* numel_host, int n_tensors, const float* step_dev, float lr, float beta1, float beta2, float eps,
                   void* stream);
int fst_rmsprop_multi_dev(float* const* p_host, const float* const* g_host, float* const* v_host, const int64_t* numel_host,
                          const float* const* lr_dev_host, int n_tensors, float alpha, float eps, void* stream);
int fst_adam_multi_dev(float* const* p_host, const float* const* g_host, float* const* m_host, float* const* v_host,
                       const int64_t* numel_host, int n_tensors, const float* step_dev, const float* lr_dev, float beta1, float beta2,
                       float eps, void* stream);

int64_t fst_nonfinite_slots(int n_tensors);
int fst_nonfinite_multi(const float* const* x_host, const int64_t* numel_host, const int32_t* group_host, int n_tensors,
                        int32_t verdict_mask, int32_t* slots_dev, int64_t slots_len, int32_t* counts_dev, int32_t* verdict_dev,
                        float* ok_dev, int32_t* skipped_dev, void* stream);
int fst_rmsprop_multi_guard(float* const* p_host, const float* const* g_host, float* const* v_host, const int64_t* numel_host,
                            const float* lr_host, const float* const* lr_dev_host, int n_tensors, float alpha, float eps,
                            const int32_t* verdict_dev, void* stream);
int fst_adam_multi_guard(float* const* p_host, const float* const* g_host, float* const* m_host, float* const* v_host,
                         const int64_t* numel_host, int n_tensors, const float* step_dev, float lr, const float* lr_dev, float beta1,
                         float beta2, float eps, const int32_t* verdict_dev, void* stream);
int fst_guard_copy_multi(void* const* dst_host, const void* const* src_host, const int64_t* words_host, int n_tensors,
                         const int32_t* verdict_dev, int when, void* stream);

#ifdef __cplusplus
}
#endif
#endif
```

Measured before the change: 3659.

## Keep WaveNet d_u0 partials on-chip in LDS and fuse start-conv grad into stack backward

Adds kernel variants of the fused WaveNet stack backward. One parks the per-layer d_u0 skip-gradient accumulator in LDS across layers instead of reloading and storing it through global memory each layer. The other also folds the start-conv input gradient (d_a times start weight) into the last layer via an extra bf16x3 MFMA stage, so the separate grad_x0 GEMM and the da_out[0] buffer are skipped. Parking is on by default for the partial (no weight grad) projection path, while the start fusion needs mode 2. In exchange it uses more LDS, which can lower occupancy, and adds more templated code paths.

```diff
diff --git a/feature_level_style_transfer_for_tsc_amd/_lib.py b/feature_level_style_transfer_for_tsc_amd/_lib.py
--- a/feature_level_style_transfer_for_tsc_amd/_lib.py
+++ b/feature_level_style_transfer_for_tsc_amd/_lib.py
@@ -7,7 +7,7 @@
 
 import torch
 
-ABI_VERSION = 21
+ABI_VERSION = 22
 _LIB_NAME = "libfst_hip.so"
 _HERE = os.path.dirname(os.path.abspath(__file__))
 LIB_PATH = os.environ.get("FST_HIP_LIB", os.path.join(_HERE, _LIB_NAME))
@@ -68,6 +68,9 @@
     "fst_wn_stack_bwd": (c_int, [_P, _P, _P, _P, _P, _P, _P, _P, _P, c_int64, c_int, c_int, c_int, c_int, c_int, c_int64, c_void_p]),
     "fst_wn_stack_bwd_proj": (c_int, [_P, _P, _P, _P, _P, _P, _P, _P, c_int, c_int64, _P, c_int64, c_int, c_int, c_int, c_int, c_int,
                                       c_int64, c_void_p]),
+    "fst_wn_stack_bwd_proj_in_ok": (c_int, [c_int, c_int, c_int, c_int, c_int]),
+    "fst_wn_stack_bwd_proj_in": (c_int, [_P, _P, _P, _P, _P, _P, _P, c_int, c_int64, _P, c_int64, c_int, c_int, c_int, c_int, c_int,
+                                         c_int64, c_void_p]),
     "fst_wn_wgrad_ok": (c_int, [c_int, c_int, c_int, c_int, c_int, c_int]),
     "fst_wn_wgrad_workspace_floats": (c_int64, [c_int, c_int, c_int, c_int, c_int, c_int]),
     "fst_wn_wgrad_in": (c_int, [_P, _P, _P, c_int, c_int64, _P, _P, _P, c_int64, c_int, c_int, c_int, c_int, c_int, c_int, c_int64,
@@ -115,6 +118,8 @@
     "fst_wn_pack_bwd_stack": (c_int, [_P, c_int, c_int, c_int, _P, c_int64, c_void_p]),
     "fst_wn_bwd_proj_image_bytes": (c_int64, [c_int, c_int, c_int]),
     "fst_wn_pack_bwd_proj_stack": (c_int, [_P, _P, c_int, c_int, c_int, _P, c_int64, c_void_p]),
+    "fst_wn_start_image_bytes": (c_int64, [c_int]),
+    "fst_wn_pack_bwd_proj_in_stack": (c_int, [_P, _P, _P, c_int, c_int, c_int, c_int, _P, c_int64, _P, c_int64, c_void_p]),
     "fst_wn_layer_bwd": (c_int, [_P, _P, _P, _P, c_int64, _P, _P, c_int64, c_int, c_int, c_int, c_int, c_int64, c_void_p]),
     "fst_wn_dgrad_image_bytes": (c_int64, [c_int]),
     "fst_wn_pack_dgrad": (c_int, [_P, _P, c_int, c_int, c_int, _P, c_int64, c_void_p]),
diff --git a/feature_level_style_transfer_for_tsc_amd/csrc/wn_fused.hip b/feature_level_style_transfer_for_tsc_amd/csrc/wn_fused.hip
--- a/feature_level_style_transfer_for_tsc_amd/csrc/wn_fused.hip
+++ b/feature_level_style_transfer_for_tsc_amd/csrc/wn_fused.hip
@@ -834,9 +834,30 @@
   uint4* img[WS_MAXL];
   const float* end_w;
   int n, h2, nl, CH, CHO;
+  const float* start_w;
+  uint4* start_img;
+  int h;
 };
 
 __global__ __launch_bounds__(64) void wn_pack_bwd_proj_stack_kernel(WnPackBwdProjParams s) {
+  if ((int)blockIdx.y == s.nl) {
+    const int c = blockIdx.x, lane = threadIdx.x, hh = lane >> 5, m = lane & 31;
+    if (c >= s.CH) return;
+    float v[8];
+#pragma unroll
+    for (int j = 0; j < 8; ++j) {
+      const int ch = 16 * c + 8 * (j >> 2) + 4 * hh + (j & 3);
+      v[j] = (m < s.h && ch < s.n) ? s.start_w[(long long)ch * s.h + m] : 0.f;
+    }
+    unsigned hi[4], lo[4];
+#pragma unroll
+    for (int j = 0; j < 4; ++j) split_bf16_pair(v[2 * j], v[2 * j + 1], hi[j], lo[j]);
+    uint4* dst = s.start_img + (long long)c * 128 + lane;
+    dst[0] = make_uint4(hi[0], hi[1], hi[2], hi[3]);
+    dst[64] = make_uint4(lo[0], lo[1], lo[2], lo[3]);
+    if (c == 0 && lane == 0) s.start_img[(long long)s.CH * 128] = make_uint4(0u, 0u, 0u, 0u);
+    return;
+  }
   const int i = blockIdx.y, last = i == s.nl - 1 ? 1 : 0, n_da = last ? 0 : s.CH, n_blocks = (n_da + s.CHO) * 4;
   const int bx = blockIdx.x;
   if (bx >= n_blocks) return;
@@ -882,25 +903,49 @@
   return (int64_t)((last ? 0 : wn_ch(n)) + wn_ch(h2)) * WN_BW_A + 16;
 }
 
-extern "C" int fst_wn_pack_bwd_proj_stack(const float* const* rs_w, const float* end_w, int nl, int n, int h2, void* const* images,
-                                          int64_t image_bytes, void* stream) {
+extern "C" int64_t fst_wn_start_image_bytes(int n) {
+  if (n <= 0) return -1;
+  return (int64_t)wn_ch(n) * 2048 + 16;
+}
+
+static int wn_pack_bwd_proj_launch(const char* who, const float* const* rs_w, const float* end_w, const float* start_w, int nl, int n,
+                                   int h2, int h, void* const* images, int64_t image_bytes, void* start_image, void* stream) {
   FST_REQUIRE(rs_w && end_w && images && n > 0 && n <= 128 && h2 > 0 && h2 <= 64,
-              "fst_wn_pack_bwd_proj_stack: bad arguments (n=%d, h2=%d; needs n <= 128, h2 <= 64)", n, h2);
-  FST_REQUIRE(nl >= 1 && nl <= WS_MAXL, "fst_wn_pack_bwd_proj_stack: %d layers (1..%d)", nl, WS_MAXL);
-  FST_REQUIRE(image_bytes == fst_wn_bwd_proj_image_bytes(n, h2, 0), "fst_wn_pack_bwd_proj_stack: images are %lld bytes, expected %lld",
+              "%s: bad arguments (n=%d, h2=%d; needs n <= 128, h2 <= 64)", who, n, h2);
+  FST_REQUIRE(nl >= 1 && nl <= WS_MAXL, "%s: %d layers (1..%d)", who, nl, WS_MAXL);
+  FST_REQUIRE(image_bytes == fst_wn_bwd_proj_image_bytes(n, h2, 0), "%s: images are %lld bytes, expected %lld", who,
               (long long)image_bytes, (long long)fst_wn_bwd_proj_image_bytes(n, h2, 0));
   WnPackBwdProjParams s = {};
   for (int i = 0; i < nl; ++i) {
-    FST_REQUIRE(rs_w[i] && images[i], "fst_wn_pack_bwd_proj_stack: null operand in layer %d", i);
-    FST_REQUIRE(fst_aligned16(images[i]), "fst_wn_pack_bwd_proj_stack: images must be 16-byte aligned");
+    FST_REQUIRE(rs_w[i] && images[i], "%s: null operand in layer %d", who, i);
+    FST_REQUIRE(fst_aligned16(images[i]), "%s: images must be 16-byte aligned", who);
     s.rs_w[i] = rs_w[i];
     s.img[i] = static_cast<uint4*>(images[i]);
   }
   s.end_w = end_w; s.n = n; s.h2 = h2; s.nl = nl; s.CH = wn_ch(n); s.CHO = wn_ch(h2);
+  s.start_w = start_w; s.start_img = static_cast<uint4*>(start_image); s.h = h;
   const int stages = (nl > 1 ? s.CH : 0) + s.CHO;
-  hipLaunchKernelGGL(wn_pack_bwd_proj_stack_kernel, dim3((unsigned)(stages * 4), (unsigned)nl), dim3(64), 0, (hipStream_t)stream, s);
+  const int gx = start_w && s.CH > stages * 4 ? s.CH : stages * 4;
+  hipLaunchKernelGGL(wn_pack_bwd_proj_stack_kernel, dim3((unsigned)gx, (unsigned)(nl + (start_w ? 1 : 0))), dim3(64), 0,
+                     (hipStream_t)stream, s);
   FST_LAUNCH_CHECK();
   return 0;
+}
+
+extern "C" int fst_wn_pack_bwd_proj_stack(const float* const* rs_w, const float* end_w, int nl, int n, int h2, void* const* images,
+                                          int64_t image_bytes, void* stream) {
+  return wn_pack_bwd_proj_launch("fst_wn_pack_bwd_proj_stack", rs_w, end_w, nullptr, nl, n, h2, 0, images, image_bytes, nullptr, stream);
+}
+
+extern "C" int fst_wn_pack_bwd_proj_in_stack(const float* const* rs_w, const float* end_w, const float* start_w, int nl, int n, int h2,
+                                             int h, void* const* images, int64_t image_bytes, void* start_image,
+                                             int64_t start_image_bytes, void* stream) {
+  FST_REQUIRE(start_w && start_image && h > 0 && h <= 32, "fst_wn_pack_bwd_proj_in_stack: bad arguments (h=%d; needs h <= 32)", h);
+  FST_REQUIRE(fst_aligned16(start_image) && start_image_bytes == fst_wn_start_image_bytes(n),
+              "fst_wn_pack_bwd_proj_in_stack: the start image is %lld bytes, expected %lld, 16-byte aligned", (long long)start_image_bytes,
+              (long long)fst_wn_start_image_bytes(n));
+  return wn_pack_bwd_proj_launch("fst_wn_pack_bwd_proj_in_stack", rs_w, end_w, start_w, nl, n, h2, h, images, image_bytes, start_image,
+                                 stream);
 }
 
 struct WnBwdParams {
@@ -1400,11 +1445,22 @@
   int dil[WS_MAXL], nblkw[WS_MAXL], gsw[WS_MAXL], slot_d[WS_MAXL];
   int nl, B, L, n, h, CH, CHK;
   int SR, SCH;
+  const char* img_start;
+  int park_off, park_nr;
 };
 
-__global__ __launch_bounds__(512, 2) void wn_stack_bwd_kernel(WnStackParams p_by_value) {
+#define WS_PARK 1
+#define WS_START 2
+
+__device__ __forceinline__ float* ws_park_ptr(char* ldsb, int park_off, int wave_s) {
+  unsigned lane;
+  asm volatile("v_mbcnt_lo_u32_b32 %0, -1, 0\n\tv_mbcnt_hi_u32_b32 %0, -1, %0" : "=v"(lane));
+  return reinterpret_cast<float*>(ldsb + park_off + wave_s * 256) + lane;
+}
+
+template <int FORM>
+__device__ __forceinline__ void wn_stack_bwd_body() {
   const auto& p = *(const __attribute__((address_space(4))) WnStackParams*)__builtin_amdgcn_kernarg_segment_ptr();
-  (void)p_by_value;
   extern __shared__ __attribute__((aligned(16))) float lds[];
   char* const ldsb = reinterpret_cast<char*>(lds);
   const int tid = threadIdx.x, lane = tid & 63;
@@ -1538,6 +1594,25 @@
         run_pass(std::integral_constant<int, 0>{});
         run_pass(std::integral_constant<int, 1>{});
         if (rs_out) wn_reduce_row_sums(rsum, 256, rs_out, p.B, b, tid);
+        if constexpr ((FORM & WS_PARK) != 0) {
+          __builtin_amdgcn_sched_barrier(0);
+          if (last) {
+            const __amdgpu_buffer_rsrc_t du_r = ws_rsrc(p.d_u0 + (long long)b * p.d_u0_bs);
+            ws_acc_load(acc[4][0], du_r, wl0, 0, wave_n0, p.h, L);
+            ws_acc_load(acc[4][1], du_r, wl1, 0, wave_n0 + 32, p.h, L);
+          } else {
+            const float* const park = ws_park_ptr(ldsb, p.park_off, wave_s);
+            const int nr = ws_opaque(p.park_nr);
+#pragma unroll
+            for (int r = 0; r < 16; ++r)
+#pragma unroll
+              for (int cb = 0; cb < 2; ++cb) {
+                float x = 0.f;
+                if (r < nr) x = park[(2 * r + cb) * 512];
+                acc[4][cb][r] = x;
+              }
+          }
+        }
         FST_T(ta3);
         wait_vmcnt<0>();
         __syncthreads();
@@ -1555,8 +1630,10 @@
         const int sub = (0 - dil) & 3;
         auto issue = [&](int c, int slot) { wn_dgrad_issue(ldsb + slot * slotb, img, dgr, c, 0, n, L, dil, nblkw, gsw, wave_s, lane); };
         FST_T(tb0);
-        ws_acc_load(acc[4][0], du_r, wl0, 0, wave_n0, p.h, L);
-        ws_acc_load(acc[4][1], du_r, wl1, 0, wave_n0 + 32, p.h, L);
+        if constexpr ((FORM & WS_PARK) == 0) {
+          ws_acc_load(acc[4][0], du_r, wl0, 0, wave_n0, p.h, L);
+          ws_acc_load(acc[4][1], du_r, wl1, 0, wave_n0 + 32, p.h, L);
+        }
         asm volatile("" ::: "memory");
         issue(0, 0);
         int slot = 0;
@@ -1572,6 +1649,37 @@
         FST_T(tb2);
         FST_ACC(5, tb1, tb2);
         __syncthreads();
+        if constexpr ((FORM & WS_START) != 0) {
+          if (i == 0) {
+            const char* const img_s = p.img_start + lane * 16;
+            f32x16 su[2];
+            zero_acc(su);
+            auto start_stage = [&](auto cc) {
+              constexpr int c = decltype(cc)::value;
+              if (c < CH) {
+                const bf16x8 ah = *reinterpret_cast<const bf16x8*>(img_s + c * 2048);
+                const bf16x8 al = *reinterpret_cast<const bf16x8*>(img_s + c * 2048 + 1024);
+#pragma unroll
+                for (int cb = 0; cb < 2; ++cb) {
+                  float v[8];
+#pragma unroll
+                  for (int j = 0; j < 8; ++j) v[j] = acc[c >> 1][cb][8 * (c & 1) + j];
+                  bf16x8 bh, bl;
+                  split_bf16x8(v, bh, bl);
+                  mfma_bf3(su[cb], ah, al, bh, bl);
+                }
+              }
+            };
+            start_stage(std::integral_constant<int, 0>{}); start_stage(std::integral_constant<int, 1>{});
+            start_stage(std::integral_constant<int, 2>{}); start_stage(std::integral_constant<int, 3>{});
+            start_stage(std::integral_constant<int, 4>{}); start_stage(std::integral_constant<int, 5>{});
+            start_stage(std::integral_constant<int, 6>{}); start_stage(std::integral_constant<int, 7>{});
+#pragma unroll
+            for (int cb = 0; cb < 2; ++cb)
+#pragma unroll
+              for (int r = 0; r < 16; ++r) acc[4][cb][r] += su[cb][r];
+          }
+        }
         {
           const int ni = i > 0 ? i - 1 : p.nl - 1, nb = i > 0 ? b : b + (int)gridDim.x;
           if (nb < p.B) {
@@ -1589,8 +1697,14 @@
           const int rows = ib < 4 ? n - ib * 32 : p.h;
           if (ib < 4) {
             if (da_store) ws_acc_store(acc[ib][cb], dan_r, cb ? wl1 : wl0, ib * 32, tcol, rows, L);
+          } else if ((FORM & WS_PARK) == 0 || i == 0) {
+            ws_acc_store(acc[ib][cb], du_r, cb ? wl1 : wl0, 0, tcol, rows, L);
           } else {
-            ws_acc_store(acc[ib][cb], du_r, cb ? wl1 : wl0, 0, tcol, rows, L);
+            float* const park = ws_park_ptr(ldsb, p.park_off, wave_s);
+            const int nr = ws_opaque(p.park_nr);
+#pragma unroll
+            for (int r = 0; r < 16; ++r)
+              if (r < nr) park[(2 * r + cb) * 512] = acc[ib][cb][r];
           }
           if (rs_out && ib < 4) {
             float av[16];
@@ -1602,8 +1716,10 @@
         if (rs_out) wn_reduce_row_sums(rsum, 128, rs_out, p.B, b, tid);
         FST_T(tb3);
         FST_ACC(6, tb2, tb3);
-        wait_vmcnt<0>();
-        __syncthreads();
+        if constexpr ((FORM & WS_PARK) == 0) {
+          wait_vmcnt<0>();
+          __syncthreads();
+        }
         FST_T(tb4);
         FST_ACC(7, tb3, tb4);
       }
@@ -1613,6 +1729,10 @@
   FST_ACC(9, tw0, tw1);
   FST_FLUSH(wn_stamps);
 }
+
+__global__ __launch_bounds__(512, 2) void wn_stack_bwd_kernel(WnStackParams) { wn_stack_bwd_body<0>(); }
+__global__ __launch_bounds__(512, 2) void wn_stack_bwd_park_kernel(WnStackParams) { wn_stack_bwd_body<WS_PARK>(); }
+__global__ __launch_bounds__(512, 2) void wn_stack_bwd_in_kernel(WnStackParams) { wn_stack_bwd_body<WS_PARK | WS_START>(); }
 
 extern "C" int fst_wn_stack_bwd_ok(int n, int h, int L, int nl) {
   if (!(n > 0 && n <= 128 && h > 0 && h <= 32 && L > 0 && L <= WS_TN && L % 4 == 0 && nl > 0 && nl <= WS_MAXL)) return 0;
@@ -1621,11 +1741,29 @@
   return 1;
 }
 
+static inline int wn_park_regs(int h) {
+  int nr = 0;
+  for (int r = 0; r < 16; ++r) nr += (r & 3) + 8 * (r >> 2) < h ? 1 : 0;
+  return nr;
+}
+
+static size_t wn_stack_bwd_lds(int nl, int n, int h, int skip_rows, bool park) {
+  size_t lds_bytes = WS_LDS_A + 8192;
+  for (int i = 0; i < nl; ++i) {
+    int nblkw, gsw, slot;
+    wn_dgrad_geometry(1 << i, &nblkw, &gsw, &slot);
+    if ((size_t)2 * slot > lds_bytes) lds_bytes = (size_t)2 * slot;
+  }
+  const size_t park_end = (size_t)(wn_ch(n) + wn_ch(skip_rows)) * WN_BW_A + (size_t)wn_park_regs(h) * 2 * 2048;
+  return park && park_end > lds_bytes ? park_end : lds_bytes;
+}
+
 static int wn_stack_bwd_launch(const char* who, const float* const* ts, const void* const* img_b, const void* const* img_d,
                                float* const* dg, float* const* da_out, float* const* rs_b, float* const* rs_d, const float* skip,
                                int skip_rows, float* d_u0, int64_t d_u0_bs, int nl, int B, int L, int n, int h, int64_t numel_a,
-                               void* stream) {
-  FST_REQUIRE(ts && img_b && img_d && dg && da_out && skip && d_u0, "%s: null table", who);
+                               void* stream, int form = 0, const void* img_start = nullptr) {
+  const bool start = (form & WS_START) != 0;
+  FST_REQUIRE(ts && img_b && img_d && dg && (da_out || start) && skip && d_u0, "%s: null table", who);
   FST_REQUIRE(fst_wn_stack_bwd_ok(n, h, L, nl), "%s: not served: n=%d h=%d L=%d nl=%d (needs n <= 128, h <= 32, "
               "L <= 512, L %% 4 == 0, nl <= %d)", who, n, h, L, nl, WS_MAXL);
   FST_REQUIRE(B > 0 && (long long)B * n * L == (long long)numel_a,
@@ -1634,17 +1772,17 @@
               "%s: d_u0 batch stride %lld (needs >= h*L = %lld and a multiple of 4)", who, (long long)d_u0_bs, (long long)h * L);
   FST_REQUIRE((rs_b == nullptr) == (rs_d == nullptr), "%s: row sums of both kinds or of neither", who);
   WnStackParams p = {};
-  size_t lds_bytes = WS_LDS_A + 8192;
+  const size_t lds_bytes = wn_stack_bwd_lds(nl, n, h, skip_rows, (form & WS_PARK) != 0);
   for (int i = 0; i < nl; ++i) {
-    FST_REQUIRE(ts[i] && img_b[i] && img_d[i] && dg[i] && (i > 0 || da_out[i]), "%s: null operand of layer %d", who, i);
-    FST_REQUIRE(fst_aligned16(ts[i]) && fst_aligned16(img_b[i]) && fst_aligned16(img_d[i]) && fst_aligned16(dg[i]) && fst_aligned16(da_out[i]),
+    float* const da_i = da_out ? da_out[i] : nullptr;
+    FST_REQUIRE(ts[i] && img_b[i] && img_d[i] && dg[i] && (i > 0 || da_i || start), "%s: null operand of layer %d", who, i);
+    FST_REQUIRE(fst_aligned16(ts[i]) && fst_aligned16(img_b[i]) && fst_aligned16(img_d[i]) && fst_aligned16(dg[i]) && fst_aligned16(da_i),
                 "%s: operands of layer %d must be 16-byte aligned", who, i);
     p.ts[i] = ts[i]; p.img_b[i] = static_cast<const char*>(img_b[i]); p.img_d[i] = static_cast<const char*>(img_d[i]);
-    p.dg[i] = dg[i]; p.da_out[i] = da_out[i];
+    p.dg[i] = dg[i]; p.da_out[i] = da_i;
     p.rs_b[i] = rs_b ? rs_b[i] : nullptr; p.rs_d[i] = rs_d ? rs_d[i] : nullptr;
     p.dil[i] = 1 << i;
     wn_dgrad_geometry(p.dil[i], &p.nblkw[i], &p.gsw[i], &p.slot_d[i]);
-    if ((size_t)2 * p.slot_d[i] > lds_bytes) lds_bytes = (size_t)2 * p.slot_d[i];
   }
   FST_REQUIRE(fst_aligned16(skip) && fst_aligned16(d_u0), "%s: %s / d_u0 must be 16-byte aligned", who, skip_rows == n ? "d_out" : "d_o");
   FST_REQUIRE(lds_bytes <= 160 * 1024, "%s: %zu bytes of LDS", who, lds_bytes);
@@ -1652,11 +1790,14 @@
   p.nl = nl; p.B = B; p.L = L; p.n = n; p.h = h; p.CH = wn_ch(n); p.CHK = (2 * n + 15) / 16;
   p.SR = skip_rows; p.SCH = wn_ch(skip_rows);
   FST_REQUIRE((size_t)(p.CH + p.SCH) * WN_BW_A <= WS_LDS_A, "%s: a weight image of %d stages does not fit its LDS", who, p.CH + p.SCH);
-  if (int rc = fst_allow_full_lds((const void*)wn_stack_bwd_kernel, who)) return rc;
+  p.img_start = static_cast<const char*>(img_start);
+  p.park_off = (p.CH + p.SCH) * WN_BW_A; p.park_nr = wn_park_regs(h);
+  void (*const kernel)(WnStackParams) = form == 0 ? wn_stack_bwd_kernel : (start ? wn_stack_bwd_in_kernel : wn_stack_bwd_park_kernel);
+  if (int rc = fst_allow_full_lds((const void*)kernel, who)) return rc;
   const int cus = fst_cu_count_or(256);
   const int grid = B < cus ? B : cus;
-  fst_wn_set_route(FST_WN_ROUTE_STACK_BWD, 0, 0, 0, 0, grid, 1, 1, 1, 2, nl, (int)lds_bytes);
-  hipLaunchKernelGGL(wn_stack_bwd_kernel, dim3((unsigned)grid), dim3(512), lds_bytes, (hipStream_t)stream, p);
+  fst_wn_set_route(FST_WN_ROUTE_STACK_BWD, form, 0, 0, 0, grid, 1, 1, 1, 2, nl, (int)lds_bytes);
+  hipLaunchKernelGGL(kernel, dim3((unsigned)grid), dim3(512), lds_bytes, (hipStream_t)stream, p);
   FST_LAUNCH_CHECK();
   return 0;
 }
@@ -1680,3 +1821,23 @@
   return wn_stack_bwd_launch("fst_wn_stack_bwd_proj", ts, img_b, img_d, dg, da_out, rs_b, rs_d, d_o, h2, d_u0, d_u0_bs, nl, B, L, n, h,
                              numel_a, stream);
 }
+
+extern "C" int fst_wn_stack_bwd_proj_in_ok(int n, int h, int h2, int L, int nl) {
+  if (!fst_wn_stack_bwd_ok(n, h, L, nl) || h2 <= 0 || h2 > 64) return 0;
+  if ((size_t)(wn_ch(n) + wn_ch(h2)) * WN_BW_A > WS_LDS_A) return 0;
+  return wn_stack_bwd_lds(nl, n, h, h2, true) <= 160 * 1024 ? 1 : 0;
+}
+
+extern "C" int fst_wn_stack_bwd_proj_in(const float* const* ts, const void* const* img_b, const void* const* img_d, float* const* dg,
+                                        float* const* da_out, const void* img_start, const float* d_o, int h2, int64_t numel_o,
+                                        float* d_u0, int64_t d_u0_bs, int nl, int B, int L, int n, int h, int64_t numel_a,
+                                        void* stream) {
+  fst_wn_clear_route();
+  FST_REQUIRE(fst_wn_stack_bwd_proj_in_ok(n, h, h2, L, nl), "fst_wn_stack_bwd_proj_in: not served: n=%d h=%d h2=%d L=%d nl=%d", n, h, h2,
+              L, nl);
+  FST_REQUIRE(B > 0 && (long long)B * h2 * L == (long long)numel_o,
+              "fst_wn_stack_bwd_proj_in: B*h2*L does not match the element count %lld of d_o [B][h2][L]", (long long)numel_o);
+  FST_REQUIRE(fst_aligned16(img_start), "fst_wn_stack_bwd_proj_in: the start image must be 16-byte aligned");
+  return wn_stack_bwd_launch("fst_wn_stack_bwd_proj_in", ts, img_b, img_d, dg, da_out, nullptr, nullptr, d_o, h2, d_u0, d_u0_bs, nl, B,
+                             L, n, h, numel_a, stream, img_start ? (WS_PARK | WS_START) : WS_PARK, img_start);
+}
diff --git a/feature_level_style_transfer_for_tsc_amd/ops.py b/feature_level_style_transfer_for_tsc_amd/ops.py
--- a/feature_level_style_transfer_for_tsc_amd/ops.py
+++ b/feature_level_style_transfer_for_tsc_amd/ops.py
@@ -92,6 +92,8 @@
         return f"wn_layer_fwd_kernel<{route[1]}>"
     if fam == WN_ROUTE_LAYER_INFER:
         return f"wn_layer_infer_kernel<{route[1]}>"
+    if fam == WN_ROUTE_STACK_BWD and route[1]:
+        return "wn_stack_bwd_in_kernel" if route[1] & 2 else "wn_stack_bwd_park_kernel"
     return _WN_ROUTE_NAMES[fam]
 
 
@@ -1276,6 +1278,23 @@
                                                                 stream_ptr()), "fst_wn_pack_bwd_proj_stack")))
 
 
+def wn_pack_bwd_proj_in_layers(rs_ws: Sequence[Tensor], end_w: Tensor, start_w: Tensor, n: int) -> List[Tensor]:
+    lib, nl, h2, h = _lib.load(), len(rs_ws), end_w.size(0), start_w.size(1)
+    if nl > WN_PACK_MAX_LAYERS or tuple(end_w.shape) != (h2, n, 1) or h2 > 64 or tuple(start_w.shape) != (n, h, 1) or h > 32:
+        raise ValueError(f"wn_pack_bwd_proj_in_layers: {nl} layers, end_w {tuple(end_w.shape)}, start_w {tuple(start_w.shape)} (at most "
+                         f"{WN_PACK_MAX_LAYERS} layers, end_w [2h <= 64, n = {n}, 1], start_w [n, h <= 32, 1])")
+    return _pack_stack(_WnImages(
+        nl + 1,
+        lambda i: (("wn_bwd_proj", n, h2, i == nl - 1, rs_ws[i].data_ptr(), rs_ws[i]._version, end_w.data_ptr(), end_w._version)
+                   if i < nl else ("wn_bwd_start", n, h, start_w.data_ptr(), start_w._version)),
+        lambda i: lib.fst_wn_bwd_proj_image_bytes(n, h2, int(i == nl - 1)) if i < nl else lib.fst_wn_start_image_bytes(n),
+        lambda i: (rs_ws[i], end_w) if i < nl else (start_w,), None,
+        lambda srcs, imgs: check(lib.fst_wn_pack_bwd_proj_in_stack(
+            _ptr_table([s_[0] for s_ in srcs[:nl]]), ptr(srcs[0][1]), ptr(srcs[nl][0]), nl, n, h2, h, _ptr_table(imgs[:nl]),
+            lib.fst_wn_bwd_proj_image_bytes(n, h2, 0), ptr(imgs[nl]), lib.fst_wn_start_image_bytes(n), stream_ptr()),
+            "fst_wn_pack_bwd_proj_in_stack")))
+
+
 def _wn_dgrad_images(in_ws: Sequence[Tensor], cond_ws: Sequence[Tensor], n: int, h: int) -> _WnImages:
     lib, nl = _lib.load(), len(in_ws)
     nbytes = lib.fst_wn_dgrad_image_bytes(n)
@@ -1409,6 +1428,13 @@
     return 2 * h <= 64 and (mode == "2" or (mode != "0" and _PARTIAL_BACKWARD and not need_w))
 
 
+def wn_partial_onchip(n: int, h: int, L: int, nl: int) -> int:
+    mode = os.environ.get("FST_WN_PARTIAL_ONCHIP", "1")
+    if mode == "0" or not _PARTIAL_BACKWARD or not _lib.load().fst_wn_stack_bwd_proj_in_ok(n, h, 2 * h, L, nl):
+        return 0
+    return 2 if mode == "2" else 1
+
+
 def wn_stack_bwd_ok(n: int, h: int, L: int, nl: int) -> bool:
     if os.environ.get("FST_WN_STACK", "1") == "0":
         return False
@@ -1465,16 +1491,19 @@
 
 def wn_stack_bwd(ts_list: Sequence[Tensor], imgs_b: Sequence[Tensor], imgs_d: Sequence[Tensor], dgs: Sequence[Tensor],
                  da_out: Sequence[Optional[Tensor]], d_out: Optional[Tensor], d_u0: Tensor, n: int, h: int,
-                 part_b: Optional[Tensor] = None, part_d: Optional[Tensor] = None, do: Optional[Tensor] = None) -> None:
+                 part_b: Optional[Tensor] = None, part_d: Optional[Tensor] = None, do: Optional[Tensor] = None,
+                 onchip: bool = False, start_img: Optional[Tensor] = None) -> None:
     lib = _lib.load()
     nl = len(ts_list)
     if (do is None) == (d_out is None):
         raise ValueError("wn_stack_bwd: d_out or do, one of them")
+    if (onchip or start_img is not None) and (do is None or not onchip or part_b is not None or part_d is not None):
+        raise ValueError("wn_stack_bwd: onchip / start_img need do, onchip and no row sums")
     if do is not None:
         if do.dim() != 3 or not do.is_contiguous() or do.dtype != torch.float32:
             raise ValueError("wn_stack_bwd: do must be a contiguous fp32 [B, 2h, L]")
         B, h2, L = do.shape
-        numel = _same_numel(*[t for t in da_out if t is not None])
+        numel = _same_numel(*[t for t in da_out if t is not None]) if any(t is not None for t in da_out) else B * n * L
         if numel != B * n * L:
             raise ValueError(f"wn_stack_bwd: da_out must be [B, n, L] = {(B, n, L)}")
     else:
@@ -1494,7 +1523,11 @@
     t0 = KERNEL_TIMER.begin() if KERNEL_TIMER is not None else None
     rs_b = None if part_b is None else _ptr_table([part_b[i] for i in range(nl)])
     rs_d = None if part_d is None else _ptr_table([part_d[i] for i in range(nl)])
-    if do is not None:
+    if onchip:
+        check(lib.fst_wn_stack_bwd_proj_in(_ptr_table(ts_list), _ptr_table(imgs_b), _ptr_table(imgs_d), _ptr_table(dgs),
+                                           _ptr_table(da_out), None if start_img is None else ptr(start_img), ptr(do), h2, do.numel(),
+                                           ptr(d_u0), d_u0_bs, nl, B, L, n, h, numel, stream_ptr()), "fst_wn_stack_bwd_proj_in")
+    elif do is not None:
         check(lib.fst_wn_stack_bwd_proj(_ptr_table(ts_list), _ptr_table(imgs_b), _ptr_table(imgs_d), _ptr_table(dgs),
                                         _ptr_table(da_out), rs_b, rs_d, ptr(do), h2, do.numel(), ptr(d_u0), d_u0_bs, nl, B, L, n, h,
                                         numel, stream_ptr()), "fst_wn_stack_bwd_proj")
@@ -1505,7 +1538,9 @@
     if t0 is not None:
         sr = n if do is None else h2
         flops = 2.0 * B * L * (n * ((n + sr) * nl - n) + nl * 2 * n * (3 * n + h))
-        rows = nl * (2 * n + sr + 2 * 2 * n + 2 * h) + n * sum(t is not None for t in da_out)
+        rows = nl * (2 * n + sr + 2 * 2 * n) + 2 * h * (1 if onchip else nl) + n * sum(t is not None for t in da_out)
+        if start_img is not None:
+            flops += 2.0 * B * L * n * h
         KERNEL_TIMER.end("wn_stack_bwd_kernel", t0, flops, 4.0 * B * L * rows)
 
 
@@ -1599,10 +1634,12 @@
     if not fused:
         d_a = _wn_backward_unfused(S, W, G, a_list, ts_list, acts_list, u0, d_out, d_u0, da_sums)
     elif stack:
-        d_a, part_b, part_d = _wn_backward_stack(S, W, G, a_list, ts_list, u0, d_out, d_u0, pool, do if proj else None)
+        onchip = wn_partial_onchip(n, h, L, nl) if proj and not need_w else 0
+        d_a, part_b, part_d = _wn_backward_stack(S, W, G, a_list, ts_list, u0, d_out, d_u0, pool, do if proj else None, onchip)
     else:
         d_a, part_b, part_d = _wn_backward_layers(S, W, G, a_list, ts_list, u0, d_out, d_u0, da_sums, pool)
-    S.start.grad_x0(d_a, W[0], out=d_u0, flags=EPI_ACC1)
+    if d_a is not None:
+        S.start.grad_x0(d_a, W[0], out=d_u0, flags=EPI_ACC1)
     if need_w:
         S.start.grad_w(u0, None, d_a, out0=G[0])
         o0 = S.offsets[6 + nl]
@@ -1642,20 +1679,27 @@
 
 
 def _wn_backward_stack(S: WNSpecs, W, G, a_list, ts_list, u0: Tensor, d_out: Optional[Tensor], d_u0: Tensor, pool,
-                       do: Optional[Tensor] = None):
+                       do: Optional[Tensor] = None, onchip: int = 0):
     nl, n, h = S.n_layers, S.n, S.h
     B, _, L = u0.shape
     rs_ws = [_wn_layer(S, W, i)[4] for i in range(nl)]
-    imgs_b = wn_pack_bwd_layers(rs_ws, n, acc_order=True) if do is None else wn_pack_bwd_proj_layers(rs_ws, W[4], n)
+    start_img = None
+    if do is None:
+        imgs_b = wn_pack_bwd_layers(rs_ws, n, acc_order=True)
+    elif onchip == 2:
+        *imgs_b, start_img = wn_pack_bwd_proj_in_layers(rs_ws, W[4], W[0], n)
+    else:
+        imgs_b = wn_pack_bwd_proj_layers(rs_ws, W[4], n)
     imgs_d = wn_pack_dgrad_layers([_wn_layer(S, W, i)[0] for i in range(nl)], [_wn_layer(S, W, i)[1] for i in range(nl)], n, h)
     new = lambda *shape: torch.empty(*shape, device=u0.device, dtype=torch.float32)
     if G is None:
-        dgs, da_out = [new(B, 2 * n, L)] * nl, [new(B, n, L)] + [None] * (nl - 1)
+        dgs, da_out = [new(B, 2 * n, L)] * nl, [None if start_img is not None else new(B, n, L)] + [None] * (nl - 1)
         part_b = part_d = None
     else:
         dgs, da_out = [new(B, 2 * n, L) for _ in range(nl)], [new(B, n, L) for _ in range(nl)]
         part_b, part_d = new(nl, 256, B), new(nl, 128, B)
-    wn_stack_bwd(ts_list, imgs_b, imgs_d, dgs, da_out, d_out if do is None else None, d_u0, n, h, part_b, part_d, do)
+    wn_stack_bwd(ts_list, imgs_b, imgs_d, dgs, da_out, d_out if do is None else None, d_u0, n, h, part_b, part_d, do,
+                 onchip=onchip > 0, start_img=start_img)
     if G is not None:
         for i in range(nl):
             _wn_wgrad_rs(S, i, da_out[i + 1] if i + 1 < nl else None, d_out, ts_list[i], G, pool)
diff --git a/include/fst_hip.h b/include/fst_hip.h
--- a/include/fst_hip.h
+++ b/include/fst_hip.h
@@ -7,7 +7,7 @@
 extern "C" {
 #endif
 
-#define FST_ABI_VERSION 21
+#define FST_ABI_VERSION 22
 
 int fst_version(void);
 const char* fst_last_error(void);
@@ -117,6 +117,10 @@
 int64_t fst_wn_bwd_proj_image_bytes(int n, int h2, int last);
 int fst_wn_pack_bwd_proj_stack(const float* const* rs_w, const float* end_w, int nl, int n, int h2, void* const* images,
                                int64_t image_bytes, void* stream);
+int64_t fst_wn_start_image_bytes(int n);
+int fst_wn_pack_bwd_proj_in_stack(const float* const* rs_w, const float* end_w, const float* start_w, int nl, int n, int h2, int h,
+                                  void* const* images, int64_t image_bytes, void* start_image, int64_t start_image_bytes,
+                                  void* stream);
 int fst_wn_layer_fwd(const float* a, int64_t a_bs, const float* u0, int64_t u0_bs, const void* image, int64_t image_bytes,
                      float* ts, float* acts, float* a_next, float* out, int first, int last,
                      int B, int L, int n, int h, int dil, int64_t numel_a, void* stream);
@@ -159,6 +163,11 @@
                           float* const* da_out, float* const* rs_b , float* const* rs_d ,
                           const float* d_o, int h2, int64_t numel_o, float* d_u0, int64_t d_u0_bs, int nl, int B, int L, int n,
                           int h, int64_t numel_a, void* stream);
+int fst_wn_stack_bwd_proj_in_ok(int n, int h, int h2, int L, int nl);
+int fst_wn_stack_bwd_proj_in(const float* const* ts, const void* const* img_b, const void* const* img_d, float* const* dg,
+                             float* const* da_out , const void* img_start ,
+                             const float* d_o, int h2, int64_t numel_o, float* d_u0, int64_t d_u0_bs, int nl, int B, int L, int n,
+                             int h, int64_t numel_a, void* stream);
 
 int fst_wn_wgrad_ok(int kind, int B, int L, int n, int h, int dil);
 int64_t fst_wn_wgrad_workspace_floats(int kind, int B, int L, int n, int h, int last);
```

Result: no change. 3680, median of 5 (+0.6%).
